# matteosantama/dantzig

Hardware: AMD Instinct MI355X
Metric: simplex_iterations_per_sec (higher is better)
Workload: dtype f64

## Files before the change

dantzig_amd/_build.py:

```python
from __future__ import annotations

import os
import shutil
import subprocess
from concurrent.futures import ThreadPoolExecutor

HERE = os.path.dirname(os.path.abspath(__file__))
CSRC = os.path.join(HERE, "csrc")
OBJ = os.path.join(HERE, "_obj")
LIB = os.path.join(HERE, "libdantzig_amd.so")
ARCH = "gfx950"
SOURCES = ["engine.hip", "k_vector.hip", "k_price.hip", "k_strict.hip", "k_fast.hip", "k_chain.hip", "k_sparse.hip", "k_refactor.hip", "k_rowshard.hip", "k_drift.hip", "k_restart.hip", "k_extend.hip", "k_remove.hip", "k_batch.hip", "k_batch_fast.hip",
           "k_mip.hip", "k_duals.hip", "k_ranging.hip", "k_rays.hip", "model.cpp", "mip.cpp", "lpgen.cpp"]
FLAGS = ["-O3", "-std=c++17", "-fPIC", "-ffp-contract=off", "-fno-fast-math", "-Wall",
         "-Wno-unused-result", "-Wno-unused-value"]


def _hipcc() -> str:
    exe = shutil.which("hipcc") or "/opt/rocm/bin/hipcc"
    if not os.path.exists(exe):
        raise RuntimeError("hipcc not found: dantzig_amd needs the ROCm toolchain to build")
    return exe


def _newest(paths) -> float:
    return max(os.path.getmtime(p) for p in paths)


def _deps():
    hdrs = [os.path.join(CSRC, "common.h"), os.path.join(CSRC, "k_price_kernels.h"),
            os.path.join(CSRC, "fast_decide.h"), os.path.join(CSRC, "fast_rows.h"),
            os.path.join(CSRC, "chain_barrier.h"), os.path.join(CSRC, "batch_strict.h"),
            os.path.join(CSRC, "batch_host.h"),
            os.path.join(CSRC, "mip_internal.h"), os.path.join(CSRC, "duals.h"), os.path.join(CSRC, "ranging.h"), os.path.join(CSRC, "rays.h"),
            os.path.join(os.path.dirname(HERE), "include", "dantzig_amd.h")]
    return hdrs


def _compile(src: str) -> str:
    path = os.path.join(CSRC, src)
    obj = os.path.join(OBJ, src + ".o")
    if os.path.exists(obj) and os.path.getmtime(obj) >= _newest([path] + _deps()):
        return obj
    cmd = [_hipcc(), f"--offload-arch={ARCH}", *FLAGS, "-c", path, "-o", obj]
    if src.endswith(".cpp"):
        cmd.insert(1, "-x")
        cmd.insert(2, "c++")
        cmd = [c for c in cmd if not c.startswith("--offload-arch")]
    subprocess.check_call(cmd)
    return obj


def build(force: bool = False, verbose: bool = False) -> str:
    os.makedirs(OBJ, exist_ok=True)
    if force:
        for f in os.listdir(OBJ):
            os.remove(os.path.join(OBJ, f))
    with ThreadPoolExecutor(max_workers=4) as ex:
        objs = list(ex.map(_compile, SOURCES))
    if force or not os.path.exists(LIB) or os.path.getmtime(LIB) < _newest(objs):
        cmd = [_hipcc(), f"--offload-arch={ARCH}", "-shared", "-fPIC", "-o", LIB, *objs, "-ldl", "-pthread"]
        subprocess.check_call(cmd)
    if verbose:
        print("built", LIB)
    return LIB


if __name__ == "__main__":
    import sys

    build(force="--force" in sys.argv, verbose=True)
```

dantzig_amd/_ffi.py:

```python
from __future__ import annotations

import ctypes as C
import os

import numpy as np

_HERE = os.path.dirname(os.path.abspath(__file__))
LIB_PATH = os.path.join(_HERE, "libdantzig_amd.so")

OPTIMAL, UNBOUNDED, INFEASIBLE, ITER_LIMIT, SINGULAR, PANIC, RUNNING, NEAR_TIE, NODE_LIMIT = range(9)
E_DEVICE, E_ARG, E_NOMEM = -1, -2, -3
STRICT, FAST, AUTO = 0, 1, 2
PRICE_AUTO, PRICE_SEQ, PRICE_WAVE, PRICE_TREE = 0, 1, 2, 3
STEP_PRIMAL, STEP_DUAL = 0, 1
NEAR_TIE_COUNT, NEAR_TIE_STOP = 0, 1
(K_STATUS, K_FTRAN, K_RATIO, K_BTRAN, K_PRICE, K_UPDATE, K_BASIS_UPDATE, K_LU, K_XCHG1, K_XCHG2,
 K_COUNT) = range(11)
KERNEL_CLASSES = ["status", "ftran", "ratio", "btran", "price", "update", "basis_update", "lu",
                  "exchange1", "exchange2"]

EXPORTS = [
    "dzg_abi_version", "dzg_status_str", "dzg_last_error", "dzg_device_count",
    "dzg_opts_default", "dzg_solver_create", "dzg_solver_run", "dzg_solver_result",
    "dzg_solver_destroy", "dzg_core_solve", "dzg_model_solve", "dzg_build_standard_form",
    "dzg_kernel_lu_solve", "dzg_kernel_neg_t_dot", "dzg_kernel_first_pivot",
    "dzg_kernel_second_pivot", "dzg_gen_dense_lp", "dzg_gen_sparse_lp", "dzg_merge_candidates",
    "dzg_shard_record_doubles", "dzg_shard_phase1", "dzg_shard_phase2", "dzg_shard_phase3",
    "dzg_solver_poll", "dzg_solver_set_budget", "dzg_comm_unique_id", "dzg_shard_comm_init",
    "dzg_shard_run", "dzg_shard_run_lockstep", "dzg_solver_stream", "dzg_solver_refactor",
    "dzg_gen_dense_lp_block", "dzg_solver_set_profile", "dzg_kernel_neg_t_dot_csc",
    "dzg_shard_comm_size", "dzg_solver_upload_columns", "dzg_debug_hold_cus", "dzg_debug_hold_wait",
    "dzg_core_solve_full_csc", "dzg_debug_live_lists", "dzg_debug_rl_listed",
    "dzg_debug_basis_inverse", "dzg_batch_solve", "dzg_model_solve_batch", "dzg_mip_opts_default",
    "dzg_mip_solve", "dzg_mip_last_warm_stats", "dzg_debug_cand_reduce", "dzg_debug_chain_instance",
    "dzg_solver_duals", "dzg_batch_solve_duals", "dzg_model_solve_duals",
    "dzg_model_solve_batch_duals", "dzg_model_map_duals",
    "dzg_solver_ranging", "dzg_batch_solve_ranging", "dzg_model_solve_ranging",
    "dzg_model_solve_batch_ranging",
    "dzg_solver_ray", "dzg_batch_solve_rays", "dzg_model_solve_rays", "dzg_model_solve_batch_rays",
    "dzg_model_map_ray",
    "dzg_batch_solve_fast", "dzg_model_solve_batch_fast", "dzg_debug_batch_fast_inverse",
    "dzg_solver_reoptimize",
    "dzg_solver_extend", "dzg_solver_dims", "dzg_debug_matrix", "dzg_debug_matrix_rows",
    "dzg_debug_extend_ms",
    "dzg_solver_remove",
]

BATCH_MAX_ROWS = 128
DUALS_FRESH, DUALS_CARRIED = 1, 2
DUALS_SOURCE_NAMES = {DUALS_FRESH: "fresh", DUALS_CARRIED: "carried"}
RAY_PRIMAL, RAY_FARKAS = 1, 2


class Lp(C.Structure):
    _fields_ = [
        ("m", C.c_int64), ("n", C.c_int64), ("n_struct", C.c_int64),
        ("a", C.c_void_p), ("lda", C.c_int64), ("var_col", C.c_void_p),
        ("c", C.c_void_p), ("constant", C.c_double),
        ("basis", C.c_void_p), ("nonbasis", C.c_void_p), ("x", C.c_void_p), ("z", C.c_void_p),
        ("col_ptr", C.c_void_p), ("row_idx", C.c_void_p), ("val", C.c_void_p),
        ("xbar", C.c_void_p), ("zbar", C.c_void_p),
    ]


class Opts(C.Structure):
    _fields_ = [
        ("numerics", C.c_int32), ("price_kernel", C.c_int32), ("device", C.c_int32),
        ("auto_strict_rows", C.c_int32), ("max_iter", C.c_int64), ("epsilon", C.c_double),
        ("log_capacity", C.c_int64), ("poll_interval", C.c_int32), ("profile", C.c_int32),
        ("col_begin", C.c_int64), ("col_end", C.c_int64), ("rank", C.c_int32),
        ("world", C.c_int32), ("stream", C.c_void_p), ("refactor_interval", C.c_int64),
        ("a_is_block", C.c_int32), ("near_tie_action", C.c_int32),
        ("replicate_matrix", C.c_int32), ("auto_restart_rows", C.c_int32), ("tie_tol", C.c_double),
        ("seven_launches", C.c_int32), ("auto_strict_budget_s", C.c_int32),
        ("shard_rows", C.c_int32), ("reserved0", C.c_int32),
    ]


class Pivot(C.Structure):
    _fields_ = [("kind", C.c_int32), ("reserved", C.c_int32), ("entering", C.c_int64),
                ("leaving", C.c_int64), ("mu", C.c_double)]


class Result(C.Structure):
    _fields_ = [
        ("status", C.c_int32), ("numerics_used", C.c_int32), ("iterations", C.c_int64),
        ("objective", C.c_double),
        ("basis", C.c_void_p), ("nonbasis", C.c_void_p), ("x", C.c_void_p), ("xbar", C.c_void_p),
        ("z", C.c_void_p), ("zbar", C.c_void_p), ("log", C.c_void_p), ("log_cap", C.c_int64),
        ("kernel_ms", C.c_double * K_COUNT), ("kernel_launches", C.c_int64 * K_COUNT),
        ("price_bytes", C.c_double), ("solve_ms", C.c_double), ("max_pivot_error", C.c_double),
        ("near_ties", C.c_int64), ("first_near_tie", C.c_int64), ("min_margin", C.c_double),
        ("margins", C.c_void_p), ("dense_columns", C.c_int64), ("refactors", C.c_int64),
        ("chain_fallbacks", C.c_int64), ("price_pass_used", C.c_int32),
        ("price_rows_copy", C.c_int32), ("state_drift", C.c_double),
    ]


class Model(C.Structure):
    _fields_ = [
        ("nvars", C.c_int64), ("has_lb", C.c_void_p), ("has_ub", C.c_void_p),
        ("lb", C.c_void_p), ("ub", C.c_void_p),
        ("obj_nterms", C.c_int64), ("obj_var", C.c_void_p), ("obj_coef", C.c_void_p),
        ("obj_const", C.c_double),
        ("ncons", C.c_int64), ("con_ptr", C.c_void_p), ("con_var", C.c_void_p),
        ("con_coef", C.c_void_p), ("con_b", C.c_void_p),
    ]


class ModelResult(C.Structure):
    _fields_ = [("status", C.c_int32), ("numerics_used", C.c_int32), ("iterations", C.c_int64),
                ("objective", C.c_double), ("values", C.c_void_p), ("m", C.c_int64),
                ("n", C.c_int64), ("near_ties", C.c_int64), ("first_near_tie", C.c_int64)]


class Duals(C.Structure):
    _fields_ = [("source", C.c_int32), ("reserved", C.c_int32), ("y", C.c_void_p), ("d", C.c_void_p),
# ... 66 lines not shown
class MipWarmStats(C.Structure):
    _fields_ = [("nodes_warm", C.c_int64), ("nodes_restarted", C.c_int64),
                ("warm_iterations", C.c_int64), ("restart_iterations", C.c_int64)]


class MipNode(C.Structure):
    _fields_ = [("id", C.c_int64), ("parent", C.c_int64), ("branch_var", C.c_int64),
                ("direction", C.c_int32), ("status", C.c_int32), ("bound", C.c_double),
                ("iterations", C.c_int64), ("objective", C.c_double)]


class MipResult(C.Structure):
    _fields_ = [("status", C.c_int32), ("has_incumbent", C.c_int32), ("objective", C.c_double),
                ("values", C.c_void_p), ("best_bound", C.c_double), ("nodes_solved", C.c_int64),
                ("nodes_batched", C.c_int64), ("nodes_sequential", C.c_int64), ("nodes_fast", C.c_int64),
                ("nodes_pruned", C.c_int64), ("nodes_dropped", C.c_int64), ("rounds", C.c_int64),
                ("lp_iterations", C.c_int64), ("incumbent_node", C.c_int64), ("failed_node", C.c_int64),
                ("log", C.c_void_p), ("log_cap", C.c_int64), ("log_count", C.c_int64)]


class Candidate(C.Structure):
    _fields_ = [("ratio", C.c_double), ("pos", C.c_int64), ("y", C.c_double),
                ("ybar", C.c_double), ("dy", C.c_double)]


class DantzigAmdError(RuntimeError):
    """A call into the HIP engine failed (no GPU, bad argument, out of memory)."""


_lib = None


def lib() -> C.CDLL:
    global _lib
    if _lib is None:
        if not os.path.exists(LIB_PATH):
            raise DantzigAmdError(
                f"{LIB_PATH} is missing: build the HIP engine first "
                "(python -m dantzig_amd._build). dantzig_amd has no CPU fallback.")
        _lib = C.CDLL(LIB_PATH)
        _lib.dzg_status_str.restype = C.c_char_p
        _lib.dzg_last_error.restype = C.c_char_p
        _lib.dzg_merge_candidates.restype = C.c_int64
        _lib.dzg_solver_destroy.restype = None
        _lib.dzg_opts_default.restype = None
        _lib.dzg_gen_dense_lp.argtypes = [C.c_uint64, C.c_int64, C.c_int64, C.c_void_p, C.c_int64,
                                          C.c_void_p, C.c_void_p]
        _lib.dzg_gen_dense_lp_block.argtypes = [C.c_uint64, C.c_int64, C.c_int64, C.c_int64,
                                                C.c_int64, C.c_void_p, C.c_int64, C.c_void_p,
                                                C.c_void_p]
        _lib.dzg_solver_run.argtypes = [C.c_void_p, C.c_int64]
        _lib.dzg_solver_result.argtypes = [C.c_void_p, C.c_void_p]
        _lib.dzg_solver_destroy.argtypes = [C.c_void_p]
        _lib.dzg_shard_record_doubles.restype = C.c_int64
        _lib.dzg_shard_record_doubles.argtypes = [C.c_void_p]
        _lib.dzg_shard_phase1.argtypes = [C.c_void_p, C.c_void_p]
        _lib.dzg_shard_phase2.argtypes = [C.c_void_p, C.c_void_p, C.c_void_p]
        _lib.dzg_shard_phase3.argtypes = [C.c_void_p, C.c_void_p]
        _lib.dzg_solver_poll.argtypes = [C.c_void_p, C.c_void_p, C.c_void_p]
        _lib.dzg_solver_set_budget.argtypes = [C.c_void_p, C.c_int64]
        _lib.dzg_comm_unique_id.argtypes = [C.c_void_p]
        _lib.dzg_shard_comm_init.argtypes = [C.c_void_p, C.c_void_p]
        _lib.dzg_shard_run.argtypes = [C.c_void_p, C.c_int64]
        _lib.dzg_shard_comm_size.argtypes = [C.c_void_p]
        _lib.dzg_shard_run_lockstep.argtypes = [C.c_void_p, C.c_int32, C.c_int64]
        _lib.dzg_solver_stream.restype = C.c_void_p
        _lib.dzg_solver_stream.argtypes = [C.c_void_p]
        _lib.dzg_solver_refactor.argtypes = [C.c_void_p]
        _lib.dzg_solver_set_profile.argtypes = [C.c_void_p, C.c_int32]
        _lib.dzg_core_solve_full_csc.argtypes = [C.c_int64, C.c_int64, C.c_void_p, C.c_void_p,
                                                 C.c_void_p, C.c_void_p, C.c_double, C.c_void_p,
                                                 C.c_void_p, C.c_void_p, C.c_void_p, C.c_void_p,
                                                 C.c_void_p]
        _lib.dzg_debug_hold_cus.argtypes = [C.c_int32, C.c_int32, C.c_double]
        _lib.dzg_debug_live_lists.restype = C.c_int64
        _lib.dzg_debug_live_lists.argtypes = [C.c_void_p, C.c_void_p]
        _lib.dzg_debug_basis_inverse.restype = C.c_int
        _lib.dzg_debug_basis_inverse.argtypes = [C.c_void_p, C.c_int64, C.c_int64, C.c_void_p, C.c_void_p]
        _lib.dzg_debug_cand_reduce.restype = C.c_int
        _lib.dzg_debug_cand_reduce.argtypes = [C.c_int32, C.c_int32, C.c_int64, C.c_void_p, C.c_void_p,
                                               C.c_void_p, C.c_void_p, C.c_void_p, C.c_void_p, C.c_void_p]
        _lib.dzg_debug_chain_instance.restype = C.c_int
        _lib.dzg_debug_chain_instance.argtypes = [C.c_int32] * 7
        _lib.dzg_batch_solve.argtypes = [C.c_void_p, C.c_int64, C.c_void_p, C.c_int64, C.c_void_p]
        _lib.dzg_model_solve_batch.argtypes = [C.c_void_p, C.c_int64, C.c_void_p, C.c_void_p]
        _lib.dzg_batch_solve_fast.argtypes = [C.c_void_p, C.c_int64, C.c_void_p, C.c_int64, C.c_int64,
                                              C.c_void_p]
        _lib.dzg_model_solve_batch_fast.argtypes = [C.c_void_p, C.c_int64, C.c_void_p, C.c_void_p]
        _lib.dzg_debug_batch_fast_inverse.restype = C.c_int
        _lib.dzg_debug_batch_fast_inverse.argtypes = [C.c_void_p, C.c_int64, C.c_void_p, C.c_int64, C.c_int64,
                                                      C.c_void_p, C.c_void_p]
        _lib.dzg_solver_duals.argtypes = [C.c_void_p, C.c_void_p]
        _lib.dzg_batch_solve_duals.argtypes = [C.c_void_p, C.c_int64, C.c_void_p, C.c_int64, C.c_void_p,
                                               C.c_void_p]
        _lib.dzg_model_solve_duals.argtypes = [C.c_void_p, C.c_void_p, C.c_void_p, C.c_void_p]
        _lib.dzg_model_solve_batch_duals.argtypes = [C.c_void_p, C.c_int64, C.c_void_p, C.c_void_p,
                                                     C.c_void_p]
        _lib.dzg_model_map_duals.argtypes = [C.c_void_p, C.c_void_p, C.c_int64, C.c_void_p]
        _lib.dzg_solver_ranging.argtypes = [C.c_void_p, C.c_void_p, C.c_void_p, C.c_void_p]
        _lib.dzg_batch_solve_ranging.argtypes = [C.c_void_p, C.c_int64, C.c_void_p, C.c_int64, C.c_void_p,
                                                 C.c_void_p, C.c_void_p, C.c_void_p]
        _lib.dzg_model_solve_ranging.argtypes = [C.c_void_p, C.c_void_p, C.c_void_p, C.c_void_p, C.c_void_p,
                                                 C.c_void_p]
        _lib.dzg_model_solve_batch_ranging.argtypes = [C.c_void_p, C.c_int64, C.c_void_p, C.c_void_p,
                                                       C.c_void_p, C.c_void_p, C.c_void_p]
        _lib.dzg_solver_ray.argtypes = [C.c_void_p, C.c_void_p]
        _lib.dzg_batch_solve_rays.argtypes = [C.c_void_p, C.c_int64, C.c_void_p, C.c_int64, C.c_void_p,
                                              C.c_void_p, C.c_void_p]
        _lib.dzg_model_solve_rays.argtypes = [C.c_void_p, C.c_void_p, C.c_void_p, C.c_void_p, C.c_void_p]
        _lib.dzg_model_solve_batch_rays.argtypes = [C.c_void_p, C.c_int64, C.c_void_p, C.c_void_p,
                                                    C.c_void_p, C.c_void_p]
        _lib.dzg_model_map_ray.argtypes = [C.c_void_p, C.c_int32, C.c_void_p, C.c_void_p, C.c_int64,
                                           C.c_int64, C.c_void_p]
        _lib.dzg_solver_reoptimize.argtypes = [C.c_void_p, C.c_void_p]
        _lib.dzg_solver_extend.argtypes = [C.c_void_p, C.c_void_p]
        _lib.dzg_solver_remove.argtypes = [C.c_void_p, C.c_void_p, C.c_void_p, C.c_void_p]
        _lib.dzg_solver_dims.argtypes = [C.c_void_p, C.c_void_p, C.c_void_p, C.c_void_p]
        _lib.dzg_debug_matrix.argtypes = [C.c_void_p, C.c_int64, C.c_int64, C.c_void_p, C.c_int64]
        _lib.dzg_debug_matrix_rows.restype = C.c_int64
        _lib.dzg_debug_matrix_rows.argtypes = [C.c_void_p, C.c_int64, C.c_int64, C.c_void_p, C.c_int64]
        _lib.dzg_debug_extend_ms.argtypes = [C.c_void_p, C.c_void_p]
        _lib.dzg_mip_opts_default.restype = None
        _lib.dzg_mip_opts_default.argtypes = [C.c_void_p]
        _lib.dzg_mip_solve.argtypes = [C.c_void_p, C.c_void_p, C.c_void_p, C.c_void_p, C.c_void_p]
        _lib.dzg_mip_last_warm_stats.restype = None
        _lib.dzg_mip_last_warm_stats.argtypes = [C.c_void_p]
        _lib.dzg_solver_upload_columns.argtypes = [C.c_void_p, C.c_int64, C.c_int64, C.c_void_p,
                                                   C.c_int64]
    return _lib


def ptr(a: np.ndarray | None) -> C.c_void_p:
    return C.c_void_p(None if a is None else a.ctypes.data)


def f64(a) -> np.ndarray:
    return np.ascontiguousarray(a, dtype=np.float64)


def i64(a) -> np.ndarray:
    return np.ascontiguousarray(a, dtype=np.int64)


def status_str(code: int) -> str:
    return lib().dzg_status_str(int(code)).decode()


def check(rc: int, what: str) -> int:
    if rc < 0:
        msg = lib().dzg_last_error().decode()
        raise DantzigAmdError(f"{what}: {status_str(rc)} ({msg})")
    return rc


class RangingBuffers:

    def __init__(self, cost_dirs, rhs_dirs, pivot_tol: float = 0.0):
        def csr(dirs):
            ptr_, idx, val = [0], [], []
            for d in dirs:
                for j, v in d.items():
                    idx.append(int(j))
                    val.append(float(v))
                ptr_.append(len(idx))
            return i64(ptr_), i64(idx + [0]), f64(val + [0.0])

# ... 90 lines not shown
```

dantzig_amd/core.py:

```python
from __future__ import annotations

import ctypes as C
from dataclasses import dataclass, field

import numpy as np

from . import _ffi
from ._ffi import (AUTO, FAST, STRICT, PRICE_AUTO, PRICE_SEQ, PRICE_WAVE, PRICE_TREE,
                   STEP_DUAL,
                   STEP_PRIMAL, NEAR_TIE_COUNT, NEAR_TIE_STOP, DantzigAmdError, f64, i64, ptr)

STATUS_NAMES = {0: "optimal", 1: "unbounded", 2: "infeasible", 3: "iter_limit", 4: "singular",
                5: "panic", 6: "running", 7: "near_tie"}


@dataclass
class CoreLP:
    a: np.ndarray | None
    c: np.ndarray
    basis: np.ndarray
    nonbasis: np.ndarray
    x: np.ndarray
    z: np.ndarray
    var_col: np.ndarray | None = None
# ... 416 lines not shown
        c = None if c is None else f64(c)
        if b is not None and b.shape != (m,):
            raise ValueError(f"reoptimize: b has shape {b.shape}, the LP has {m} rows")
        if c is not None and c.shape != (n,):
            raise ValueError(f"reoptimize: c has shape {c.shape}, the LP has {n} variables")
        chg = _ffi.Reopt(ptr(b), ptr(c), 0.0 if constant is None else float(constant),
                         0 if constant is None else 1, 0)
        _ffi.check_reopt(_ffi.lib().dzg_solver_reoptimize(self._h, C.byref(chg)), "dzg_solver_reoptimize")

    def extend(self, rows=None, rhs=None, cols=None, c_cols=None) -> None:
        lp2 = extended_lp(self._lp, rows, rhs, cols, c_cols)
        m, ns = self._lp.m, self._lp.n_struct
        rows, rhs, cols, c_cols = _extend_blocks(m, ns, rows, rhs, cols, c_cols)
        p, r = len(rhs), len(c_cols)
        rows_rm = np.ascontiguousarray(rows)
        cols_cm = np.ascontiguousarray(cols.T)
        ext = _ffi.Extend(p, r, ptr(rows_rm) if p else None, max(ns, 1), ptr(rhs) if p else None,
                          ptr(cols_cm) if r else None, max(m + p, 1), ptr(c_cols) if r else None)
        _ffi.check_extend(_ffi.lib().dzg_solver_extend(self._h, C.byref(ext)), "dzg_solver_extend")
        self._lp = lp2

    def _at_current_basis(self) -> CoreLP:
        import dataclasses

        res = self.result(log=False)
        return dataclasses.replace(self._lp, basis=res.basis, nonbasis=res.nonbasis, x=res.x, z=res.z,
                                   xbar=None, zbar=None)

    def removable(self) -> tuple[np.ndarray, np.ndarray]:
        if self._lp.a is None or self._lp.block is not None:
            raise NotImplementedError("remove is not supported on CSC storage or sharded solvers")
        m, ns = self._lp.m, self._lp.n_struct
        res = self.result(log=False)
        codes = _codes(self._lp)
        in_basis, out_of_basis = codes[res.basis], codes[res.nonbasis]
        row_mask, col_mask = np.zeros(m, bool), np.zeros(ns, bool)
        row_mask[-1 - in_basis[in_basis < 0]] = True
        col_mask[out_of_basis[out_of_basis >= 0]] = True
        return row_mask, col_mask

    def remove(self, rows=None, cols=None) -> tuple[np.ndarray, np.ndarray]:
        if self._lp.a is None or self._lp.block is not None:
            raise NotImplementedError("remove is not supported on CSC storage or sharded solvers")
        drop_row, drop_col = _remove_lists(self._lp.m, self._lp.n_struct, rows, cols)
        lp2, _, _ = reduced_lp(self._at_current_basis(), rows, cols)
        r, c = np.flatnonzero(drop_row).astype(np.int64), np.flatnonzero(drop_col).astype(np.int64)
        var_map, row_map = np.zeros(self._lp.n, np.int64), np.zeros(self._lp.m, np.int64)
        rem = _ffi.Remove(len(r), ptr(r) if len(r) else None, len(c), ptr(c) if len(c) else None)
        _ffi.check_extend(_ffi.lib().dzg_solver_remove(self._h, C.byref(rem), ptr(var_map), ptr(row_map)),
                          "dzg_solver_remove")
        self._lp = lp2
        return var_map, row_map

    def dims(self) -> tuple[int, int, int]:
        v = [C.c_int64(0), C.c_int64(0), C.c_int64(0)]
        _ffi.check(_ffi.lib().dzg_solver_dims(self._h, *(C.byref(x) for x in v)), "dzg_solver_dims")
        return tuple(int(x.value) for x in v)

    def debug_matrix(self) -> np.ndarray:
        m, _, ns = self.dims()
        out = np.zeros((max(ns, 1), max(m, 1)))
        _ffi.check(_ffi.lib().dzg_debug_matrix(self._h, 0, ns, ptr(out), max(m, 1)), "dzg_debug_matrix")
        return out[:ns, :m].T.copy()

    def debug_matrix_rows(self) -> np.ndarray | None:
        m, _, ns = self.dims()
        out = np.zeros((max(m, 1), max(ns, 1)))
        got = _ffi.lib().dzg_debug_matrix_rows(self._h, 0, m, ptr(out), max(ns, 1))
        _ffi.check(int(got), "dzg_debug_matrix_rows")
        return out[:m, :ns].copy() if got == m and m > 0 else None

    def debug_extend_ms(self) -> tuple[float, float, float]:
        ms = np.zeros(3)
        _ffi.check(_ffi.lib().dzg_debug_extend_ms(self._h, ptr(ms)), "dzg_debug_extend_ms")
        return tuple(float(x) for x in ms)

    def debug_inverse(self, row0: int, row1: int) -> tuple[np.ndarray, dict]:
        m = self._lp.m
        out = np.zeros((max(int(row1) - int(row0), 0), m))
        info = np.zeros(4, np.int64)
        _ffi.check(_ffi.lib().dzg_debug_basis_inverse(self._h, int(row0), int(row1), ptr(out), ptr(info)),
                   "dzg_debug_basis_inverse")
        return out, dict(k=int(info[0]), neta=int(info[1]), rows=(int(info[2]), int(info[3])))

    def close(self) -> None:
        if self._h:
            _ffi.lib().dzg_solver_destroy(self._h)
            self._h = C.c_void_p(None)

    def __enter__(self):
        return self

    def __exit__(self, *exc):
        self.close()

    def __del__(self):
        try:
            self.close()
        except Exception:
            pass


def solve(lp: CoreLP, log: bool = True, **opts) -> CoreResult:
    with Solver(lp, **opts) as s:
        s.run(0)
        return s.result(log=log)


def core_solve(lp: CoreLP, log_cap: int = 1 << 20, **opts) -> CoreResult:
    with Solver.__new__(Solver)._prepare(lp, opts) as s:
        m, q = lp.m, lp.n - lp.m
        basis, nonbasis = np.zeros(max(m, 1), np.int64), np.zeros(max(q, 1), np.int64)
        x, xbar = np.zeros(max(m, 1)), np.zeros(max(m, 1))
        z, zbar = np.zeros(max(q, 1)), np.zeros(max(q, 1))
        buf = (_ffi.Pivot * max(log_cap, 1))()
        margins = np.full(max(log_cap, 1), np.inf)
        r = _ffi.Result()
        r.basis, r.nonbasis, r.x, r.xbar = ptr(basis), ptr(nonbasis), ptr(x), ptr(xbar)
        r.z, r.zbar = ptr(z), ptr(zbar)
        r.log, r.log_cap, r.margins = C.cast(buf, C.c_void_p), log_cap, ptr(margins)
        rc = _ffi.lib().dzg_core_solve(C.byref(s._c_lp), C.byref(s._opts), C.byref(r))
        _ffi.check(rc, "dzg_core_solve")
        cnt = int(min(r.iterations, log_cap))
        arr = np.ctypeslib.as_array(buf)[:cnt]
        pivots = list(zip(arr["kind"].tolist(), arr["entering"].tolist(),
                          arr["leaving"].tolist(), arr["mu"].tolist()))
        return CoreResult(
            status=STATUS_NAMES.get(r.status, str(r.status)), status_code=r.status,
            numerics="strict" if r.numerics_used == STRICT else "fast",
            iterations=int(r.iterations), objective=float(r.objective),
            basis=basis[:m].copy(), nonbasis=nonbasis[:q].copy(), x=x[:m].copy(),
            xbar=xbar[:m].copy(), z=z[:q].copy(), zbar=zbar[:q].copy(), pivots=pivots,
            margins=margins[:cnt].copy(), **_counters(r))


_PIVOT_DTYPE = np.dtype([("kind", "<i4"), ("reserved", "<i4"), ("entering", "<i8"),
                         ("leaving", "<i8"), ("mu", "<f8")])


def solve_batch(lps, log: bool = True, log_cap: int = 4096, pivots_per_launch: int = 0,
                duals: bool = False, ranging=False, pivot_tol: float = 0.0, rays: bool = False,
                **opts) -> list:
    import time

    lps = list(lps)
    numerics = opts.get("numerics", AUTO)
    if numerics not in (STRICT, AUTO):
        raise ValueError("solve_batch runs STRICT numerics only (numerics=STRICT or AUTO)")
    if rays and ranging is not False and ranging is not None:
        raise ValueError("rays=True and ranging: the ranging call carries no ray; ask in two calls")
    for i, lp in enumerate(lps):
        if lp.block is not None:
            raise ValueError(f"lps[{i}]: a column-block LP cannot be batched")
        if lp.a is None and lp.n_struct > 0:
            raise ValueError(f"lps[{i}]: CSC input cannot be batched (dense `a` only)")
        if lp.m > _ffi.BATCH_MAX_ROWS:
            raise ValueError(f"lps[{i}]: {lp.m} rows; the batch takes at most {_ffi.BATCH_MAX_ROWS}")
    marshalled = [_c_lp(lp) for lp in lps]
    count = len(lps)
    c_lps = (_ffi.Lp * max(count, 1))(*[c for c, _ in marshalled])
    ms = [lp.m for lp in lps]
    qs = [lp.n - lp.m for lp in lps]
    mo = np.concatenate([[0], np.cumsum(ms)]).astype(np.int64)
    qo = np.concatenate([[0], np.cumsum(qs)]).astype(np.int64)
    basis, x, xbar = np.zeros(mo[-1] + 1, np.int64), np.zeros(mo[-1] + 1), np.zeros(mo[-1] + 1)
    nonbasis, z, zbar = np.zeros(qo[-1] + 1, np.int64), np.zeros(qo[-1] + 1), np.zeros(qo[-1] + 1)
# ... 303 lines not shown
```

dantzig_amd/csrc/common.h:

```cpp
#pragma once

#include <hip/hip_runtime.h>
#include <stdint.h>

#include "../../include/dantzig_amd.h"

#define DZG_WAVE 64

struct DzgCtl {
    int status;
    int kind;
    long long iter;
    long long iter_stop;
    int enter_pos;
    int leave_pos;
    int enter_var;
    int leave_var;
    double mu;
    double t, s, tbar, sbar;
    long long nb_struct;
    double price_bytes;
    int lu_mu;
    int lu_pivot_zero;
    int ncompact;
// ... 457 lines not shown
    double *P0, *P1;
    int *piv;
    int *pz;
    int *ptab;
    double *part_r;
    int *part_k;
    int nparts;
};
void dzg_lu_layout(int n, DzgLu *w);

struct __attribute__((aligned(16))) DzgLiveEntry {
    int row;
    int pad_;
    double val;
};

struct DzgDev {
    int m, q, n, ns;
    long long lda;
    const double *A;
    int csc;
    const long long *cptr;
    const int *ridx;
    const double *cval;
    const int *var_col;
    int *basis, *nonbasis;
    double *x, *xbar, *z, *zbar;
    double *dx, *dz, *v, *acol;
    DzgCtl *ctl;
    int *log_kind, *log_enter, *log_leave;
    double *log_mu;
    long long log_cap;
    double *binv;
    long long ldb;
    int *drow;
    int *dslot;
    double *U;
    double *W;
    long long ldw;
    double *Wc;
    double *ag;
    double *beta;
    double *beta_part;
    int beta_split;
    int *plist;
    int *pslot;
    int *pcode;
    int *cpos;
    double *fpx_r, *fpz_r, *rx_r, *rz_r;
    int *fpx_k, *fpz_k, *rx_k, *rz_k;
    double *fpx_h, *fpz_h, *rx_h, *rz_h;
    double *log_margin;
    int *bcode, *nbcode;
    int spb;
    const long long *rptr;
    const int *cidx;
    const double *rval;
    int *sslot;
    int *spos;
    int *bslot;
    int *rowpos;
    int *bcnt;
    int *bcol;
    double *bval;
    double *dxs;
    int *acol_code;
    int *lcnt;
    DzgLiveEntry *lent;
    unsigned long long *rl_work;
    DzgLu lu;
    double eps;
    int col0, col1, rank, world;
    int repl;
    long long xstride;
    const double *At;
    long long ldt;
    double *ppart;
    double *vc;
    int rows_T;
    int k_lo_hint;
    int k_hint;
    int price_cols_hint;
    int rs, rs_r0, rs_r1;
    long long rs_mcol;
    int ftran_variant;
    int ftran_nt_k;
    int fold_k;
};

#ifdef __HIPCC__
__device__ __forceinline__ const double *dzg_enter_col(const DzgCtl *ctl, int code,
                                                       const double *A, long long lda, int col0,
                                                       const double *xrecv, long long xstride)
{
    if (code < 0) return nullptr;
    if (xrecv && xstride > 8) return xrecv + (long long)ctl->enter_src * xstride + 8;
    return A + (long long)(code - col0) * lda;
}
#endif

void dzg_launch_status(const DzgDev &d, hipStream_t st);
void dzg_launch_ratio(const DzgDev &d, int need_kind, hipStream_t st);
void dzg_launch_prepare(const DzgDev &d, hipStream_t st);
void dzg_launch_update_vectors(const DzgDev &d, hipStream_t st);
void dzg_launch_load_column(const DzgDev &d, int need_kind, hipStream_t st);
void dzg_launch_unit_rhs(const DzgDev &d, hipStream_t st);
int dzg_run_first_pivot(int64_t len, const double *y, const double *ybar, int64_t *pos_out);
int dzg_run_second_pivot(int64_t len, double mu, const double *y, const double *ybar,
                         const double *dy, int64_t *pos_out);

void dzg_launch_price(const DzgDev &d, int kernel, hipStream_t st);
void dzg_launch_price_fast(const DzgDev &d, int kernel, hipStream_t st, int need_kind = -1,
                           int skip_finish = 0, int small = 0, unsigned long long *dbg = nullptr);
int dzg_price_small(const DzgDev &d, int kernel);
int dzg_price_small_partials(const DzgDev &d);
int dzg_price_rows_certain(const DzgDev &d, int kernel);
void dzg_launch_transpose_to_rows(const double *A, long long lda, int m, int n, double *At,
                                  long long ldt, hipStream_t st);
int dzg_price_rows_groups(void);
int dzg_price_partials(int kernel);
int dzg_price_partials_dev(const DzgDev &d, int kernel);
#define DZG_PRICE_CSC_KERNEL 100
#define DZG_RL_WORK_SLOTS 2048
void dzg_launch_price_raw(int kernel, int m, long long lda, const double *A, const int *cols,
                          int ncols, const double *v, double *out, hipStream_t st);
void dzg_launch_price_csc_raw(const long long *cptr, const int *ridx, const double *cval,
                              const int *cols, int ncols, const double *v, double *out,
                              hipStream_t st);

void dzg_launch_strict_solve(const DzgDev &d, int transposed, hipStream_t st);
void dzg_launch_lu_raw(const DzgLu &w, DzgCtl *ctl, double *x_out, hipStream_t st);

void dzg_launch_fast_init(const DzgDev &d, hipStream_t st);
void dzg_launch_fast_select_prep(const DzgDev &d, int mode, int nrz, const double *xrecv,
                                 hipStream_t st);
void dzg_launch_fast_gemv(const DzgDev &d, int need_kind, const double *xrecv, hipStream_t st);
void dzg_launch_fast_btran(const DzgDev &d, hipStream_t st);
void dzg_launch_fast_update(const DzgDev &d, int only_partials, hipStream_t st);
void dzg_launch_fast_flush(const DzgDev &d, hipStream_t st);
void dzg_launch_refactor_lists(const DzgDev &d, int *spos, int *scode, int *lpos, int *lrow,
                               int *counts, hipStream_t st);
void dzg_launch_refactor_a(const DzgDev &d, int k, double *G, double *X, long long ldg, int *scode,
                           int *singular, hipStream_t st);
double *dzg_launch_refactor_b(const DzgDev &d, int k, int nl, double *G, double *X, double *Pn, double *Tri,
                              long long ldg,
                              int *piv, int *spos, int *scode, int *lpos, int *lrow, int *lslot,
                              int *singular, hipStream_t st);
void dzg_launch_refactor_c(const DzgDev &d, int k, int nl, double *G, double *X, long long ldg,
                           int *lpos, int *singular, hipStream_t st);
void dzg_launch_lockstep_sum(double *const *bufs, int world, long long count, hipStream_t st);
void dzg_launch_shard_propose(const DzgDev &d, int mode, int nrz, double *xsend, hipStream_t st);
void dzg_launch_lockstep_allgather(double *const *ptrs, int world, int which, long long xstride,
                                   hipStream_t st);

#define DZG_CHAIN_AGCAP 16384
#define DZG_CHAIN_BAR_WORDS (16 * 10)
int dzg_chain_resident_per_cu(void);
enum {
    DZG_CHAIN_GENERIC = 0,
    DZG_CHAIN_P1_NARROW = 1,
    DZG_CHAIN_P4_NARROW = 2,
    DZG_CHAIN_P4_WIDE = 3,
};
void dzg_launch_chain_pre(const DzgDev &d, int grid, unsigned long long *bar,
                          unsigned long long *dbg, const double *xrecv, hipStream_t st, int instances = 0);
void dzg_launch_chain_post(const DzgDev &d, int grid, unsigned long long *bar,
                           unsigned long long *dbg, int only_partials, int nrz, const double *xrecv,
                           hipStream_t st, int fold = 0, int price_small = 0, int instances = 0);

void dzg_launch_rs_propose(const DzgDev &d, int mode, int nrz, double *xsend, hipStream_t st);
void dzg_launch_rs_select(const DzgDev &d, int mode, const double *xrecv, hipStream_t st);
void dzg_launch_rs_gemv(const DzgDev &d, int kind, const double *xrecv1, const double *xrecv2,
                        hipStream_t st);
void dzg_launch_rs_books(const DzgDev &d, const double *xrecv1, hipStream_t st);
void dzg_launch_rs_lockstep_gather(double *const *ptrs, int world, int m, int slice, hipStream_t st);
void dzg_launch_rs_pack(const DzgDev &d, int slice, double *send, hipStream_t st);
void dzg_launch_rs_unpack(const DzgDev &d, int slice, const double *recv, hipStream_t st);

void dzg_launch_drift(const DzgDev &d, const double *b0, const double *xb0, const double *cdev,
                      const double *cbdev, double *agb, double *agx, double *part, double *y, double *dzy, double *out,
                      int k_bound, hipStream_t st);
int dzg_drift_blocks(void);
int dzg_drift_chunks(void);

void dzg_launch_restart_x(const DzgDev &d, const double *rhs, double *ag, int k_bound, hipStream_t st);
void dzg_launch_restart_z(const DzgDev &d, const double *cdev, const double *dzy, hipStream_t st);

void dzg_launch_extend_restride(const double *src, long long lda, double *dst, long long ldn, int m, int ncols,
                                hipStream_t st);
void dzg_launch_extend_rows(const double *rows, long long ldr, int p, int ns, double *A, long long lda, int row0,
                            hipStream_t st);

void dzg_launch_remove_gather(const double *src, long long lda, double *dst, long long ldn, int m,
                              const int *keep_row, int mk, const int *keep_col, int nk, hipStream_t st);

void dzg_launch_sp_init(const DzgDev &d, int first, hipStream_t st);
void dzg_launch_sp_ftran(const DzgDev &d, int need_kind, int nrz, hipStream_t st);
void dzg_launch_sp_btran(const DzgDev &d, hipStream_t st);
void dzg_launch_sp_pivot(const DzgDev &d, hipStream_t st);
void dzg_launch_sp_update(const DzgDev &d, int only_partials, hipStream_t st);
void dzg_launch_sp_flush(const DzgDev &d, hipStream_t st);
void dzg_launch_sp_ref_copy(const DzgDev &d, int k, const double *Xinv, long long ldx, hipStream_t st);
int dzg_sp_grid(int m);
int dzg_sp_fused_resident_per_cu(void);
void dzg_launch_sp_pre(const DzgDev &d, unsigned long long *bar, hipStream_t st);
void dzg_launch_sp_mid(const DzgDev &d, unsigned long long *bar, int nrz, hipStream_t st);
```

dantzig_amd/csrc/engine.hip:

```cpp
#include <dlfcn.h>

#include <chrono>
#include <cstdio>
#include <cstdlib>
#include <cstring>
#include <limits>
#include <string>
#include <utility>
#include <algorithm>
#include <vector>

#include "common.h"
#include "duals.h"
#include "ranging.h"
#include "rays.h"

static thread_local std::string g_err;

static int fail(int code, const std::string &msg)
{
    g_err = msg;
    return code;
}

// ... 21 lines not shown
    case DZG_NEAR_TIE: return "near_tie";
    case DZG_NODE_LIMIT: return "node_limit";
    case DZG_E_DEVICE: return "device_error";
    case DZG_E_ARG: return "bad_argument";
    case DZG_E_NOMEM: return "out_of_memory";
    default: return "unknown";
    }
}

extern "C" int dzg_device_count(void)
{
    int n = 0;
    if (hipGetDeviceCount(&n) != hipSuccess) return 0;
    return n;
}

extern "C" void dzg_opts_default(dzg_opts *o)
{
    std::memset(o, 0, sizeof(*o));
    o->numerics = DZG_NUMERICS_AUTO;
    o->price_kernel = DZG_PRICE_AUTO;
    o->device = 0;
    o->auto_strict_rows = 192;
    o->max_iter = 10000000;
    o->epsilon = 1e-12;
    o->log_capacity = -1;
    o->poll_interval = 32;
    o->profile = 0;
    o->world = 1;
    o->near_tie_action = DZG_NEAR_TIE_COUNT;
    o->auto_restart_rows = DZG_AUTO_STRICT_RESTART_ROWS;
    o->tie_tol = 1e-11;
}

struct dzg_solver {
    DzgDev d{};
    dzg_opts opts{};
    int numerics = DZG_NUMERICS_FAST;
    hipStream_t st = nullptr;
    bool own_stream = true;
    DzgCtl *h_ctl = nullptr;
    std::vector<void *> allocs;
    std::vector<double> c_host;
    std::vector<double> x0_host;
    std::vector<int> var_col_host;
    double constant = 0.0;
    double solve_ms = 0.0;
    int since_flush = 0;
    double *rfG = nullptr, *rfX = nullptr, *rfPn = nullptr, *rfTri = nullptr;
    long long rf_ld = 0, rf_rows = 0;
    int *rf_piv = nullptr, *rf_spos = nullptr, *rf_scode = nullptr, *rf_lpos = nullptr,
        *rf_lrow = nullptr, *rf_counts = nullptr, *rf_lslot = nullptr;
    long long since_refactor = 0;
    bool pending_refactor = false;
    bool in_lockstep = false;
    hipGraphExec_t g_solve[2] = {nullptr, nullptr};
    bool graphs_tried = false;
    int prof_slot = -1;
    int64_t refactors = 0;
    double *A_alloc = nullptr;
    long long cols_present = 0;
    std::vector<std::pair<int64_t, int64_t>> col_blocks;
    double drift_trigger = 1e-9;
    double max_err_life = 0.0;
    double state_drift = 0.0;
    double *dr_b0 = nullptr, *dr_xb0 = nullptr, *dr_c = nullptr, *dr_cb = nullptr, *dr_agb = nullptr,
           *dr_agx = nullptr,
           *dr_part = nullptr, *dr_y = nullptr, *dr_dzy = nullptr, *dr_out = nullptr;
    double *du_c = nullptr, *du_rhs0 = nullptr, *du_part = nullptr, *du_y = nullptr, *du_dzy = nullptr,
           *du_d = nullptr, *du_out = nullptr;
    int *du_codes = nullptr;
    DzgCtl *du_ctl = nullptr;
    double *ry_vec = nullptr, *ry_d = nullptr, *ry_part = nullptr, *ry_h = nullptr, *ry_res = nullptr;
    double *ro_ag = nullptr;
    double *ro_res = nullptr;
    double extend_ms[3] = {0.0, 0.0, 0.0};
    unsigned long long *chain_bar = nullptr;
    unsigned long long *chain_dbg = nullptr;
    int chain_grid = 0;
    long long chain_kcap = DZG_CHAIN_AGCAP;
    bool batch_chain = false;
    bool chain_fold = true;
    bool chain_instances = true;
    int64_t chain_fallbacks = 0;
    long long chain_retry_iter = 0;
    void *comm = nullptr;
    double *xsend = nullptr, *xrecv1 = nullptr, *xrecv2 = nullptr;
    long long xstride_max = 0;
    const double *rs_recv1 = nullptr;
    int rs_slice = 0;
    double *rs_gsend = nullptr, *rs_grecv = nullptr;
    std::vector<hipEvent_t> ev;
    double kernel_ms[DZG_K_COUNT] = {};
    int64_t kernel_launches[DZG_K_COUNT] = {};
};

template <typename T> static int dev_alloc(dzg_solver *s, T **p, size_t count)
{
    void *q = nullptr;
    size_t bytes = sizeof(T) * (count ? count : 1);
    if (hipMalloc(&q, bytes) != hipSuccess)
        return fail(DZG_E_NOMEM, "hipMalloc of " + std::to_string(bytes) + " bytes failed");
    s->allocs.push_back(q);
    *p = static_cast<T *>(q);
    return 0;
}

#define TRY(expr)            \
    do {                     \
        int rc_ = (expr);    \
        if (rc_ != 0) return rc_; \
    } while (0)

static int validate(const dzg_lp *lp, std::string &why, bool matrix_on_device = false)
{
    if (!lp) { why = "lp is NULL"; return 0; }
    if (lp->m < 0 || lp->n < lp->m || lp->n_struct < 0 || lp->n_struct > lp->n) { why = "bad sizes"; return 0; }
    if (lp->n >= (1ll << 31) - 64 || lp->m >= (1ll << 31) - 64) { why = "index range"; return 0; }
    if (lp->n_struct > 0 && lp->a && lp->lda < lp->m) { why = "lda"; return 0; }
    if (lp->n_struct > 0 && !lp->a && !matrix_on_device) {
        if (!lp->col_ptr || lp->col_ptr[0] != 0) { why = "neither a nor col_ptr"; return 0; }
        for (int64_t j = 0; j < lp->n_struct; ++j) {
            if (lp->col_ptr[j + 1] < lp->col_ptr[j]) { why = "col_ptr not monotone"; return 0; }
            for (int64_t e = lp->col_ptr[j]; e < lp->col_ptr[j + 1]; ++e) {
                if (!lp->row_idx || !lp->val || lp->row_idx[e] < 0 || lp->row_idx[e] >= lp->m ||
                    (e > lp->col_ptr[j] && lp->row_idx[e] <= lp->row_idx[e - 1])) {
                    why = "row_idx must ascend strictly inside a column";
                    return 0;
                }
            }
        }
    }
    const int64_t q = lp->n - lp->m;
    if ((lp->m > 0 && (!lp->basis || !lp->x)) || (q > 0 && (!lp->nonbasis || !lp->z)) || (lp->n > 0 && !lp->c)) { why = "NULL state vector"; return 0; }
    if (!lp->var_col && lp->n != lp->n_struct + lp->m) { why = "var_col == NULL needs n == n_struct + m"; return 0; }
    std::vector<char> seen((size_t)lp->n, 0);
    for (int64_t k = 0; k < lp->n; ++k) {
        int64_t v = k < lp->m ? lp->basis[k] : lp->nonbasis[k - lp->m];
        if (v < 0 || v >= lp->n || seen[(size_t)v]) { why = "basis/nonbasis is not a partition of 0..n-1"; return 0; }
        seen[(size_t)v] = 1;
    }
    if (lp->var_col) {
        for (int64_t v = 0; v < lp->n; ++v) {
            int64_t c = lp->var_col[v];
            if (c >= lp->n_struct || c < -lp->m) { why = "var_col out of range"; return 0; }
        }
    }
    return 1;
}

int dzg_set_error(int code, const std::string &msg) { return fail(code, msg); }
int dzg_lp_valid(const dzg_lp *lp, std::string &why) { return validate(lp, why); }

namespace {
struct NcclUniqueId { char internal[128]; };
struct Rccl {
    void *handle = nullptr;
    int (*GetUniqueId)(NcclUniqueId *) = nullptr;
    int (*CommInitRank)(void **, int, NcclUniqueId, int) = nullptr;
    int (*AllGather)(const void *, void *, size_t, int, void *, hipStream_t) = nullptr;
    int (*AllReduce)(const void *, void *, size_t, int, int, void *, hipStream_t) = nullptr;
    int (*CommDestroy)(void *) = nullptr;
    int (*CommCount)(void *, int *) = nullptr;
    const char *(*GetErrorString)(int) = nullptr;
    bool ok = false;
};
// ... 464 lines not shown
        if (!d.csc) TRY(dev_alloc(s, &d.cpos, (size_t)(d.col1 > d.col0 ? d.col1 - d.col0 : 1)));
        const size_t np = 4096;
        TRY(dev_alloc(s, &d.fpx_r, np)); TRY(dev_alloc(s, &d.fpz_r, np));
        TRY(dev_alloc(s, &d.rx_r, np)); TRY(dev_alloc(s, &d.rz_r, np));
        TRY(dev_alloc(s, &d.fpx_k, np)); TRY(dev_alloc(s, &d.fpz_k, np));
        TRY(dev_alloc(s, &d.rx_k, np)); TRY(dev_alloc(s, &d.rz_k, np));
        TRY(dev_alloc(s, &d.fpx_h, np)); TRY(dev_alloc(s, &d.fpz_h, np));
        TRY(dev_alloc(s, &d.rx_h, np)); TRY(dev_alloc(s, &d.rz_h, np));
        if (o.refactor_interval != 0) TRY(refactor_workspace(s));
        if (d.spb && !o.seven_launches) {
            hipDeviceProp_t prop;
            HIP_OK(hipGetDeviceProperties(&prop, o.device));
            const int cus = prop.multiProcessorCount > 0 ? prop.multiProcessorCount : 1;
            const char *off = std::getenv("DZG_SP_FUSED");
            if (!(off && off[0] == '0') && (long long)dzg_sp_fused_resident_per_cu() * cus >= dzg_sp_grid(m)) {
                TRY(dev_alloc(s, &s->chain_bar, (size_t)DZG_CHAIN_BAR_WORDS));
                HIP_OK(hipMemsetAsync(s->chain_bar, 0, sizeof(unsigned long long) * DZG_CHAIN_BAR_WORDS, s->st));
            }
        }
        if (d.spb) {
            TRY(dev_alloc(s, &d.sslot, (size_t)m)); TRY(dev_alloc(s, &d.spos, (size_t)m));
            TRY(dev_alloc(s, &d.bslot, (size_t)(ns ? ns : 1))); TRY(dev_alloc(s, &d.rowpos, (size_t)m));
            TRY(dev_alloc(s, &d.dxs, (size_t)m)); TRY(dev_alloc(s, &d.acol_code, 1));
            HIP_OK(hipMemsetAsync(d.acol, 0, sizeof(double) * (size_t)(m ? m : 1), s->st));
            HIP_OK(hipMemsetAsync(d.dxs, 0, sizeof(double) * (size_t)(m ? m : 1), s->st));
        }
        if (!d.csc && !o.seven_launches && !d.rs) {
            hipDeviceProp_t prop;
            HIP_OK(hipGetDeviceProperties(&prop, o.device));
            int grid = prop.multiProcessorCount > 0 ? prop.multiProcessorCount : 1;
            if (grid > 256) grid = 256;
            const int per_cu = dzg_chain_resident_per_cu();
            if (per_cu < 1) grid = 0;
            if (const char *g = std::getenv("DZG_CHAIN_GRID")) {
                const int v = std::atoi(g);
                if (v >= 1 && v < grid) grid = v;
            }
            const int gdiv = grid > 0 ? grid : 1;
            const long long rows_per = (((long long)m + gdiv - 1) / gdiv + 3) & ~3ll;
            const long long cols_per = ((long long)q + gdiv - 1) / gdiv;
            if (grid >= 1 && rows_per <= 512 && cols_per <= 512) {
                s->chain_grid = grid;
                if (const char *cap = std::getenv("DZG_CHAIN_KCAP")) {
                    const long long v = std::atoll(cap);
                    if (v >= 0 && v < s->chain_kcap) s->chain_kcap = v;
                }
                if (const char *dbg = std::getenv("DZG_CHAIN_DEBUG")) {
                    if (dbg[0] == '1') {
                        TRY(dev_alloc(s, &s->chain_dbg, (size_t)16 * DZG_STAMP_SLOTS));
                        HIP_OK(hipMemsetAsync(s->chain_dbg, 0, sizeof(unsigned long long) * 16 * DZG_STAMP_SLOTS, s->st));
                    }
                }
                if (const char *nf = std::getenv("DZG_CHAIN_NO_FOLD")) s->chain_fold = nf[0] != '1';
                if (const char *ci = std::getenv("DZG_CHAIN_INSTANCES")) s->chain_instances = ci[0] != '0';
                TRY(dev_alloc(s, &s->chain_bar, (size_t)DZG_CHAIN_BAR_WORDS));
                HIP_OK(hipMemsetAsync(s->chain_bar, 0, sizeof(unsigned long long) * DZG_CHAIN_BAR_WORDS, s->st));
            }
        }
        {
            const char *rows_env = std::getenv("DZG_PRICE_ROWS");
            const int nown = d.col1 - d.col0;
            if (!d.csc && o.price_kernel == DZG_PRICE_AUTO && m > 0 && nown > 0 && ns > 0 &&
                !(rows_env && rows_env[0] == '0')) {
                d.ldt = ((long long)nown + 3) / 4 * 4;
                void *at_mem = nullptr;
                if (hipMalloc(&at_mem, sizeof(double) * (size_t)m * (size_t)d.ldt) != hipSuccess) {
                    (void)hipGetLastError();
                    at_mem = nullptr;
                }
                double *at = static_cast<double *>(at_mem);
                if (at) {
                    s->allocs.push_back(at_mem);
                    TRY(dev_alloc(s, &d.ppart, (size_t)dzg_price_rows_groups() * (size_t)d.ldt));
                    TRY(dev_alloc(s, &d.vc, (size_t)m));
                    HIP_OK(hipMemsetAsync(d.vc, 0, sizeof(double) * (size_t)m, s->st));
                    dzg_launch_transpose_to_rows(d.A, d.lda, m, nown, at, d.ldt, s->st);
                }
                d.At = at;
                d.rows_T = (int)(0.93 * (double)m * (double)ns / ((double)ns + (double)m));
                if (const char *t = std::getenv("DZG_PRICE_ROWS_T")) d.rows_T = std::atoi(t);
                if (d.rows_T < 1) { d.At = nullptr; d.vc = nullptr; }
            }
        }
        dzg_launch_fast_init(d, s->st);
        if (d.spb) {
            dzg_launch_sp_init(d, 1, s->st);
            dzg_launch_sp_update(d, 1, s->st);
        } else {
            dzg_launch_fast_update(d, 1, s->st);
        }
        if (needs_initial_refactor && src) {
            HIP_OK(hipStreamSynchronize(s->st));
            const auto t0 = std::chrono::steady_clock::now();
            TRY(refactor_now(s));
            HIP_OK(hipStreamSynchronize(s->st));
            s->extend_ms[1] = ms_since(t0);
        } else if (needs_initial_refactor) {
            TRY(refactor_now(s));
        }
    } else {
        dzg_lu_layout(m, &d.lu);
        const size_t mm = (size_t)(m ? m : 1);
        TRY(dev_alloc(s, &d.lu.W, mm * (size_t)d.lu.ldw));
        TRY(dev_alloc(s, &d.lu.P0, mm * DZG_LU_LDP)); TRY(dev_alloc(s, &d.lu.P1, mm * DZG_LU_LDP));
        TRY(dev_alloc(s, &d.lu.piv, mm)); TRY(dev_alloc(s, &d.lu.pz, mm));
        TRY(dev_alloc(s, &d.lu.ptab, mm * DZG_LU_NB));
        TRY(dev_alloc(s, &d.lu.part_r, (size_t)2 * d.lu.nparts));
        TRY(dev_alloc(s, &d.lu.part_k, (size_t)2 * d.lu.nparts));
    }
    if (o.profile) {
        s->ev.resize((size_t)o.poll_interval * DZG_K_COUNT * 2);
        for (auto &e : s->ev) HIP_OK(hipEventCreateWithFlags(&e, hipEventDisableSystemFence));
    }
    HIP_OK(hipStreamSynchronize(s->st));
    HIP_OK(hipGetLastError());
    guard.s = nullptr;
    *out = s;
    return 0;
}

extern "C" int dzg_solver_create(const dzg_lp *lp, const dzg_opts *opts_in, dzg_solver **out)
{
    return solver_create(lp, opts_in, out, nullptr);
}

namespace {
static inline bool prof_on(const dzg_solver *s, int cls, int slot)
{
    const int p = s->opts.profile;
    if (p == 0 || slot < 0) return false;
    if (p < 0) return true;
    const int stride = (p >> 16) & 0xff;
    return (p & (1 << cls)) && (stride <= 1 || slot % stride == stride - 1);
}

struct Prof {
    dzg_solver *s;
    int slot;
    void begin(int cls) const
    {
        if (prof_on(s, cls, slot))
            hipEventRecord(s->ev[((size_t)slot * DZG_K_COUNT + cls) * 2], s->st);
    }
    void end(int cls) const
    {
        if (prof_on(s, cls, slot))
            hipEventRecord(s->ev[((size_t)slot * DZG_K_COUNT + cls) * 2 + 1], s->st);
    }
};
}

static int price_kernel_for(const dzg_solver *s)
{
    if (s->d.csc)
        return s->opts.price_kernel == DZG_PRICE_SEQ ? DZG_PRICE_SEQ : DZG_PRICE_CSC_KERNEL;
    if (s->opts.price_kernel != DZG_PRICE_AUTO) return s->opts.price_kernel;
    return DZG_PRICE_TREE;
}

static int price_partials_for(const dzg_solver *s, int pk)
{
    return dzg_price_partials_dev(s->d, pk);
}

static void enqueue_fast_iteration(dzg_solver *s, int slot)
{
    const DzgDev &d = s->d;
    hipStream_t st = s->st;
    Prof pf{s, slot};
    const int pk = price_kernel_for(s);
    pf.begin(DZG_K_STATUS);
    dzg_launch_fast_select_prep(d, 0, 0, nullptr, st);
    pf.end(DZG_K_STATUS);
    pf.begin(DZG_K_FTRAN);
    dzg_launch_fast_gemv(d, DZG_STEP_PRIMAL, nullptr, st);
    pf.end(DZG_K_FTRAN);
    pf.begin(DZG_K_BTRAN);
    dzg_launch_fast_btran(d, st);
    pf.end(DZG_K_BTRAN);
    pf.begin(DZG_K_PRICE);
    dzg_launch_price_fast(d, pk, st);
    pf.end(DZG_K_PRICE);
    pf.begin(DZG_K_RATIO);
    dzg_launch_fast_select_prep(d, 1, price_partials_for(s, pk), nullptr, st);
    dzg_launch_fast_gemv(d, DZG_STEP_DUAL, nullptr, st);
    pf.end(DZG_K_RATIO);
    pf.begin(DZG_K_UPDATE);
    dzg_launch_fast_update(d, 0, st);
    pf.end(DZG_K_UPDATE);
    if (++s->since_flush >= DZG_RMAX) {
        pf.begin(DZG_K_BASIS_UPDATE);
        dzg_launch_fast_flush(d, st);
        pf.end(DZG_K_BASIS_UPDATE);
        s->since_flush = 0;
    } else {
        pf.begin(DZG_K_BASIS_UPDATE);
        pf.end(DZG_K_BASIS_UPDATE);
    }
}

static void enqueue_chain_iteration(dzg_solver *s, int slot)
{
    const DzgDev &d = s->d;
    hipStream_t st = s->st;
    Prof pf{s, slot};
    const int pk = price_kernel_for(s);
    pf.begin(DZG_K_FTRAN);
    dzg_launch_chain_pre(d, s->chain_grid, s->chain_bar, s->chain_dbg, nullptr, st,
                         s->chain_instances);
    pf.end(DZG_K_FTRAN);
    const int small = dzg_price_small(d, pk);
    const int fold = !small && s->chain_fold && dzg_price_rows_certain(d, pk);
    pf.begin(DZG_K_PRICE);
    dzg_launch_price_fast(d, pk, st, -1, fold, small, small ? s->chain_dbg : nullptr);
    pf.end(DZG_K_PRICE);
    pf.begin(DZG_K_UPDATE);
    dzg_launch_chain_post(d, s->chain_grid, s->chain_bar, s->chain_dbg, 0,
                          small ? dzg_price_small_partials(d)
                                : (fold ? s->chain_grid : price_partials_for(s, pk)),
                          nullptr, st, fold, small, s->chain_instances);
    pf.end(DZG_K_UPDATE);
    pf.begin(DZG_K_BASIS_UPDATE);
    if (++s->since_flush >= DZG_RMAX) {
        dzg_launch_fast_flush(d, st);
        s->since_flush = 0;
    }
    pf.end(DZG_K_BASIS_UPDATE);
}

static void enqueue_sparse_iteration(dzg_solver *s, int slot)
{
    const DzgDev &d = s->d;
    hipStream_t st = s->st;
    Prof pf{s, slot};
    if (s->batch_chain) {
        const int pk = price_kernel_for(s);
        pf.begin(DZG_K_FTRAN);
        dzg_launch_sp_pre(d, s->chain_bar, st);
        pf.end(DZG_K_FTRAN);
        pf.begin(DZG_K_PRICE);
        dzg_launch_price_fast(d, pk, st);
        pf.end(DZG_K_PRICE);
        pf.begin(DZG_K_RATIO);
        dzg_launch_sp_mid(d, s->chain_bar, price_partials_for(s, pk), st);
        pf.end(DZG_K_RATIO);
        pf.begin(DZG_K_UPDATE);
        dzg_launch_sp_update(d, 0, st);
        pf.end(DZG_K_UPDATE);
        pf.begin(DZG_K_BASIS_UPDATE);
        if (++s->since_flush >= DZG_RMAX) {
            dzg_launch_sp_flush(d, st);
            s->since_flush = 0;
        }
        pf.end(DZG_K_BASIS_UPDATE);
        return;
    }
    pf.begin(DZG_K_FTRAN);
    dzg_launch_sp_ftran(d, DZG_STEP_PRIMAL, 0, st);
    pf.end(DZG_K_FTRAN);
    pf.begin(DZG_K_BTRAN);
    dzg_launch_sp_btran(d, st);
    pf.end(DZG_K_BTRAN);
    pf.begin(DZG_K_PRICE);
    dzg_launch_price_fast(d, price_kernel_for(s), st);
    pf.end(DZG_K_PRICE);
    pf.begin(DZG_K_RATIO);
    dzg_launch_sp_ftran(d, DZG_STEP_DUAL, price_partials_for(s, price_kernel_for(s)), st);
    pf.end(DZG_K_RATIO);
    pf.begin(DZG_K_UPDATE);
    dzg_launch_sp_pivot(d, st);
    dzg_launch_sp_update(d, 0, st);
    pf.end(DZG_K_UPDATE);
    pf.begin(DZG_K_BASIS_UPDATE);
    if (++s->since_flush >= DZG_RMAX) {
        dzg_launch_sp_flush(d, st);
        s->since_flush = 0;
    }
    pf.end(DZG_K_BASIS_UPDATE);
}

static void collect_profile(dzg_solver *s, int slots_real)
{
    if (!s->opts.profile) return;
    for (int slot = 0; slot < slots_real; ++slot)
        for (int cls = 0; cls < DZG_K_COUNT; ++cls) {
            if (!prof_on(s, cls, slot)) continue;
            if (s->d.csc && !s->d.spb && s->d.world == 1 && !s->comm && cls != DZG_K_PRICE)
                continue;
            if (s->batch_chain && s->d.world == 1 && !s->comm &&
                (cls == DZG_K_STATUS || cls == DZG_K_BTRAN || (cls == DZG_K_RATIO && !s->d.spb)))
                continue;
            float ms = 0.f;
            size_t base = ((size_t)slot * DZG_K_COUNT + cls) * 2;
            if (hipEventElapsedTime(&ms, s->ev[base], s->ev[base + 1]) == hipSuccess) {
                s->kernel_ms[cls] += ms;
                s->kernel_launches[cls] += 1;
            }
// ... 63 lines not shown
                   s->h_ctl->status == DZG_INFEASIBLE))
        *active = true;
    if (!*active) return 0;
    if (counts[0] != s->h_ctl->ncompact)
        return fail(DZG_E_DEVICE, "refactor: structural basics != dense columns");
    TRY(refactor_panels(s, counts[0], counts[1]));
    dzg_launch_refactor_a(d, counts[0], s->rfG, s->rfX, s->rf_ld, s->rf_scode, s->rf_counts + 2, s->st);
    return 0;
}

static int refactor_stage_b(dzg_solver *s, const int counts[2], double **block)
{
    *block = dzg_launch_refactor_b(s->d, counts[0], counts[1], s->rfG, s->rfX, s->rfPn, s->rfTri, s->rf_ld,
                                   s->rf_piv, s->rf_spos, s->rf_scode, s->rf_lpos, s->rf_lrow, s->rf_lslot,
                                   s->rf_counts + 2, s->st);
    return 0;
}

static int refactor_stage_c(dzg_solver *s, const int counts[2])
{
    dzg_launch_refactor_c(s->d, counts[0], counts[1], s->rfG, s->rfX, s->rf_ld, s->rf_lpos,
                          s->rf_counts + 2, s->st);
    s->since_flush = 0;
    s->h_ctl->neta = 0;
    s->since_refactor = 0;
    s->refactors += 1;
    s->pending_refactor = false;
    return 0;
}

static int shard_sum(dzg_solver *s, double *buf, size_t count)
{
    if (count == 0) return 0;
    Rccl &r = rccl();
    if (!s->comm || !r.ok || !r.AllReduce)
        return fail(DZG_E_ARG, "refactorisation of a partitioned column-sharded solver needs its "
                               "ranks' columns: dzg_shard_comm_init first (or the lockstep loop)");
    if (r.AllReduce(buf, buf, count, kNcclFloat64, kNcclSum, s->comm, s->st) != 0)
        return fail(DZG_E_DEVICE, "ncclAllReduce (basic columns of a refactorisation)");
    return 0;
}

static int measure_drift(dzg_solver *s)
{
    if (!s->dr_b0 || s->d.world != 1 || s->d.spb) return 0;
    DzgDev &d = s->d;
    if (!s->dr_out) {
        TRY(dev_alloc(s, &s->dr_agb, (size_t)d.m + 2)); TRY(dev_alloc(s, &s->dr_agx, (size_t)d.m + 2));
        TRY(dev_alloc(s, &s->dr_part, (size_t)dzg_drift_chunks() * (size_t)d.ldw));
        TRY(dev_alloc(s, &s->dr_y, (size_t)d.m + 2)); TRY(dev_alloc(s, &s->dr_dzy, (size_t)d.q));
        TRY(dev_alloc(s, &s->dr_out, (size_t)8 * dzg_drift_blocks()));
    }
    dzg_launch_drift(d, s->dr_b0, s->dr_xb0, s->dr_c, s->dr_cb, s->dr_agb, s->dr_agx, s->dr_part, s->dr_y,
                     s->dr_dzy, s->dr_out, (int)s->h_ctl->ncompact, s->st);
    const int nb = dzg_drift_blocks();
    std::vector<double> out((size_t)8 * nb);
    HIP_OK(hipMemcpyAsync(out.data(), s->dr_out, sizeof(double) * out.size(), hipMemcpyDeviceToHost, s->st));
    HIP_OK(hipStreamSynchronize(s->st));
    double e[8] = {0, 0, 0, 0, 0, 0, 0, 0};
    for (int b = 0; b < nb; ++b) {
        for (int j = 0; j < 4; ++j) e[j] = std::max(e[j], out[(size_t)4 * b + j]);
        for (int j = 0; j < 2; ++j) e[4 + j] = std::max(e[4 + j], out[(size_t)4 * nb + 2 * b + j]);
        for (int j = 0; j < 2; ++j) e[6 + j] = std::max(e[6 + j], out[(size_t)6 * nb + 2 * b + j]);
    }
    double drift = 0.0;
    for (int j = 0; j < 8; j += 2) {
        const double rel = e[j] / std::max(1.0, e[j + 1]);
        if (rel == rel && rel > drift) drift = rel;
    }
    s->state_drift = drift;
    DzgCtl *h = s->h_ctl;
    h->drift_tau = 4.0 * drift;
    HIP_OK(hipMemcpyAsync(&d.ctl->drift_tau, &h->drift_tau, sizeof(double), hipMemcpyHostToDevice, s->st));
    if (h->tie_tol >= 0.0) {
        h->tau = std::max(h->tie_tol, h->drift_tau);
        HIP_OK(hipMemcpyAsync(&d.ctl->tau, &h->tau, sizeof(double), hipMemcpyHostToDevice, s->st));
    }
    HIP_OK(hipStreamSynchronize(s->st));
    return 0;
}

static int refactor_now(dzg_solver *s, bool at_end)
{
    if (partitioned(s) && s->in_lockstep)
        return fail(DZG_E_ARG, "refactor: the lockstep loop refactorises its ranks together");
    int counts[2];
    bool active = false;
    TRY(refactor_stage_a(s, counts, &active, at_end));
    if (!active) return 0;
    if (partitioned(s)) TRY(shard_sum(s, s->rfG, (size_t)counts[0] * (size_t)s->rf_ld));
    double *block = nullptr;
    TRY(refactor_stage_b(s, counts, &block));
    if (partitioned(s) && block) TRY(shard_sum(s, block, (size_t)counts[1] * (size_t)s->rf_ld));
    TRY(refactor_stage_c(s, counts));
    return measure_drift(s);
}

static int refactor_lockstep(dzg_solver **sv, int world)
{
    if (!partitioned(sv[0])) {
        for (int r = 0; r < world; ++r) TRY(refactor_now(sv[r]));
        return 0;
    }
    std::vector<int> counts((size_t)2 * world, 0);
    bool active = false;
    for (int r = 0; r < world; ++r) {
        bool a = false;
        TRY(refactor_stage_a(sv[r], &counts[(size_t)2 * r], &a));
        if (r > 0 && (a != active || counts[(size_t)2 * r] != counts[0] || counts[(size_t)2 * r + 1] != counts[1]))
            return fail(DZG_E_DEVICE, "lockstep refactor: ranks diverged");
        active = a;
    }
    if (!active) return 0;
    hipStream_t st = sv[0]->st;
    double **dptrs = nullptr;
    HIP_OK(hipMalloc(&dptrs, sizeof(double *) * (size_t)world));
    struct Free { double **p; ~Free() { hipFree(p); } } free_ptrs{dptrs};
    std::vector<double *> ptrs((size_t)world);
    for (int r = 0; r < world; ++r) ptrs[(size_t)r] = sv[r]->rfG;
    HIP_OK(hipMemcpyAsync(dptrs, ptrs.data(), sizeof(double *) * (size_t)world, hipMemcpyHostToDevice, st));
    dzg_launch_lockstep_sum(dptrs, world, (long long)counts[0] * sv[0]->rf_ld, st);
    HIP_OK(hipStreamSynchronize(st));
    bool any_block = false;
    for (int r = 0; r < world; ++r) {
        double *block = nullptr;
        TRY(refactor_stage_b(sv[r], &counts[(size_t)2 * r], &block));
        ptrs[(size_t)r] = block;
        any_block = any_block || block;
    }
    if (any_block) {
        HIP_OK(hipMemcpyAsync(dptrs, ptrs.data(), sizeof(double *) * (size_t)world, hipMemcpyHostToDevice, st));
        dzg_launch_lockstep_sum(dptrs, world, (long long)counts[1] * sv[0]->rf_ld, st);
        HIP_OK(hipStreamSynchronize(st));
    }
    for (int r = 0; r < world; ++r) TRY(refactor_stage_c(sv[r], &counts[(size_t)2 * r]));
    return 0;
}

extern "C" int dzg_solver_refactor(dzg_solver *s)
{
    if (!s || s->numerics != DZG_NUMERICS_FAST) return fail(DZG_E_ARG, "refactor: FAST solver");
    HIP_OK(hipSetDevice(s->opts.device));
    TRY(refactor_now(s));
    HIP_OK(hipStreamSynchronize(s->st));
    HIP_OK(hipGetLastError());
    return 0;
}

static int batch_size(const dzg_solver *s)
{
    const long long remaining = s->h_ctl->iter_stop - s->h_ctl->iter;
    const int poll = s->opts.poll_interval;
    return (int)(remaining < poll ? (remaining < 1 ? 1 : remaining) : poll);
}

static int health_stop(dzg_solver *s)
{
    if (s->h_ctl->max_pivot_err > 1e-4) {
        int st = DZG_SINGULAR;
        HIP_OK(hipMemcpy(&s->d.ctl->status, &st, sizeof(int), hipMemcpyHostToDevice));
        s->h_ctl->status = st;
    }
    return 0;
}

enum HealthAction { HEALTH_OK = 0, HEALTH_REFACTOR, HEALTH_GIVE_UP };

static bool can_refactor(const dzg_solver *s)
{
    return !partitioned(s) || s->comm != nullptr || s->in_lockstep;
}

static HealthAction health_decide(dzg_solver *s)
{
    if (!can_refactor(s)) return s->h_ctl->max_pivot_err > 1e-4 ? HEALTH_GIVE_UP : HEALTH_OK;
    if (!(s->h_ctl->max_pivot_err > s->drift_trigger && s->since_refactor > 0)) return HEALTH_OK;
    const bool fresh = s->refactors > 0 && s->since_refactor <= 2ll * s->opts.poll_interval;
    if (fresh) s->drift_trigger *= 100.0;
    if (fresh && s->h_ctl->max_pivot_err > 1e-4) return HEALTH_GIVE_UP;
    return HEALTH_REFACTOR;
}

static int health_give_up(dzg_solver *s, bool *stop)
{
    if (can_refactor(s)) s->h_ctl->max_pivot_err = 1.0;
    TRY(health_stop(s));
    *stop = s->h_ctl->status != DZG_RUNNING;
    return 0;
}

static int health_check(dzg_solver *s, bool *stop)
{
    *stop = false;
    switch (health_decide(s)) {
    case HEALTH_OK: return 0;
    case HEALTH_REFACTOR: {
        const int rrc = refactor_now(s);
        if (rrc == DZG_E_DEVICE || rrc == DZG_E_NOMEM) return rrc;
        if (rrc != 0) return health_give_up(s, stop);
        return 0;
    }
    default: return health_give_up(s, stop);
    }
}

static int budget_spent(dzg_solver *s, bool *spent)
{
    *spent = s->h_ctl->status == DZG_RUNNING && s->h_ctl->iter >= s->h_ctl->iter_stop;
    if (*spent) {
        int st = DZG_ITER_LIMIT;
        HIP_OK(hipMemcpy(&s->d.ctl->status, &st, sizeof(int), hipMemcpyHostToDevice));
        s->h_ctl->status = st;
    }
    return 0;
}

static int chain_recover(dzg_solver *s)
{
    DzgCtl *h = s->h_ctl;
    s->chain_fallbacks += 1;
    s->chain_retry_iter = s->chain_fallbacks >= 3 ? std::numeric_limits<long long>::max()
                                                  : h->iter + 64ll * s->opts.poll_interval;
    HIP_OK(hipMemsetAsync(s->chain_bar, 0, sizeof(unsigned long long) * DZG_CHAIN_BAR_WORDS, s->st));
    h->status = DZG_RUNNING;
    h->bar_timeout = 0;
    h->bar_gen = 0;
    HIP_OK(hipMemcpyAsync(&s->d.ctl->status, &h->status, sizeof(int), hipMemcpyHostToDevice, s->st));
    HIP_OK(hipMemcpyAsync(&s->d.ctl->bar_timeout, &h->bar_timeout, sizeof(int), hipMemcpyHostToDevice, s->st));
    HIP_OK(hipMemcpyAsync(&s->d.ctl->bar_gen, &h->bar_gen, sizeof(unsigned long long), hipMemcpyHostToDevice, s->st));
    HIP_OK(hipStreamSynchronize(s->st));
    return 0;
}

static int run_fast(dzg_solver *s)
{
    for (;;) {
        bool spent = false;
        TRY(budget_spent(s, &spent));
        if (spent) break;
        if (s->opts.refactor_interval > 0 && s->since_refactor >= s->opts.refactor_interval)
            TRY(refactor_now(s));
        const long long before = s->h_ctl->iter;
        const int batch = batch_size(s);
        s->since_flush = s->h_ctl->neta;
        s->d.price_cols_hint = (int)s->h_ctl->nb_struct + batch;
        const int k_bound = (int)s->h_ctl->ncompact + batch;
        const int k_low = (int)s->h_ctl->ncompact > batch ? (int)s->h_ctl->ncompact - batch : 0;
        if (s->d.spb) {
            s->d.k_hint = k_bound;
            s->batch_chain = s->chain_bar && s->h_ctl->iter >= s->chain_retry_iter;
            for (int b = 0; b < batch; ++b) enqueue_sparse_iteration(s, b);
            s->d.k_hint = 0;
        } else if (s->d.csc) {
            TRY(shard_buffers(s));
            const size_t nb = sizeof(double) * (size_t)s->d.xstride;
            for (int b = 0; b < batch; ++b) {
                s->prof_slot = s->opts.profile ? b : -1;
                TRY(dzg_shard_phase1(s, s->xsend));
                HIP_OK(hipMemcpyAsync(s->xrecv1, s->xsend, nb, hipMemcpyDeviceToDevice, s->st));
                TRY(dzg_shard_phase2(s, s->xrecv1, s->xsend));
                HIP_OK(hipMemcpyAsync(s->xrecv2, s->xsend, nb, hipMemcpyDeviceToDevice, s->st));
                TRY(dzg_shard_phase3(s, s->xrecv2));
            }
            s->prof_slot = -1;
        } else {
            s->batch_chain = s->chain_bar && s->h_ctl->iter >= s->chain_retry_iter &&
                             (long long)s->h_ctl->ncompact + batch <= s->chain_kcap;
            s->d.k_hint = k_bound;
            s->d.k_lo_hint = k_low;
            if (s->batch_chain)
                for (int b = 0; b < batch; ++b) enqueue_chain_iteration(s, b);
            else
                for (int b = 0; b < batch; ++b) enqueue_fast_iteration(s, b);
            s->d.k_hint = s->d.k_lo_hint = 0;
        }
        s->since_refactor += batch;
        TRY(read_ctl(s));
        HIP_OK(hipGetLastError());
        if (s->h_ctl->bar_timeout) {
            TRY(chain_recover(s));
            continue;
        }
        collect_profile(s, (int)(s->h_ctl->iter - before));
        if (s->h_ctl->status != DZG_RUNNING) break;
        bool stop = false;
        TRY(health_check(s, &stop));
        if (stop) break;
    }
    return 0;
}

static void strict_solve(dzg_solver *s, int transposed)
{
    const DzgDev &d = s->d;
    hipStream_t st = s->st;
    if (!s->graphs_tried) {
        s->graphs_tried = true;
        const bool off = getenv("DZG_NO_GRAPH") != nullptr;
        for (int t = 0; t < 2 && !off; ++t) {
            hipGraph_t graph = nullptr;
            if (hipStreamBeginCapture(st, hipStreamCaptureModeThreadLocal) != hipSuccess) break;
            dzg_launch_strict_solve(d, t, st);
            if (hipStreamEndCapture(st, &graph) != hipSuccess || !graph) {
                (void)hipGetLastError();
                break;
            }
            if (hipGraphInstantiate(&s->g_solve[t], graph, nullptr, nullptr, 0) != hipSuccess) {
                s->g_solve[t] = nullptr;
                (void)hipGetLastError();
            }
            hipGraphDestroy(graph);
        }
    }
    if (s->g_solve[transposed] && hipGraphLaunch(s->g_solve[transposed], st) == hipSuccess) return;
    dzg_launch_strict_solve(d, transposed, st);
}

static int run_strict(dzg_solver *s)
{
    const DzgDev &d = s->d;
    hipStream_t st = s->st;
    for (;;) {
        dzg_launch_status(d, st);
        TRY(read_ctl(s));
        if (s->h_ctl->status != DZG_RUNNING) break;
        if (s->h_ctl->kind == DZG_STEP_PRIMAL) {
            dzg_launch_load_column(d, -1, st);
            hipMemcpyAsync(d.dx, d.acol, sizeof(double) * (size_t)d.m, hipMemcpyDeviceToDevice, st);
            strict_solve(s, 0);
            dzg_launch_ratio(d, DZG_STEP_PRIMAL, st);
            dzg_launch_unit_rhs(d, st);
            strict_solve(s, 1);
            dzg_launch_price(d, DZG_PRICE_SEQ, st);
        } else {
            dzg_launch_unit_rhs(d, st);
            strict_solve(s, 1);
            dzg_launch_price(d, DZG_PRICE_SEQ, st);
            dzg_launch_ratio(d, DZG_STEP_DUAL, st);
            dzg_launch_load_column(d, -1, st);
            hipMemcpyAsync(d.dx, d.acol, sizeof(double) * (size_t)d.m, hipMemcpyDeviceToDevice, st);
            strict_solve(s, 0);
        }
        dzg_launch_prepare(d, st);
        dzg_launch_update_vectors(d, st);
    }
    HIP_OK(hipGetLastError());
    return 0;
}

static int set_budget(dzg_solver *s, int64_t max_new_iters)
{
    if (s->d.repl && s->cols_present != s->d.ns)
        return fail(DZG_E_ARG, "replicate_matrix: " + std::to_string(s->d.ns - s->cols_present) +
                               " structural columns have not been uploaded (dzg_solver_upload_columns)");
    s->d.k_hint = s->d.k_lo_hint = 0;
    if (s->pending_refactor && !partitioned(s)) TRY(refactor_now(s));
// ... 32 lines not shown

extern "C" int dzg_solver_set_profile(dzg_solver *s, int32_t mask)
{
    if (!s) return fail(DZG_E_ARG, "solver is NULL");
    if (mask != 0 && s->ev.empty())
        return fail(DZG_E_ARG, "kernel timing needs opts.profile != 0 at creation (it reserves the events)");
    s->opts.profile = mask;
    return 0;
}

extern "C" int dzg_solver_poll(dzg_solver *s, int32_t *status, int64_t *iterations)
{
    if (!s) return fail(DZG_E_ARG, "solver is NULL");
    HIP_OK(hipSetDevice(s->opts.device));
    TRY(read_ctl(s));
    HIP_OK(hipGetLastError());
    if (status) *status = s->h_ctl->status;
    if (iterations) *iterations = s->h_ctl->iter;
    return 0;
}

extern "C" int64_t dzg_shard_record_doubles(const dzg_solver *s) { return s ? s->d.xstride : 0; }

static void phase_stamp(dzg_solver *s, int cls, int end)
{
    if (prof_on(s, cls, s->prof_slot))
        hipEventRecord(s->ev[((size_t)s->prof_slot * DZG_K_COUNT + cls) * 2 + end], s->st);
}

extern "C" int dzg_shard_phase1(dzg_solver *s, double *send_dev)
{
    if (!s || !send_dev || s->numerics != DZG_NUMERICS_FAST) return fail(DZG_E_ARG, "phase1");
    phase_stamp(s, DZG_K_STATUS, 0);
    if (s->d.rs)
        dzg_launch_rs_propose(s->d, 0, 0, send_dev, s->st);
    else
        dzg_launch_shard_propose(s->d, 0, 0, send_dev, s->st);
    phase_stamp(s, DZG_K_STATUS, 1);
    return 0;
}

extern "C" int dzg_shard_phase2(dzg_solver *s, const double *recv_dev, double *send_dev)
{
    if (!s || !recv_dev || !send_dev || s->numerics != DZG_NUMERICS_FAST)
        return fail(DZG_E_ARG, "phase2");
    const DzgDev &d = s->d;
    hipStream_t st = s->st;
    const int pk = price_kernel_for(s);
    if (d.rs) {
        s->rs_recv1 = recv_dev;
        phase_stamp(s, DZG_K_FTRAN, 0);
        dzg_launch_rs_select(d, 0, recv_dev, st);
        dzg_launch_rs_gemv(d, DZG_STEP_PRIMAL, recv_dev, nullptr, st);
        phase_stamp(s, DZG_K_FTRAN, 1);
        phase_stamp(s, DZG_K_PRICE, 0);
        dzg_launch_price_fast(d, pk, st, DZG_STEP_DUAL);
        phase_stamp(s, DZG_K_PRICE, 1);
        phase_stamp(s, DZG_K_RATIO, 0);
        dzg_launch_rs_propose(d, 1, price_partials_for(s, pk), send_dev, st);
        phase_stamp(s, DZG_K_RATIO, 1);
        return 0;
    }
    phase_stamp(s, DZG_K_FTRAN, 0);
    if (s->batch_chain) {
        dzg_launch_chain_pre(d, s->chain_grid, s->chain_bar, s->chain_dbg, recv_dev, st);
    } else {
        dzg_launch_fast_select_prep(d, 4, 0, recv_dev, st);
        dzg_launch_fast_gemv(d, DZG_STEP_PRIMAL, recv_dev, st);
        dzg_launch_fast_btran(d, st);
    }
    phase_stamp(s, DZG_K_FTRAN, 1);
    phase_stamp(s, DZG_K_PRICE, 0);
    dzg_launch_price_fast(d, pk, st);
    phase_stamp(s, DZG_K_PRICE, 1);
    phase_stamp(s, DZG_K_RATIO, 0);
    dzg_launch_shard_propose(d, 1, price_partials_for(s, pk), send_dev, st);
    phase_stamp(s, DZG_K_RATIO, 1);
    return 0;
}

extern "C" int dzg_shard_phase3(dzg_solver *s, const double *recv_dev)
{
    if (!s || !recv_dev || s->numerics != DZG_NUMERICS_FAST) return fail(DZG_E_ARG, "phase3");
    const DzgDev &d = s->d;
    hipStream_t st = s->st;
    phase_stamp(s, DZG_K_UPDATE, 0);
    if (d.rs) {
        if (!s->rs_recv1) return fail(DZG_E_ARG, "phase3 before phase2");
        if (s->rs_recv1 == recv_dev)
            return fail(DZG_E_ARG, "shard_rows: phase 3 still reads the records of exchange 1 (the leaving "
                                   "row of a dual step, the entering column of a primal one): the second "
                                   "exchange needs a receive buffer of its own");
        dzg_launch_rs_select(d, 1, recv_dev, st);
        dzg_launch_price_fast(d, price_kernel_for(s), st, DZG_STEP_PRIMAL);
        dzg_launch_rs_gemv(d, DZG_STEP_DUAL, s->rs_recv1, recv_dev, st);
        dzg_launch_rs_books(d, s->rs_recv1, st);
        dzg_launch_fast_update(d, 0, st);
    } else if (s->batch_chain) {
        dzg_launch_chain_post(d, s->chain_grid, s->chain_bar, s->chain_dbg, 0, 0, recv_dev, st);
    } else {
        dzg_launch_fast_select_prep(d, 5, 0, recv_dev, st);
        dzg_launch_fast_gemv(d, DZG_STEP_DUAL, recv_dev, st);
        dzg_launch_fast_update(d, 0, st);
    }
    if (++s->since_flush >= DZG_RMAX) {
        dzg_launch_fast_flush(d, st);
        s->since_flush = 0;
    }
    phase_stamp(s, DZG_K_UPDATE, 1);
    return 0;
}

static void rs_batch_stride(dzg_solver *s, int k_bound)
{
    if (!s->d.rs) return;
    long long krow = ((long long)s->d.m + 2 + 15) / 16 * 16;
    if (k_bound > 0) {
        const long long need = ((long long)k_bound + 2 + 15) / 16 * 16;
        if (need < krow) krow = need;
    }
    s->d.xstride = DZG_RS_COL + s->d.rs_mcol + krow;
}

static int rs_gather_state(dzg_solver *s)
{
    if (!s->d.rs) return 0;
    Rccl &r = rccl();
    dzg_launch_rs_pack(s->d, s->rs_slice, s->rs_gsend, s->st);
    if (r.AllGather(s->rs_gsend, s->rs_grecv, (size_t)2 * s->rs_slice, kNcclFloat64, s->comm, s->st) != 0)
        return fail(DZG_E_DEVICE, "ncclAllGather (x, xbar of a row-sharded solve)");
    dzg_launch_rs_unpack(s->d, s->rs_slice, s->rs_grecv, s->st);
    HIP_OK(hipStreamSynchronize(s->st));
    return 0;
}

static void shard_comm_destroy(dzg_solver *s)
{
    if (s->comm && rccl().ok) rccl().CommDestroy(s->comm);
    s->comm = nullptr;
}

extern "C" void *dzg_solver_stream(dzg_solver *s) { return s ? (void *)s->st : nullptr; }

extern "C" int dzg_comm_unique_id(void *unique_id_128)
{
    if (!unique_id_128) return fail(DZG_E_ARG, "unique_id is NULL");
    Rccl &r = rccl();
    if (!r.ok) return fail(DZG_E_DEVICE, "librccl could not be loaded");
    NcclUniqueId id;
    const int rc = r.GetUniqueId(&id);
    if (rc != 0) return fail(DZG_E_DEVICE, std::string("ncclGetUniqueId: ") + (r.GetErrorString ? r.GetErrorString(rc) : "?"));
    std::memcpy(unique_id_128, &id, sizeof(id));
    return 0;
}

static int shard_buffers(dzg_solver *s)
{
    if (s->xsend) return 0;
    const size_t n = (size_t)(s->xstride_max ? s->xstride_max : s->d.xstride);
    if (s->d.rs) {
        TRY(dev_alloc(s, &s->rs_gsend, (size_t)2 * s->rs_slice));
        TRY(dev_alloc(s, &s->rs_grecv, (size_t)2 * s->rs_slice * (size_t)s->d.world));
    }
    TRY(dev_alloc(s, &s->xsend, n));
    TRY(dev_alloc(s, &s->xrecv1, n * (size_t)s->d.world));
    TRY(dev_alloc(s, &s->xrecv2, n * (size_t)s->d.world));
// ... 1741 lines not shown
    HIP_OK(hipMalloc(&dout, sizeof(double) * (size_t)(ncols ? ncols : 1)));
    HIP_OK(hipMalloc(&dcols, sizeof(int) * (size_t)(ncols ? ncols : 1)));
    HIP_OK(hipMemset(dA, 0, abytes));
    HIP_OK(hipMemset(dv, 0, sizeof(double) * ((size_t)m + 2)));
    if (n_struct > 0)
        HIP_OK(hipMemcpy2D(dA, sizeof(double) * ldd, a, sizeof(double) * lda, sizeof(double) * m,
                           n_struct, hipMemcpyHostToDevice));
    HIP_OK(hipMemcpy(dv, v, sizeof(double) * m, hipMemcpyHostToDevice));
    std::vector<int> c32((size_t)(ncols ? ncols : 1));
    for (int64_t k = 0; k < ncols; ++k) {
        if (cols[k] >= n_struct || cols[k] < -m) return fail(DZG_E_ARG, "cols out of range");
        c32[(size_t)k] = (int)cols[k];
    }
    HIP_OK(hipMemcpy(dcols, c32.data(), sizeof(int) * (size_t)(ncols ? ncols : 1), hipMemcpyHostToDevice));
    dzg_launch_price_raw(kernel, (int)m, ldd, dA, dcols, (int)ncols, dv, dout, 0);
    HIP_OK(hipDeviceSynchronize());
    HIP_OK(hipGetLastError());
    if (ncols > 0) HIP_OK(hipMemcpy(out, dout, sizeof(double) * ncols, hipMemcpyDeviceToHost));
    hipFree(dA); hipFree(dv); hipFree(dout); hipFree(dcols);
    return 0;
}

extern "C" int dzg_kernel_neg_t_dot_csc(int64_t m, int64_t n_struct, const int64_t *col_ptr,
                                        const int32_t *row_idx, const double *val,
                                        const int64_t *cols, int64_t ncols, const double *v,
                                        double *out, int32_t device)
{
    if (m <= 0 || n_struct < 0 || ncols < 0 || !v || !out || (ncols > 0 && !cols) || !col_ptr ||
        col_ptr[0] != 0 || (n_struct > 0 && col_ptr[n_struct] > 0 && (!row_idx || !val)))
        return fail(DZG_E_ARG, "bad argument");
    if (dzg_device_count() <= 0) return fail(DZG_E_DEVICE, "no HIP device visible");
    HIP_OK(hipSetDevice(device));
    const size_t nnz = (size_t)col_ptr[n_struct];
    for (int64_t j = 0; j < n_struct; ++j)
        for (int64_t e = col_ptr[j]; e < col_ptr[j + 1]; ++e)
            if (row_idx[e] < 0 || row_idx[e] >= m) return fail(DZG_E_ARG, "row_idx out of range");
    std::vector<long long> cp((size_t)n_struct + 1);
    for (int64_t j = 0; j <= n_struct; ++j) cp[(size_t)j] = col_ptr[j];
    std::vector<int> c32((size_t)(ncols ? ncols : 1));
    for (int64_t k = 0; k < ncols; ++k) {
        if (cols[k] >= n_struct || cols[k] < -m) return fail(DZG_E_ARG, "cols out of range");
        c32[(size_t)k] = (int)cols[k];
    }
    long long *dcp; int *dri, *dcols; double *dcv, *dv, *dout;
    HIP_OK(hipMalloc(&dcp, sizeof(long long) * cp.size()));
    HIP_OK(hipMalloc(&dri, sizeof(int) * (nnz + 1)));
    HIP_OK(hipMalloc(&dcv, sizeof(double) * (nnz + 1)));
    HIP_OK(hipMalloc(&dv, sizeof(double) * ((size_t)m + 2)));
    HIP_OK(hipMalloc(&dout, sizeof(double) * c32.size()));
    HIP_OK(hipMalloc(&dcols, sizeof(int) * c32.size()));
    HIP_OK(hipMemcpy(dcp, cp.data(), sizeof(long long) * cp.size(), hipMemcpyHostToDevice));
    if (nnz) {
        HIP_OK(hipMemcpy(dri, row_idx, sizeof(int) * nnz, hipMemcpyHostToDevice));
        HIP_OK(hipMemcpy(dcv, val, sizeof(double) * nnz, hipMemcpyHostToDevice));
    }
    HIP_OK(hipMemset(dv, 0, sizeof(double) * ((size_t)m + 2)));
    HIP_OK(hipMemcpy(dv, v, sizeof(double) * m, hipMemcpyHostToDevice));
    HIP_OK(hipMemcpy(dcols, c32.data(), sizeof(int) * c32.size(), hipMemcpyHostToDevice));
    dzg_launch_price_csc_raw(dcp, dri, dcv, dcols, (int)ncols, dv, dout, 0);
    HIP_OK(hipDeviceSynchronize());
    HIP_OK(hipGetLastError());
    if (ncols > 0) HIP_OK(hipMemcpy(out, dout, sizeof(double) * ncols, hipMemcpyDeviceToHost));
    hipFree(dcp); hipFree(dri); hipFree(dcv); hipFree(dv); hipFree(dout); hipFree(dcols);
    return 0;
}

extern "C" int dzg_kernel_first_pivot(int64_t len, const double *y, const double *ybar,
                                      int64_t *pos_out, int32_t device)
{
    if (len < 0 || !pos_out) return fail(DZG_E_ARG, "bad argument");
    if (dzg_device_count() <= 0) return fail(DZG_E_DEVICE, "no HIP device visible");
    HIP_OK(hipSetDevice(device));
    return dzg_run_first_pivot(len, y, ybar, pos_out);
}

extern "C" int dzg_kernel_second_pivot(int64_t len, double mu, const double *y, const double *ybar,
                                       const double *dy, int64_t *pos_out, int32_t device)
{
    if (len < 0 || !pos_out) return fail(DZG_E_ARG, "bad argument");
    if (dzg_device_count() <= 0) return fail(DZG_E_DEVICE, "no HIP device visible");
    HIP_OK(hipSetDevice(device));
    return dzg_run_second_pivot(len, mu, y, ybar, dy, pos_out);
}
```

dantzig_amd/csrc/k_chain.hip:

```cpp
#include <chrono>
#include "common.h"
#include "fast_decide.h"
#include "fast_rows.h"

#include "chain_barrier.h"


#define CH_NW (CH_THREADS / 64)
#define CH_MAXP 16

template <bool NARROW>
__device__ __forceinline__ bool chain_wide(int k)
{
    if constexpr (NARROW)
        return false;
    else
        return k > 512;
}
template <bool NOFOLD>
__device__ __forceinline__ int chain_fold_on(int fold)
{
    if constexpr (NOFOLD)
        return 0;
    else
        return fold;
}
template <bool NOFOLD>
__device__ __forceinline__ bool chain_one_wave(int nrz)
{
    if constexpr (NOFOLD)
        return true;
    else
        return nrz <= 256;
}

__device__ __forceinline__ void chain_rows(int m, int &r0, int &r1)
{
    const int per = ((m + (int)gridDim.x - 1) / (int)gridDim.x + 3) & ~3;
    r0 = (int)blockIdx.x * per;
    if (r0 > m) r0 = m;
    r1 = r0 + per < m ? r0 + per : m;
}

__device__ __forceinline__ void chain_cols(int q, int &q0, int &q1)
{
    const int per = (q + (int)gridDim.x - 1) / (int)gridDim.x;
    q0 = (int)blockIdx.x * per;
    if (q0 > q) q0 = q;
    q1 = q0 + per < q ? q0 + per : q;
}

__device__ __forceinline__ DzgCand2 chain_wave_best2(DzgCand2 c)
{
    return dzg_wave_best2_flat<64>(c);
}
__device__ __forceinline__ DzgCand2 chain_block_best2(DzgCand2 c)
{
    static_assert(CH_THREADS == 512, "eight wave results: one half row");
    return dzg_block_best2_flat<8>(c, true);
}

struct ChainSpec {
    double r[4], h[4];
    int k[4];
};
__device__ __forceinline__ void chain_spec_load(ChainSpec &s, const double *__restrict__ pr,
                                                const int *__restrict__ pk,
                                                const double *__restrict__ ph, int lane)
{
#pragma unroll
    for (int j = 0; j < 4; ++j) {
        s.r[j] = pr[lane + 64 * j];
        s.k[j] = pk[lane + 64 * j];
        s.h[j] = ph[lane + 64 * j];
    }
}
__device__ __forceinline__ DzgCand2 chain_spec_reduce(const ChainSpec &s, int count, int lane);
__device__ __forceinline__ void chain_spec_pin(const ChainStamps &ts, ChainSpec &s)
{
    if (ts.on)
        asm volatile("" : "+v"(s.r[0]), "+v"(s.r[1]), "+v"(s.r[2]), "+v"(s.r[3]), "+v"(s.k[0]), "+v"(s.k[1]),
                          "+v"(s.k[2]), "+v"(s.k[3]), "+v"(s.h[0]), "+v"(s.h[1]), "+v"(s.h[2]), "+v"(s.h[3]));
}
__device__ __forceinline__ void chain_spec_load_sc1(ChainSpec &s, const double *pr, const int *pk,
                                                    const double *ph, int lane)
{
// ... 122 lines not shown
    }
    int turn = CH_BETA_WAVE;
    for (int item = blockIdx.x; item < 4 * neta; item += gridDim.x) {
        if (wave == turn) chain_beta_item(d, item, code, a);
        turn = turn + 1 < CH_NW ? turn + 1 : 0;
    }
}
__device__ __forceinline__ void chain_beta_published()
{
    __builtin_amdgcn_s_waitcnt(0);
}
__device__ __forceinline__ void chain_beta_fetch(const DzgDev &d, int neta, int code, double *s_beta)
{
    const int tid = threadIdx.x;
    if (tid < 4 * R_) {
        const double s0 = tid < 4 * neta ? ld_sc1(d.beta_part + tid) : 0.0;
        const double s1 = __shfl_down(s0, 1, DZG_WAVE);
        const double s2 = __shfl_down(s0, 2, DZG_WAVE);
        const double s3 = __shfl_down(s0, 3, DZG_WAVE);
        const int t = tid >> 2;
        if ((tid & 3) == 0) s_beta[t] = t < neta ? (code < 0 ? s0 : fast_beta_fold(s0, s1, s2, s3)) : 0.0;
    }
}

template <int LPR, int MAXP>
__device__ __forceinline__ void chain_dot_head(const DzgDev &d, int r0, int r1, int k,
                                               const double *s_ag, double (&accs)[MAXP])
{
    constexpr int RPW = 64 / LPR;
    const int lane = threadIdx.x & 63, wave = threadIdx.x >> 6;
    const int sub = lane % LPR, grp = lane / LPR;
    const int k2 = (k + 1) & ~1;
    const int variant = d.ftran_variant >= 0 ? d.ftran_variant : (k >= d.ftran_nt_k ? 2 : 0);
    if (LPR == 64 && variant == 1) {
#pragma unroll
        for (int pass = 0; pass < MAXP; ++pass) {
            const int i = r0 + (pass * CH_NW + wave) * RPW + grp;
            accs[pass] = fast_gemv_row_head<LPR, 1>(i < r1 ? i : d.m, d.m, k2, d.binv, d.ldb, s_ag, sub);
        }
        return;
    }
    if (LPR == 64 && variant == 2) {
#pragma unroll
        for (int pass = 0; pass < MAXP; ++pass) {
            const int i = r0 + (pass * CH_NW + wave) * RPW + grp;
            accs[pass] = fast_gemv_row_head<LPR, 2>(i < r1 ? i : d.m, d.m, k2, d.binv, d.ldb, s_ag, sub);
        }
        return;
    }
#pragma unroll
    for (int pass = 0; pass < MAXP; ++pass) {
        const int i = r0 + (pass * CH_NW + wave) * RPW + grp;
        accs[pass] = fast_gemv_row_head<LPR>(i < r1 ? i : d.m, d.m, k2, d.binv, d.ldb, s_ag, sub);
    }
}

template <int LPR, int MAXP>
__device__ __forceinline__ void chain_dot_tail(const DzgDev &d, int r0, int r1, int k, int neta,
                                               const double *s_ag, const double *s_beta,
                                               const double (&accs)[MAXP], double *s_dx)
{
    constexpr int RPW = 64 / LPR;
    const int lane = threadIdx.x & 63, wave = threadIdx.x >> 6;
    const int sub = lane % LPR, grp = lane / LPR;
    const int k2 = (k + 1) & ~1;
    const int npass = (r1 - r0 + CH_NW * RPW - 1) / (CH_NW * RPW);
#pragma unroll
    for (int pass = 0; pass < MAXP; ++pass) {
        if (pass < npass) {
            const int i = r0 + (pass * CH_NW + wave) * RPW + grp;
            const int ii = i < r1 ? i : d.m;
            const double acc = fast_gemv_row_tail<LPR>(accs[pass], ii, d.m, neta, d.U, d.ldw, s_beta, sub);
            if (ii < d.m && sub == 0) s_dx[i - r0] = acc;
        }
    }
    for (int pass = MAXP; pass < npass; ++pass) {
        const int i = r0 + (pass * CH_NW + wave) * RPW + grp;
        const int ii = i < r1 ? i : d.m;
        const double acc = fast_gemv_row<LPR>(ii, d.m, k2, neta, d.binv, d.ldb, s_ag, d.U, d.ldw, s_beta, sub);
        if (ii < d.m && sub == 0) s_dx[i - r0] = acc;
    }
}

template <bool SHARD, int MAXP, bool NARROW>
__global__ __launch_bounds__(CH_THREADS) void k_chain_pre(const DzgDev d, unsigned long long *bar,
                                                          unsigned long long *dbg,
                                                          const double *__restrict__ xrecv)
{
    __shared__ double s_ag[CH_AGCAP];
    __shared__ double s_beta[R_], s_dx[CH_THREADS], s_up[R_];
    __shared__ ChainSlots s_c;
    ChainStamps ts;
    ts.start(dbg);
    DzgCtl *ctl = d.ctl;
    const int tid = threadIdx.x, lane = tid & 63, wave = tid >> 6;
    const int m = d.m, nwg = (int)gridDim.x;
    const bool lead = blockIdx.x == 0 && tid == 0;
    ChainSpec sp;
    if (wave == 0 && !SHARD)
        chain_spec_load(sp, d.fpz_r, d.fpz_k, d.fpz_h, lane);
    else if (wave == 1)
        chain_spec_load(sp, d.fpx_r, d.fpx_k, d.fpx_h, lane);
    DzgCand2 cj_rec = dzg_cand2_none();
    int w_rec = -1;
    if (SHARD) w_rec = shard_merge(xrecv, d.xstride, d.world, cj_rec);
    int r0, r1;
    chain_rows(m, r0, r1);
    const int row = r0 + tid;
    const bool has_row = row < r1;
    int dslot_i = -1, bcode_i = 0;
    double x_i = 0.0, xbar_i = 0.0;
    if (has_row) {
        dslot_i = d.dslot[row];
        bcode_i = d.bcode[row];
        x_i = d.x[row];
        xbar_i = d.xbar[row];
    }
    DzgCtl c = *ctl;
    if (c.status != DZG_RUNNING) return;
    unsigned long long gen = c.bar_gen;
    const int neta = c.neta, k = c.ncompact;
    const int dr0 = tid < k ? d.drow[tid] : -1;
    const int dr1 = tid + CH_THREADS < k ? d.drow[tid + CH_THREADS] : -1;
    if (wave < 2 && !(SHARD && wave == 0)) {
        chain_spec_pin(ts, sp);
        const unsigned long long t_site = ts.now();
        DzgCand2 w = chain_spec_reduce(sp, c.fp_count, lane);
        ts.pin(w);
        ts.site(DZG_SITE_PRE_FIRST, t_site);
        if (lane == 0) chain_put(s_c, wave, w);
    }
    __syncthreads();
    const DzgCand2 cj = SHARD ? cj_rec : chain_get(s_c, 0), ci = chain_get(s_c, 1);
    int kind;
    double mu;
    const unsigned long long t_status = ts.now();
    if (!fast_status(ctl, c, lead, cj, ci, d.eps, m, SHARD, kind, &mu)) return;
    ts.pin(mu);
    ts.site(DZG_SITE_PRE_STATUS, t_status);
    const int slot = kind == DZG_STEP_PRIMAL ? 0 : 1;
    ts.mark(slot);
    if (k > CH_AGCAP || c.fp_count > 256 || (NARROW && k > 512)) {
        if (lead) ctl->status = DZG_PANIC;
        return;
    }
    if (lead) {
        ctl->neta_cur = neta;
        ctl->k_cur = k;
    }
    int p;
    if (kind == DZG_STEP_PRIMAL) {
        const int epos = cj.k;
        const int code = d.nbcode[epos];
        double zr = 0.0, zbr = 0.0;
        if (lead) {
            zr = d.z[epos];
            zbr = d.zbar[epos];
        }
        const double *a = chain_col<SHARD>(d, code, xrecv, w_rec);
        const bool has_unit = has_row && bcode_i < 0;
        double unit_i = 0.0;
        if (has_unit) unit_i = code >= 0 ? a[-1 - bcode_i] : (code == bcode_i ? 1.0 : 0.0);
        int edslot = -1;
        if (lead && code < 0) edslot = d.dslot[-1 - code];
        chain_stage_ag(s_ag, k, code, a, d.drow, dr0, dr1);
        chain_beta(d, neta, code, a);
        ts.mark(slot);
        if (lead) {
            ctl->enter_code = code;
            ctl->zr = zr;
            ctl->zbar_r = zbr;
            ctl->enter_dslot = edslot;
            if (SHARD) ctl->enter_src = w_rec;
        }
        __syncthreads();
        double accs[MAXP];
        if (chain_wide<NARROW>(k))
            chain_dot_head<64>(d, r0, r1, k, s_ag, accs);
        else
            chain_dot_head<16>(d, r0, r1, k, s_ag, accs);
        chain_beta_published();
        ts.mark(slot);
        if (!chain_barrier(ctl, bar, gen)) return;
        ts.mark(slot);
        chain_beta_fetch(d, neta, code, s_beta);
        __syncthreads();
        if (chain_wide<NARROW>(k))
            chain_dot_tail<64>(d, r0, r1, k, neta, s_ag, s_beta, accs, s_dx);
        else
            chain_dot_tail<16>(d, r0, r1, k, neta, s_ag, s_beta, accs, s_dx);
        __syncthreads();
        DzgCand2 best = dzg_cand2_none();
        if (has_row) {
            double dxi = s_dx[tid];
            if (has_unit) dxi += unit_i;
            d.dx[row] = dxi;
            const double scaled = mu * xbar_i;
            const double den = x_i + scaled;
            DzgCand2 cnd;
            cnd.r = dzg_div(dxi, den);
            cnd.k = row;
            cnd.h = -__builtin_inf();
            if (cnd.r > 0.0) best = dzg_better2(best, cnd);
            if (dzg_noise_zero(den, x_i, scaled, c.tau)) best.h = __builtin_inf();
        }
        ts.pin(best);
        const unsigned long long t_rowbest = ts.now();
        best = chain_best(best, r1 - r0);
        ts.pin(best);
        ts.site(DZG_SITE_PRE_ROWBEST, t_rowbest);
        if (tid == 0) {
            st_sc1(d.rx_r + blockIdx.x, best.r);
            st_sc1(d.rx_k + blockIdx.x, best.k);
            st_sc1(d.rx_h + blockIdx.x, best.h);
        }
        ts.mark(slot);
        if (!chain_barrier(ctl, bar, gen)) return;
        ts.mark(slot);
        const unsigned long long t_sc1 = ts.now();
        if (wave == 0) {
            const DzgCand2 w = chain_reduce_sc1(d.rx_r, d.rx_k, d.rx_h, nwg, lane);
            if (lane == 0) chain_put(s_c, 0, w);
        }
        __syncthreads();
        DzgCand2 cw = chain_get(s_c, 0);
        ts.pin(cw);
        ts.site(DZG_SITE_PRE_SC1, t_sc1);
        if (!fast_ratio_outcome(ctl, c, lead, cw, DZG_UNBOUNDED)) {
            if (lead) ctl->bar_gen = gen;
            return;
        }
        p = cw.k;
        if (lead) ctl->leave_pos = p;
        ts.mark(slot);
    } else {
        p = ci.k;
    }
    const int lcode = d.bcode[p];
    double xp = 0.0, xbp = 0.0;
    if (lead) {
        xp = d.x[p];
        xbp = d.xbar[p];
    }
    double up = 0.0, base = 0.0, w[R_];
    if (tid < R_ && tid < neta) up = d.U[(long long)tid * d.ldw + p];
    if (has_row) {
        if (dslot_i >= 0) base = d.binv[(long long)p * d.ldb + dslot_i];
        fast_btran_eta_load(w, neta, d.W, d.ldw, row);
    }
    if (tid < R_) s_up[tid] = up;
    __syncthreads();
    if (has_row) {
        if (dslot_i < 0) base = lcode == -1 - row ? 1.0 : 0.0;
        const double vr = base - fast_btran_eta_fma(w, neta, s_up);
        d.v[row] = vr;
        if (dslot_i >= 0 && d.vc) d.vc[dslot_i] = vr;
    }
    if (lead) {
        ctl->xp = xp;
        ctl->xbp = xbp;
        ctl->leave_code = lcode;
        if (gen != c.bar_gen) ctl->bar_gen = gen;
    }
    ts.mark(slot);
    ts.done(slot);
}

__device__ __forceinline__ double chain_fold_dz(const DzgDev &d, int code, int G)
{
    if (code < 0) {
        const double p = 1.0 * -d.v[-1 - code];
        return 0.0 + p;
    }
    const double *src = d.ppart + (code - d.col0);
    double sum = 0.0;
    int gg = 0;
    for (; gg + 8 <= G; gg += 8) {
        double t[8];
#pragma unroll
        for (int e = 0; e < 8; ++e) t[e] = src[(long long)(gg + e) * d.ldt];
#pragma unroll
        for (int e = 0; e < 8; ++e) sum = sum + t[e];
    }
    for (; gg < G; ++gg) sum = sum + src[(long long)gg * d.ldt];
    return -sum;
}

template <bool SHARD, int MAXP, bool NARROW, bool NOFOLD>
__global__ __launch_bounds__(CH_THREADS) void k_chain_post(const DzgDev d, unsigned long long *bar,
                                                           const DzgPivotArgs pa, int only_partials,
                                                           int nrz, unsigned long long *dbg,
                                                           const double *__restrict__ xrecv, int fold_arg)
{
    const int fold = chain_fold_on<NOFOLD>(fold_arg);
    __shared__ double s_ag[CH_AGCAP];
    __shared__ double s_beta[R_], s_dx[CH_THREADS];
    __shared__ double s_dxp;
    __shared__ ChainSlots s_c;
    ChainStamps ts;
    ts.start(only_partials ? nullptr : dbg);
    const unsigned long long t_books = (dbg && !only_partials && blockIdx.x == 0 && threadIdx.x == CH_THREADS - 64)
                                           ? __builtin_amdgcn_s_memrealtime()
                                           : 0ull;
    int slot = 2;
    DzgCtl *ctl = d.ctl;
    const int tid = threadIdx.x, lane = tid & 63, wave = tid >> 6;
    const int m = d.m, q = d.q;
    const bool lead = blockIdx.x == 0 && tid == 0;
    DzgCand2 mine = dzg_cand2_none();
    ChainSpec sp;
    const bool one_wave = chain_one_wave<NOFOLD>(nrz);
    if (SHARD || fold) {
    } else if (!only_partials && one_wave) {
        if (wave == 0) chain_spec_load(sp, d.rz_r, d.rz_k, d.rz_h, lane);
    } else if (!only_partials) {
#pragma unroll
        for (int j = 0; j < 4; ++j) {
            const int i = tid + CH_THREADS * j;
            DzgCand2 o;
            o.r = d.rz_r[i];
            o.k = d.rz_k[i];
            o.h = d.rz_h[i];
            if (i < nrz) mine = dzg_better2(mine, o);
        }
        for (int i = tid + 4 * CH_THREADS; i < nrz; i += CH_THREADS) {
            DzgCand2 o;
            o.r = d.rz_r[i];
            o.k = d.rz_k[i];
            o.h = d.rz_h[i];
            mine = dzg_better2(mine, o);
        }
    }
    int r0, r1, q0, q1;
    chain_rows(m, r0, r1);
    chain_cols(q, q0, q1);
    const int row = r0 + tid, col = q0 + tid;
    const bool has_row = row < r1, has_col = col < q1;
    double x_i = 0.0, xbar_i = 0.0, v_i = 0.0, dx_i = 0.0, z_k = 0.0, zbar_k = 0.0, dz_k = 0.0;
    int bcode_i = 0, nbcode_k = -1;
    if (has_row) {
        x_i = d.x[row];
        xbar_i = d.xbar[row];
        if (!only_partials) {
            v_i = d.v[row];
            dx_i = d.dx[row];
            bcode_i = d.bcode[row];
        }
    }
// ... 154 lines not shown
                }
            } else {
                chain_dot_tail<16>(d, r0, r1, k, neta, s_ag, s_beta, accs, s_dx);
                if (wave == CH_NW - 1) {
                    const double acc = fast_gemv_row_tail<16>(accp, lane < 16 ? p : m, m, neta, d.U, d.ldw,
                                                              s_beta, lane % 16);
                    if (lane == 0) s_dxp = ci < 0 ? acc + unit_p : acc;
                }
            }
            __syncthreads();
            dxp = s_dxp;
            if (has_row) {
                dx_i = s_dx[tid];
                if (has_unit) dx_i += unit_i;
                d.dx[row] = dx_i;
            }
            ts.mark(slot);
        } else {
            r = c.enter_pos;
            cj = c.enter_code;
            zr = c.zr;
            zbr = c.zbar_r;
            dzr = (!SHARD && fold) ? chain_fold_dz(d, cj, G) : d.dz[r];
            if (SHARD) {
                int w_rec = -1;
                for (int rk = 0; rk < d.world && w_rec < 0; ++rk)
                    if ((int)xrecv[(long long)rk * d.xstride + 1] == r) w_rec = rk;
                if (w_rec < 0) {
                    if (lead) ctl->status = DZG_PANIC;
                    return;
                }
                const double *rec = xrecv + (long long)w_rec * d.xstride;
                zr = rec[2];
                zbr = rec[3];
                dzr = rec[4];
                if (lead) {
                    ctl->zr = zr;
                    ctl->zbar_r = zbr;
                    ctl->dz_r = dzr;
                    ctl->use_record = 1;
                }
            }
            edslot = c.enter_dslot;
            dxp = d.dx[p];
            ts.mark(slot);
        }
        const DzgPivotScalars ps = fast_pivot_scalars(xp, xbp, dxp, zr, zbr, dzr, neta, c.max_pivot_err);
        const bool appended = ci < 0, deleted = cj < 0;
        new_code_r = ci;
        if (blockIdx.x == 0 && wave == CH_NW - 1) {
            c.neta = neta;
            c.ncompact = k;
            fast_pivot_books_s(ctl, c, pa, ps, 1);
            if (t_books && kind == DZG_STEP_DUAL && lane == 0) {
                __builtin_amdgcn_s_waitcnt(0);
                dbg[16 * DZG_SITE_SLOT + DZG_SITE_BOOKS] += __builtin_amdgcn_s_memrealtime() - t_books;
                dbg[16 * (DZG_SITE_SLOT + 1) + DZG_SITE_BOOKS] += 1;
            }
        }
        if (!ps.ok) {
            if (lead && gen != c.bar_gen) ctl->bar_gen = gen;
            return;
        }
        if (deleted) {
            del_last = k + (appended ? 1 : 0) - 1;
            del_ce = edslot;
        }
        if (appended) app_col = k;
        if (lead && gen != c.bar_gen) ctl->bar_gen = gen;
        t = ps.t;
        s = ps.s;
        tbar = ps.tbar;
        sbar = ps.sbar;
        teta = neta;
        wzero = cj < 0 ? -1 - cj : -1;
        rdxp = 1.0 / dxp;
        if (c.tie_tol >= 0.0) {
            double adaptive = 64.0 * ps.max_err;
            if (c.drift_tau > adaptive) adaptive = c.drift_tau;
            tau = adaptive > c.tie_tol ? adaptive : c.tie_tol;
        }
        ts.mark(slot);
    }
    DzgCand2 bx = dzg_cand2_none(), bz = dzg_cand2_none();
    if (has_row) {
        double xi = x_i, xb = xbar_i;
        if (!only_partials) {
            const double a = t * dx_i, b = tbar * dx_i;
            xi = (row == p) ? t : xi - a;
            xb = (row == p) ? tbar : xb - b;
            d.x[row] = xi;
            d.xbar[row] = xb;
            d.U[(long long)teta * d.ldw + row] = (row == p ? dx_i - 1.0 : dx_i) * rdxp;
            d.W[(long long)teta * d.ldw + row] = (row == wzero) ? 0.0 : v_i;
            double *brow = d.binv + (long long)row * d.ldb;
            if (del_last >= 0) {
                const double last_val = (app_col == del_last) ? (row == p ? 1.0 : 0.0) : brow[del_last];
                if (del_ce != del_last) brow[del_ce] = last_val;
                brow[del_last] = 0.0;
            } else if (app_col >= 0 && row == p) {
                brow[app_col] = 1.0;
            }
        }
        dzg_first_pivot_entry(bx, xi, xb, row, tau);
    }
    if (has_col) {
        double zk = z_k, zb = zbar_k;
        if (!only_partials) {
            const double a = s * dz_k, b = sbar * dz_k;
            zk = (col == r) ? s : zk - a;
            zb = (col == r) ? sbar : zb - b;
            d.z[col] = zk;
            d.zbar[col] = zb;
        }
        bool mine = true;
        if (SHARD) {
            const int code = (!only_partials && col == r) ? new_code_r : nbcode_k;
            mine = code < 0 || (code >= d.col0 && code < d.col1);
        }
        if (mine) dzg_first_pivot_entry(bz, zk, zb, col, tau);
    }
    ts.pin(bx);
    ts.pin(bz);
    const unsigned long long t_best = ts.now();
    chain_best_pair(bx, r1 - r0, bz, q1 - q0);
    ts.pin(bx);
    ts.pin(bz);
    ts.site(DZG_SITE_POST_BX, t_best);
    if (tid == 0) {
        d.fpx_r[blockIdx.x] = bx.r;
        d.fpx_k[blockIdx.x] = bx.k;
        d.fpx_h[blockIdx.x] = bx.h;
        d.fpz_r[blockIdx.x] = bz.r;
        d.fpz_k[blockIdx.x] = bz.k;
        d.fpz_h[blockIdx.x] = bz.h;
        if (blockIdx.x == 0) ctl->fp_count = (int)gridDim.x;
    }
    ts.mark(slot);
    if (slot == 3) ts.since_start(DZG_SITE_POST_END);
    ts.done(slot);
}

static_assert(CH_BAR_WORDS == DZG_CHAIN_BAR_WORDS, "barrier counter block");

static int chain_pick(int m, int grid, int k_bound, int fold, int nrz, int shard, int post)
{
    if (shard || grid < 1 || m < 0 || k_bound <= 0) return DZG_CHAIN_GENERIC;
    const int per = ((m + grid - 1) / grid + 3) & ~3;
    const bool narrow = k_bound <= 512;
    const int rows_per_pass = CH_NW * (narrow ? 64 / 16 : 64 / 64);
    const int need = (per + rows_per_pass - 1) / rows_per_pass;
    const bool nofold = fold == 0 && nrz <= 256;
    if (narrow) {
        if (need <= 1 && (!post || nofold)) return DZG_CHAIN_P1_NARROW;
        if (need <= 4) return DZG_CHAIN_P4_NARROW;
        return DZG_CHAIN_GENERIC;
    }
    return need <= 4 ? DZG_CHAIN_P4_WIDE : DZG_CHAIN_GENERIC;
}

extern "C" int dzg_debug_chain_instance(int32_t m, int32_t grid, int32_t k_bound, int32_t fold, int32_t nrz,
                                        int32_t shard, int32_t post)
{
    switch (chain_pick(m, grid, k_bound, fold, nrz, shard, post)) {
    case DZG_CHAIN_P1_NARROW: return 1 | 0x100 | (post ? 0x200 : 0);
    case DZG_CHAIN_P4_NARROW: return 4 | 0x100;
    case DZG_CHAIN_P4_WIDE: return 4;
    default: return CH_MAXP;
    }
}

int dzg_chain_resident_per_cu(void)
{
    const void *kernels[] = {
        reinterpret_cast<const void *>(k_chain_pre<false, CH_MAXP, false>),
        reinterpret_cast<const void *>(k_chain_pre<true, CH_MAXP, false>),
        reinterpret_cast<const void *>(k_chain_pre<false, 1, true>),
        reinterpret_cast<const void *>(k_chain_pre<false, 4, true>),
        reinterpret_cast<const void *>(k_chain_pre<false, 4, false>),
        reinterpret_cast<const void *>(k_chain_post<false, CH_MAXP, false, false>),
        reinterpret_cast<const void *>(k_chain_post<true, CH_MAXP, false, false>),
        reinterpret_cast<const void *>(k_chain_post<false, 1, true, true>),
        reinterpret_cast<const void *>(k_chain_post<false, 4, true, false>),
        reinterpret_cast<const void *>(k_chain_post<false, 4, false, false>),
    };
    int least = 1 << 20, n = 0;
    for (const void *kern : kernels) {
        if (hipOccupancyMaxActiveBlocksPerMultiprocessor(&n, kern, CH_THREADS, 0) != hipSuccess) return 0;
        least = n < least ? n : least;
    }
    return least;
}

void dzg_launch_chain_pre(const DzgDev &d, int grid, unsigned long long *bar,
                          unsigned long long *dbg, const double *xrecv, hipStream_t st, int instances)
{
    const int which = instances ? chain_pick(d.m, grid, d.k_hint, 0, 0, xrecv != nullptr, 0) : DZG_CHAIN_GENERIC;
    if (xrecv)
        hipLaunchKernelGGL((k_chain_pre<true, CH_MAXP, false>), dim3(grid), dim3(CH_THREADS), 0, st, d, bar, dbg, xrecv);
    else if (which == DZG_CHAIN_P1_NARROW)
        hipLaunchKernelGGL((k_chain_pre<false, 1, true>), dim3(grid), dim3(CH_THREADS), 0, st, d, bar, dbg, xrecv);
    else if (which == DZG_CHAIN_P4_NARROW)
        hipLaunchKernelGGL((k_chain_pre<false, 4, true>), dim3(grid), dim3(CH_THREADS), 0, st, d, bar, dbg, xrecv);
    else if (which == DZG_CHAIN_P4_WIDE)
        hipLaunchKernelGGL((k_chain_pre<false, 4, false>), dim3(grid), dim3(CH_THREADS), 0, st, d, bar, dbg, xrecv);
    else
        hipLaunchKernelGGL((k_chain_pre<false, CH_MAXP, false>), dim3(grid), dim3(CH_THREADS), 0, st, d, bar, dbg, xrecv);
}

void dzg_launch_chain_post(const DzgDev &d, int grid, unsigned long long *bar,
                           unsigned long long *dbg, int only_partials, int nrz, const double *xrecv,
                           hipStream_t st, int fold, int price_small, int instances)
{
    DzgPivotArgs pa = dzg_pivot_args(d);
    pa.price_small = price_small;
    const int which = instances ? chain_pick(d.m, grid, d.k_hint, fold, nrz, xrecv != nullptr, 1) : DZG_CHAIN_GENERIC;
    if (xrecv)
        hipLaunchKernelGGL((k_chain_post<true, CH_MAXP, false, false>), dim3(grid), dim3(CH_THREADS), 0, st, d, bar,
                           pa, only_partials, nrz, dbg, xrecv, 0);
    else if (which == DZG_CHAIN_P1_NARROW)
        hipLaunchKernelGGL((k_chain_post<false, 1, true, true>), dim3(grid), dim3(CH_THREADS), 0, st, d, bar,
                           pa, only_partials, nrz, dbg, xrecv, fold);
    else if (which == DZG_CHAIN_P4_NARROW)
        hipLaunchKernelGGL((k_chain_post<false, 4, true, false>), dim3(grid), dim3(CH_THREADS), 0, st, d, bar,
                           pa, only_partials, nrz, dbg, xrecv, fold);
    else if (which == DZG_CHAIN_P4_WIDE)
        hipLaunchKernelGGL((k_chain_post<false, 4, false, false>), dim3(grid), dim3(CH_THREADS), 0, st, d, bar,
                           pa, only_partials, nrz, dbg, xrecv, fold);
    else
        hipLaunchKernelGGL((k_chain_post<false, CH_MAXP, false, false>), dim3(grid), dim3(CH_THREADS), 0, st, d, bar,
                           pa, only_partials, nrz, dbg, xrecv, fold);
}

__global__ __launch_bounds__(64) void k_debug_hold(unsigned long long ticks, int *sink, int *started)
{
    extern __shared__ double s_hold[];
    s_hold[threadIdx.x] = 1.0;
    if (threadIdx.x == 0) __hip_atomic_fetch_add(started, 1, __ATOMIC_RELAXED, __HIP_MEMORY_SCOPE_SYSTEM);
    const unsigned long long t0 = __builtin_amdgcn_s_memrealtime();
    unsigned long long spins = 0;
    while (__builtin_amdgcn_s_memrealtime() - t0 < ticks && spins < (1ull << 34)) {
        __builtin_amdgcn_s_sleep(64);
        ++spins;
    }
    if (s_hold[threadIdx.x] == 2.0) *sink = 1;
}

static hipStream_t g_hold_stream = nullptr;
static int *g_hold_sink = nullptr;
static int *g_hold_started = nullptr;

extern "C" int dzg_debug_hold_cus(int32_t device, int32_t workgroups, double seconds)
{
    if (workgroups < 1 || workgroups > 256 || !(seconds > 0.0) || seconds > 30.0) return DZG_E_ARG;
    if (hipSetDevice(device) != hipSuccess) return DZG_E_DEVICE;
    const int lds = 128 * 1024;
    if (hipFuncSetAttribute(reinterpret_cast<const void *>(k_debug_hold),
                            hipFuncAttributeMaxDynamicSharedMemorySize, lds) != hipSuccess)
        return DZG_E_DEVICE;
    if (!g_hold_stream && hipStreamCreateWithFlags(&g_hold_stream, hipStreamNonBlocking) != hipSuccess)
        return DZG_E_DEVICE;
    if (!g_hold_sink && hipMalloc(&g_hold_sink, sizeof(int)) != hipSuccess) return DZG_E_NOMEM;
    if (!g_hold_started && hipHostMalloc(&g_hold_started, sizeof(int), hipHostMallocCoherent) != hipSuccess)
        return DZG_E_NOMEM;
    *(volatile int *)g_hold_started = 0;
    hipLaunchKernelGGL(k_debug_hold, dim3(workgroups), dim3(64), lds, g_hold_stream,
                       (unsigned long long)(seconds * 1e8), g_hold_sink, g_hold_started);
    if (hipGetLastError() != hipSuccess) return DZG_E_DEVICE;
    const auto t0 = std::chrono::steady_clock::now();
    while (*(volatile int *)g_hold_started < workgroups) {
        if (std::chrono::duration<double>(std::chrono::steady_clock::now() - t0).count() > 2.0) return DZG_E_DEVICE;
    }
    return 0;
}

extern "C" int dzg_debug_hold_wait(void)
{
    if (!g_hold_stream) return 0;
    return hipStreamSynchronize(g_hold_stream) == hipSuccess ? 0 : DZG_E_DEVICE;
}
// ... 75 lines not shown
```

dantzig_amd/csrc/k_fast.hip:

```cpp
#include <cstdlib>

#include "common.h"
#include "fast_decide.h"
#include "fast_rows.h"

template <int MODE>
__global__ __launch_bounds__(256) void k_fast_select_prep(
    DzgCtl *ctl, int m, const double *__restrict__ A, long long lda, int col0,
    const double *__restrict__ xrecv, long long xstride,
    const int *__restrict__ nbcode,
    const double *__restrict__ fpx_r, const int *__restrict__ fpx_k,
    const double *__restrict__ fpx_h, const double *__restrict__ fpz_r,
    const int *__restrict__ fpz_k, const double *__restrict__ fpz_h,
    const double *__restrict__ rz_r, const int *__restrict__ rz_k,
    const double *__restrict__ rz_h, int nrz, const double *__restrict__ W, long long ldw,
    const int *__restrict__ drow, double *__restrict__ ag, double *__restrict__ beta, double eps,
    int world)
{
    DzgCtl c = *ctl;
    if (c.status != DZG_RUNNING) return;
    const bool lead = blockIdx.x == 0 && threadIdx.x == 0;
    int epos;
    int code_known = 0, code_val = -1;
    if (MODE == 0 || MODE == 4) {
// ... 220 lines not shown
                                                     int col1, int sharded, double *fpx_r,
                                                     int *fpx_k, double *fpx_h, double *fpz_r,
                                                     int *fpz_k, double *fpz_h,
                                                     const double *__restrict__ v,
                                                     double *__restrict__ U, long long ldu,
                                                     double *__restrict__ W, long long ldw,
                                                     double *__restrict__ binv, long long ldb,
                                                     int r0, int r1, int rowshard)
{
    const DzgCtl c = *ctl;
    if (c.status != DZG_RUNNING) return;
    const int p = c.leave_pos, r = c.enter_pos;
    if (!only_partials && c.del_last >= 0) {
        const int ce = c.del_ce, last = c.del_last;
        for (int i = r0 + blockIdx.x * blockDim.x + threadIdx.x; i < r1; i += gridDim.x * blockDim.x) {
            double *row = binv + (long long)i * ldb;
            if (ce != last) row[ce] = row[last];
            row[last] = 0.0;
        }
    }
    const int neta_new = only_partials ? c.neta : c.neta_next;
    if (!only_partials && blockIdx.x == 0 && threadIdx.x == 0) {
        ctl->neta = c.neta_next;
        ctl->ncompact = c.ncompact_next;
    }
    if (blockIdx.x == 0 && threadIdx.x == 0) ctl->fp_count = (int)gridDim.x;
    const int teta = neta_new - 1;
    const int wzero = c.enter_code < 0 ? -1 - c.enter_code : -1;
    const double rdxp = only_partials ? 0.0 : 1.0 / (rowshard ? c.dxp : dx[p]);
    double *ut = U + (long long)(teta < 0 ? 0 : teta) * ldu;
    double *wt = W + (long long)(teta < 0 ? 0 : teta) * ldw;
    const double t = c.t, s = c.s, tbar = c.tbar, sbar = c.sbar;
    const int stride = gridDim.x * blockDim.x;
    const double tau = c.tau;
    DzgCand2 bx = dzg_cand2_none(), bz = dzg_cand2_none();
    if (!only_partials && rowshard)
        for (int i = blockIdx.x * blockDim.x + threadIdx.x; i < m; i += stride)
            if (i < r0 || i >= r1) wt[i] = (i == wzero) ? 0.0 : v[i];
    for (int i = r0 + blockIdx.x * blockDim.x + threadIdx.x; i < r1; i += stride) {
        double xi = x[i], xb = xbar[i];
        if (!only_partials) {
            const double d = dx[i];
            const double a = t * d, b = tbar * d;
            xi = (i == p) ? t : xi - a;
            xb = (i == p) ? tbar : xb - b;
            x[i] = xi;
            xbar[i] = xb;
            ut[i] = (i == p ? d - 1.0 : d) * rdxp;
            wt[i] = (i == wzero) ? 0.0 : v[i];
        }
        dzg_first_pivot_entry(bx, xi, xb, i, tau);
    }
    for (int k = blockIdx.x * blockDim.x + threadIdx.x; k < q; k += stride) {
        double zk = z[k], zb = zbar[k];
        if (!only_partials) {
            const double d = dz[k];
            const double a = s * d, b = sbar * d;
            zk = (k == r) ? s : zk - a;
            zb = (k == r) ? sbar : zb - b;
            z[k] = zk;
            zbar[k] = zb;
        }
        bool mine = true;
        if (sharded) {
            const int code = nbcode[k];
            mine = code < 0 || (code >= col0 && code < col1);
        }
        if (mine) dzg_first_pivot_entry(bz, zk, zb, k, tau);
    }
    bx = dzg_block_best2(bx);
    bz = dzg_block_best2(bz);
    if (threadIdx.x == 0) {
        fpx_r[blockIdx.x] = bx.r;
        fpx_k[blockIdx.x] = bx.k;
        fpx_h[blockIdx.x] = bx.h;
        fpz_r[blockIdx.x] = bz.r;
        fpz_k[blockIdx.x] = bz.k;
        fpz_h[blockIdx.x] = bz.h;
    }
}

__global__ __launch_bounds__(256) void k_fast_gather_w(const DzgCtl *ctl, const double *__restrict__ W,
                                                       long long ldw, const int *__restrict__ drow,
                                                       double *__restrict__ Wc)
{
    if (ctl->neta < R_) return;
    const int k = ctl->ncompact, neta = ctl->neta;
    const int t = blockIdx.y;
    const int c = blockIdx.x * blockDim.x + threadIdx.x;
    const int kpad = (k + 15) & ~15;
    if (c >= kpad) return;
    Wc[(long long)t * ldw + c] = (t < neta && c < k) ? W[(long long)t * ldw + drow[c]] : 0.0;
}

template <bool PRELOAD>
__global__ __launch_bounds__(256) void k_fast_flush_mfma(const DzgCtl *ctl, int m,
                                                         double *__restrict__ binv, long long ldb,
                                                         const double *__restrict__ U, long long ldu,
                                                         const double *__restrict__ Wc,
                                                         long long ldw)
{
    const int neta = ctl->neta, k = ctl->ncompact;
    if (neta < R_ || k <= 0) return;
    const int lane = threadIdx.x & 63, wave = threadIdx.x >> 6;
    const int c0 = blockIdx.x * 64;
    const int i0 = (blockIdx.y * 4 + wave) * 16;
    if (c0 >= k || i0 >= m) return;
    const int li = lane & 15, lk = lane >> 4;
    double4_t acc[4];
#pragma unroll
    for (int j = 0; j < 4; ++j) {
#pragma unroll
        for (int g = 0; g < 4; ++g) {
            const int row = i0 + lk + 4 * g, col = c0 + 16 * j + li;
            acc[j][g] = (row < m && col < k) ? binv[(long long)row * ldb + col] : 0.0;
        }
    }
    const int arow = i0 + li;
    const int arowc = arow < m ? arow : 0;
    if (PRELOAD) {
        double av[R_ / 4], bv[R_ / 4][4];
#pragma unroll
        for (int s = 0; s < R_ / 4; ++s) {
            const int t = 4 * s + lk;
            av[s] = U[(long long)t * ldu + arowc];
            const double *wrow = Wc + (long long)t * ldw + c0 + li;
#pragma unroll
            for (int j = 0; j < 4; ++j) bv[s][j] = wrow[16 * j];
        }
#pragma unroll
        for (int s = 0; s < R_ / 4; ++s) {
            const double a = arow < m ? -av[s] : 0.0;
#pragma unroll
            for (int j = 0; j < 4; ++j)
                acc[j] = __builtin_amdgcn_mfma_f64_16x16x4f64(a, bv[s][j], acc[j], 0, 0, 0);
        }
    } else {
        for (int s = 0; s < R_ / 4; ++s) {
            const int t = 4 * s + lk;
            const double a = arow < m ? -U[(long long)t * ldu + arowc] : 0.0;
            const double *wrow = Wc + (long long)t * ldw + c0 + li;
#pragma unroll
            for (int j = 0; j < 4; ++j) {
                const double b = wrow[16 * j];
                acc[j] = __builtin_amdgcn_mfma_f64_16x16x4f64(a, b, acc[j], 0, 0, 0);
            }
        }
    }
#pragma unroll
    for (int j = 0; j < 4; ++j) {
#pragma unroll
        for (int g = 0; g < 4; ++g) {
            const int row = i0 + lk + 4 * g, col = c0 + 16 * j + li;
            if (row < m && col < k) binv[(long long)row * ldb + col] = acc[j][g];
        }
    }
}

#define FLD 72
__global__ __launch_bounds__(256) void k_fast_flush_mfma_lds(const DzgCtl *ctl, int m,
                                                             double *__restrict__ binv, long long ldb,
                                                             const double *__restrict__ U, long long ldu,
                                                             const double *__restrict__ Wc, long long ldw)
{
    __shared__ double s_w[R_ * FLD];
    const int neta = ctl->neta, k = ctl->ncompact;
    if (neta < R_ || k <= 0) return;
    const int lane = threadIdx.x & 63, wave = threadIdx.x >> 6;
    const int c0 = blockIdx.x * 64;
// ... 164 lines not shown
}

__global__ __launch_bounds__(256) void k_fast_init_partials(double *r, int *k, double *h, int n)
{
    const int i = blockIdx.x * blockDim.x + threadIdx.x;
    if (i < n) {
        r[i] = 0.0;
        k[i] = -1;
        h[i] = -__builtin_inf();
    }
}

void dzg_launch_fast_init(const DzgDev &d, hipStream_t st)
{
    {
        const int np = 4096;
        double *rs[4] = {d.fpx_r, d.fpz_r, d.rx_r, d.rz_r}, *hs[4] = {d.fpx_h, d.fpz_h, d.rx_h, d.rz_h};
        int *ks[4] = {d.fpx_k, d.fpz_k, d.rx_k, d.rz_k};
        for (int a = 0; a < 4; ++a)
            hipLaunchKernelGGL(k_fast_init_partials, dim3(np / 256), dim3(256), 0, st, rs[a], ks[a], hs[a], np);
    }
    {
        const int r0 = d.rs ? d.rs_r0 : 0, rows = (d.rs ? d.rs_r1 : d.m) - r0;
        if (rows > 0)
            hipMemsetAsync(d.binv + (long long)r0 * d.ldb, 0, sizeof(double) * (size_t)rows * (size_t)d.ldb, st);
    }
    hipMemsetAsync(d.U, 0, sizeof(double) * (size_t)d.ldw * R_, st);
    hipMemsetAsync(d.W, 0, sizeof(double) * (size_t)d.ldw * R_, st);
    hipMemsetAsync(d.Wc, 0, sizeof(double) * (size_t)d.ldw * R_, st);
    hipMemsetAsync(d.ag, 0, sizeof(double) * ((size_t)d.m + 2), st);
    hipLaunchKernelGGL(k_fast_init, dim3(1), dim3(256), 0, st, d.ctl, d.m, d.q, d.dslot, d.nonbasis,
                       d.var_col, d.plist, d.pslot, d.col0, d.col1, d.csc ? d.cptr : nullptr, d.drow,
                       d.basis, d.bcode, d.nbcode, d.pcode, d.cpos);
}

void dzg_launch_fast_select_prep(const DzgDev &d, int mode, int nrz, const double *xrecv,
                                 hipStream_t st)
{
#define SEL_ARGS d.ctl, d.m, d.A, d.lda, d.col0, xrecv, d.xstride, d.nbcode,                            \
                       d.fpx_r, d.fpx_k, d.fpx_h, d.fpz_r, d.fpz_k, d.fpz_h, d.rz_r, d.rz_k, d.rz_h, nrz,  \
                       d.W, d.ldw, d.drow, d.ag, d.beta, d.eps, d.world
    const dim3 grid(R_ + 1), block(256);
    switch (mode) {
    case 0: hipLaunchKernelGGL((k_fast_select_prep<0>), grid, block, 0, st, SEL_ARGS); break;
    case 1: hipLaunchKernelGGL((k_fast_select_prep<1>), grid, block, 0, st, SEL_ARGS); break;
    case 4: hipLaunchKernelGGL((k_fast_select_prep<4>), grid, block, 0, st, SEL_ARGS); break;
    default: hipLaunchKernelGGL((k_fast_select_prep<5>), grid, block, 0, st, SEL_ARGS); break;
    }
#undef SEL_ARGS
}

void dzg_launch_fast_gemv(const DzgDev &d, int need_kind, const double *xrecv, hipStream_t st)
{
    const DzgPivotArgs pa = dzg_pivot_args(d);
#define GEMV_ARGS d.ctl, need_kind, d.m, d.binv, d.ldb, d.ag, d.U, d.ldw, d.beta, d.A, d.lda, d.col0, xrecv,  \
                  d.xstride, d.bcode, d.x, d.xbar, d.dx, d.rx_r, d.rx_k, d.rx_h, pa,                         \
                  (d.ftran_variant >= 0 ? (d.ftran_variant ? 0 : 0x7fffffff) : d.ftran_nt_k)
    if (need_kind == DZG_STEP_DUAL)
        hipLaunchKernelGGL((k_fast_gemv<true>), dim3(DZG_NB_GEMV), dim3(256), 0, st, GEMV_ARGS);
    else
        hipLaunchKernelGGL((k_fast_gemv<false>), dim3(DZG_NB_GEMV), dim3(256), 0, st, GEMV_ARGS);
#undef GEMV_ARGS
}

void dzg_launch_fast_btran(const DzgDev &d, hipStream_t st)
{
    hipLaunchKernelGGL(k_fast_btran, dim3((d.m + 255) / 256), dim3(256), 0, st, d.ctl, d.m, d.binv,
                       d.ldb, d.dslot, d.bcode, d.U, d.ldw, d.W, d.ldw, d.rx_r, d.rx_k, d.rx_h,
                       d.v, d.vc);
}

void dzg_launch_fast_update(const DzgDev &d, int only_partials, hipStream_t st)
{
    hipLaunchKernelGGL(k_fast_update, dim3(DZG_NB_UPD), dim3(256), 0, st, d.ctl, only_partials, d.x,
                       d.xbar, d.z, d.zbar, d.dx, d.dz, d.m, d.q, d.nbcode, d.col0, d.col1,
                       d.world > 1 ? 1 : 0, d.fpx_r, d.fpx_k, d.fpx_h, d.fpz_r, d.fpz_k, d.fpz_h, d.v, d.U,
                       d.ldw, d.W, d.ldw, d.binv, d.ldb, d.rs ? d.rs_r0 : 0, d.rs ? d.rs_r1 : d.m, d.rs);
}

void dzg_launch_fast_flush(const DzgDev &d, hipStream_t st)
{
    const int kmax = d.k_hint > 0 && d.k_hint < d.m ? d.k_hint : d.m;
    hipLaunchKernelGGL(k_fast_gather_w, dim3((kmax + 15 + 255) / 256, R_), dim3(256), 0, st, d.ctl,
                       d.W, d.ldw, d.drow, d.Wc);
    const int r0 = d.rs ? d.rs_r0 : 0, rows = (d.rs ? d.rs_r1 : d.m) - r0;
    double *binv = d.binv + (long long)r0 * d.ldb;
    const double *U = d.U + r0;
    static const bool steps = std::getenv("DZG_FLUSH_STEPS") != nullptr;
    static const bool no_lds = std::getenv("DZG_FLUSH_NO_LDS") != nullptr;
    if (rows <= 0) {
    } else if (!steps && !no_lds)
        hipLaunchKernelGGL(k_fast_flush_mfma_lds, dim3((kmax + 63) / 64, (rows + 63) / 64), dim3(256), 0, st,
                           d.ctl, rows, binv, d.ldb, U, d.ldw, d.Wc, d.ldw);
    else if (steps)
        hipLaunchKernelGGL(k_fast_flush_mfma<false>, dim3((kmax + 63) / 64, (rows + 63) / 64), dim3(256), 0, st,
                           d.ctl, rows, binv, d.ldb, U, d.ldw, d.Wc, d.ldw);
    else
        hipLaunchKernelGGL(k_fast_flush_mfma<true>, dim3((kmax + 63) / 64, (rows + 63) / 64), dim3(256), 0, st,
                           d.ctl, rows, binv, d.ldb, U, d.ldw, d.Wc, d.ldw);
    hipLaunchKernelGGL(k_fast_flush_done, dim3(1), dim3(1), 0, st, d.ctl, ((kmax + 63) / 64) * 64);
}

void dzg_launch_shard_propose(const DzgDev &d, int mode, int nrz, double *xsend, hipStream_t st)
{
    const int hdr_only = d.xstride <= 8;
    const dim3 grid(hdr_only ? 1 : 1 + (d.m + 255) / 256);
    if (mode == 0)
        hipLaunchKernelGGL((k_shard_propose<0>), grid, dim3(256), 0, st, d.ctl, d.m, d.A, d.lda,
                           d.col0, d.col1, d.nbcode, d.z, d.zbar, d.dz, d.fpz_r,
                           d.fpz_k, d.fpz_h, DZG_NB_UPD, xsend, d.csc, hdr_only);
    else
        hipLaunchKernelGGL((k_shard_propose<1>), grid, dim3(256), 0, st, d.ctl, d.m, d.A, d.lda,
                           d.col0, d.col1, d.nbcode, d.z, d.zbar, d.dz, d.rz_r, d.rz_k,
                           d.rz_h, nrz, xsend, d.csc, hdr_only);
    if (d.csc)
        hipLaunchKernelGGL(k_shard_scatter_col, dim3(1), dim3(256), 0, st, d.ctl, mode, d.cptr,
                           d.ridx, d.cval, d.col0, d.col1, xsend);
}

__global__ __launch_bounds__(256) void k_lockstep_allgather(double *const *ptrs, int world, int which,
                                                            long long xstride)
{
    const int pair = blockIdx.y, dst = pair / world, src = pair % world;
    const double *from = ptrs[src];
    double *to = ptrs[(long long)which * world + dst] + (long long)src * xstride;
    for (long long i = blockIdx.x * blockDim.x + threadIdx.x; i < xstride; i += (long long)gridDim.x * blockDim.x)
        to[i] = from[i];
}

void dzg_launch_lockstep_allgather(double *const *ptrs, int world, int which, long long xstride,
                                   hipStream_t st)
{
    int bx = (int)((xstride + 255) / 256);
    if (bx > 64) bx = 64;
    hipLaunchKernelGGL(k_lockstep_allgather, dim3(bx, world * world), dim3(256), 0, st, ptrs, world,
                       which, xstride);
}
```

dantzig_amd/csrc/k_price_kernels.h:

```cpp
#pragma once
#include "common.h"

typedef double double2_t __attribute__((ext_vector_type(2)));

__device__ __forceinline__ int price_code(const int *__restrict__ nonbasis,
                                          const int *__restrict__ var_col, int pos)
{
    const int v = nonbasis[pos];
    return var_col ? var_col[v] : v;
}

__device__ __forceinline__ void price_candidate(DzgCand2 &best, double dzk, int pos, double mu,
                                                double tau, const double *__restrict__ z,
                                                const double *__restrict__ zbar)
{
    const double zk = z[pos], scaled = mu * zbar[pos];
    const double den = zk + scaled;
    DzgCand2 c;
    c.r = dzg_div(dzk, den);
    c.k = pos;
    c.h = -__builtin_inf();
    if (c.r > 0.0) best = dzg_better2(best, c);
    if (dzg_noise_zero(den, zk, scaled, tau)) best.h = __builtin_inf();
}

__device__ __forceinline__ void price_candidate_v(DzgCand2 &best, double dzk, int pos, double mu,
                                                  double tau, double zk, double zbk)
{
    const double scaled = mu * zbk;
    const double den = zk + scaled;
    DzgCand2 c;
    c.r = dzg_div(dzk, den);
    c.k = pos;
    c.h = -__builtin_inf();
    if (c.r > 0.0) best = dzg_better2(best, c);
    if (dzg_noise_zero(den, zk, scaled, tau)) best.h = __builtin_inf();
}

__device__ __forceinline__ void price_slack_positions(DzgCand2 &best, int q,
                                                      const int *__restrict__ nonbasis,
                                                      const int *__restrict__ var_col,
                                                      const double *__restrict__ v,
                                                      double *__restrict__ dz, double mu,
                                                      double tau, const double *__restrict__ z,
                                                      const double *__restrict__ zbar)
{
    const int nthreads = gridDim.x * blockDim.x;
    for (int pos = blockIdx.x * blockDim.x + threadIdx.x; pos < q; pos += nthreads) {
        const int code = price_code(nonbasis, var_col, pos);
        if (code < 0) {
            const double p = 1.0 * -v[-1 - code];
            const double d = 0.0 + p;
            dz[pos] = d;
            if (z) price_candidate(best, d, pos, mu, tau, z, zbar);
        }
    }
}

__device__ __forceinline__ void price_publish(DzgCand2 best, double *__restrict__ rz_r,
                                              int *__restrict__ rz_k, double *__restrict__ rz_h)
{
    best = dzg_block_best2(best);
    if (rz_r && threadIdx.x == 0) {
        rz_r[blockIdx.x] = best.r;
        rz_k[blockIdx.x] = best.k;
        rz_h[blockIdx.x] = best.h;
    }
}

__device__ __forceinline__ void price_publish_small(DzgCand2 best, double *__restrict__ rz_r,
                                                    int *__restrict__ rz_k, double *__restrict__ rz_h)
{
    best = dzg_block_best2_flat<8>(best, false);
    if (rz_r && threadIdx.x == 0) {
        rz_r[blockIdx.x] = best.r;
        rz_k[blockIdx.x] = best.k;
        rz_h[blockIdx.x] = best.h;
    }
}

template <int CW, int DEPTH = 2, int DBG = 0, bool NT = true>
__global__ __launch_bounds__(256) void k_price_seq2(
    const DzgCtl *ctl, const double *__restrict__ A, long long lda, int m, int q,
    const int *__restrict__ plist, const int *__restrict__ nonbasis,
    const int *__restrict__ var_col, const double *__restrict__ v, double *__restrict__ dz,
    const double *__restrict__ z, const double *__restrict__ zbar, double *__restrict__ rz_r,
    int *__restrict__ rz_k, double *__restrict__ rz_h, int col0 = 0)
{
    constexpr int TR = 128, PAD = 2;
    __shared__ __attribute__((aligned(16))) double tile[4][CW][TR + PAD];
    if (ctl && ctl->status != DZG_RUNNING) return;
    const int lane = threadIdx.x & 63, wave = threadIdx.x >> 6;
    const int nw = gridDim.x * 4;
    const int wg = blockIdx.x * 4 + wave;
    const double mu = ctl ? ctl->mu : 0.0, tau = ctl ? ctl->tau : 0.0;
    DzgCand2 best = dzg_cand2_none();
    price_slack_positions(best, q, nonbasis, var_col, v, dz, mu, tau, z, zbar);

    const int count = plist ? (int)ctl->nb_struct : q;
    const int base = count / nw, rem = count % nw;
    const int start = wg * base + (wg < rem ? wg : rem);
    const int cnt = base + (wg < rem ? 1 : 0);
    const int ntiles = (m + TR - 1) / TR;
    double(*mytile)[TR + PAD] = tile[wave];

    for (int c0 = 0; c0 < cnt; c0 += CW) {
        const int nc = (cnt - c0) < CW ? (cnt - c0) : CW;
        int mypos = -1, mycode = -1;
        if (lane < nc) {
            const int idx = start + c0 + lane;
            mypos = plist ? plist[idx] : idx;
            mycode = price_code(nonbasis, var_col, mypos);
        }
        int lastcode = col0;
#pragma unroll
        for (int l = 0; l < CW; ++l) {
            const int code_l = __builtin_amdgcn_readlane(mycode, l);
            if (code_l >= 0) lastcode = code_l;
        }
        long long off[CW];
#pragma unroll
        for (int l = 0; l < CW; ++l) {
            const int code_l = __builtin_amdgcn_readlane(mycode, l);
            off[l] = (long long)((code_l >= 0 ? code_l : lastcode) - col0) * lda;
        }
        double2_t rg[DEPTH][CW], vg[DEPTH];
        double dbg_sink = 0.0;
        long long cyc_park = 0, cyc_fetch = 0, cyc_walk = 0;
        const int lastpair = (int)lda - 2;
        const int lastv = ((m + 1) & ~1) - 2 >= 0 ? ((m + 1) & ~1) - 2 : 0;

        auto fetch = [&](int t, double2_t(&reg)[CW], double2_t &vreg) {
            const int row = t * TR + 2 * lane;
            const int rowc = row < lda ? row : lastpair;
#pragma unroll
            for (int l = 0; l < CW; ++l) {
                const double2_t *gp = reinterpret_cast<const double2_t *>(A + off[l] + rowc);
                reg[l] = NT ? __builtin_nontemporal_load(gp) : *gp;
            }
            vreg = *reinterpret_cast<const double2_t *>(v + (row < m ? row : lastv));
        };
        auto park = [&](int t, const double2_t(&reg)[CW], const double2_t &vreg) {
            if (DBG == 2) {
#pragma unroll
                for (int l = 0; l < CW; ++l) dbg_sink += reg[l].x + reg[l].y;
                return;
            }
            const int row = t * TR + 2 * lane;
            const bool inside = row < lda && row < m + 1;
            const double nv0 = -vreg.x, nv1 = -vreg.y;
            const double2_t zero = {0.0, 0.0};
            __builtin_amdgcn_wave_barrier();
#pragma unroll
            for (int l = 0; l < CW; ++l) {
                double2_t pr;
                pr.x = reg[l].x != 0.0 ? reg[l].x * nv0 : 0.0;
// ... 466 lines not shown
    const int spos = blockIdx.x * blockDim.x + threadIdx.x;
    const int sub = threadIdx.x & (RL_LPC - 1);
    const int group = spos / RL_LPC;
    const int ngroups = nthreads / RL_LPC;
    int scode = 0, pos0 = -1, code0 = -1;
    if (spos < q) scode = nbcode[spos];
    if (group < q) {
        pos0 = plist[group];
        code0 = pcode[group];
    }
    const int status = ctl->status, count = (int)ctl->nb_struct;
    const double mu = ctl->mu, tau = ctl->tau;
    if (status != DZG_RUNNING) return;
    DzgCand2 best = dzg_cand2_none();
    double sv = 0.0, sz = 0.0, szb = 0.0;
    if (scode < 0) {
        sv = v[-1 - scode];
        sz = z[spos];
        szb = zbar[spos];
    }
    unsigned int walked = 0;
    for (int idx0 = 0; idx0 < count; idx0 += ngroups) {
        const int idx = idx0 + group;
        int pos = -1, code = -1;
        long long e0 = 0, e1 = 0;
        if (idx < count) {
            pos = idx0 == 0 ? pos0 : plist[idx];
            code = idx0 == 0 ? code0 : pcode[idx];
            if (code >= 0) {
                e0 = cptr[code];
                e1 = e0 + lcnt[code];
            }
        }
        double zc = 0.0, zbc = 0.0;
        if (code >= 0 && sub == 0) {
            zc = z[pos];
            zbc = zbar[pos];
            walked += (unsigned int)(e1 - e0);
        }
        double a0 = 0.0, a1 = 0.0;
        long long e = e0 + sub;
        for (; e + RL_LPC < e1; e += 2 * RL_LPC) {
            const DzgLiveEntry n0 = lent[e], n1 = lent[e + RL_LPC];
            a0 = fma(n0.val, v[n0.row], a0);
            a1 = fma(n1.val, v[n1.row], a1);
        }
        if (e < e1) {
            const DzgLiveEntry n0 = lent[e];
            a0 = fma(n0.val, v[n0.row], a0);
        }
        double acc = a0 + a1;
#pragma unroll
        for (int off = RL_LPC / 2; off > 0; off >>= 1) acc += __shfl_xor(acc, off, DZG_WAVE);
        if (code >= 0 && sub == 0) {
            dz[pos] = -acc;
            price_candidate_v(best, -acc, pos, mu, tau, zc, zbc);
        }
    }
    if (scode < 0) {
        const double p = 1.0 * -sv;
        const double d = 0.0 + p;
        dz[spos] = d;
        price_candidate_v(best, d, spos, mu, tau, sz, szb);
    }
    for (int pos = spos + nthreads; pos < q; pos += nthreads) {
        const int code = nbcode[pos];
        if (code < 0) {
            const double p = 1.0 * -v[-1 - code];
            const double d = 0.0 + p;
            dz[pos] = d;
            price_candidate(best, d, pos, mu, tau, z, zbar);
        }
    }
#pragma unroll
    for (int off = 32; off > 0; off >>= 1) walked += __shfl_xor(walked, off, DZG_WAVE);
    if ((threadIdx.x & 63) == 0) s_work[threadIdx.x >> 6] = walked;
    price_publish(best, rz_r, rz_k, rz_h);
    if (threadIdx.x == 0)
        __hip_atomic_fetch_add(work + blockIdx.x,
                               (unsigned long long)s_work[0] + s_work[1] + s_work[2] + s_work[3],
                               __ATOMIC_RELAXED, __HIP_MEMORY_SCOPE_AGENT);
}

#define PR_GMAX DZG_PR_GMAX
#define PR_BATCH DZG_PR_BATCH
#define PR_PIPE 8
template <int VEC, int PIPE = PR_PIPE>
__global__ __launch_bounds__(256) void k_price_rows(
    const DzgCtl *ctl, int rows_T, const double *__restrict__ At, long long ldt,
    const int *__restrict__ drow, const int *__restrict__ bcode, const double *__restrict__ vc,
    double *__restrict__ part, int need_kind = -1)
{
    typedef double vec_t __attribute__((ext_vector_type(2)));
    __shared__ long long s_off[256];
    __shared__ double s_coef[256];
    const int status = ctl->status, k = ctl->ncompact, lp = ctl->leave_pos;
    if (status != DZG_RUNNING || k >= rows_T) return;
    if (need_kind >= 0 && ctl->kind != need_kind) return;
    int G = (k + 1 + PR_BATCH - 1) / PR_BATCH;
    G = G > (int)gridDim.y ? (int)gridDim.y : G;
    const int g = blockIdx.y;
    if (g >= G) return;
    const int lcode = lp >= 0 ? bcode[lp] : 0;
    const int nrows = k + (lcode < 0 ? 1 : 0);
    const long long j0 = ((long long)blockIdx.x * 256 + threadIdx.x) * VEC;
    const bool live = j0 < ldt;
    const double *col = At + (live ? j0 : 0);
    double acc[VEC];
#pragma unroll
    for (int e = 0; e < VEC; ++e) acc[e] = 0.0;
    for (int cbase = g; cbase < nrows; cbase += 256 * G) {
        __syncthreads();
        const int c = cbase + (int)threadIdx.x * G;
        if (c < nrows) {
            const int row = c < k ? drow[c] : -1 - lcode;
            s_off[threadIdx.x] = (long long)row * ldt;
            s_coef[threadIdx.x] = c < k ? vc[c] : 1.0;
        }
        __syncthreads();
        const int left = (nrows - cbase + G - 1) / G;
        const int n = left < 256 ? left : 256;
        const int bfull = n / PIPE;
        vec_t ra[PIPE][VEC / 2], rb[PIPE][VEC / 2];
#define PR_LOAD(B, REG)                                                                              \
    _Pragma("unroll") for (int u = 0; u < PIPE; ++u) {                                            \
        const double *src = col + s_off[(B) * PIPE + u];                                          \
        _Pragma("unroll") for (int h = 0; h < VEC / 2; ++h)                                          \
            REG[u][h] = __builtin_nontemporal_load(reinterpret_cast<const vec_t *>(src) + h);        \
    }
#define PR_FMA(B, REG)                                                                               \
    _Pragma("unroll") for (int u = 0; u < PIPE; ++u) {                                            \
        const double cf = s_coef[(B) * PIPE + u];                                                 \
        _Pragma("unroll") for (int h = 0; h < VEC / 2; ++h) {                                        \
            acc[2 * h] = fma(cf, REG[u][h].x, acc[2 * h]);                                           \
            acc[2 * h + 1] = fma(cf, REG[u][h].y, acc[2 * h + 1]);                                   \
        }                                                                                            \
    }
        int bi = 0;
        if (bfull > 0) { PR_LOAD(0, ra) }
        while (bi + 2 < bfull) {
            PR_LOAD(bi + 1, rb)
            PR_FMA(bi, ra)
            PR_LOAD(bi + 2, ra)
            PR_FMA(bi + 1, rb)
            bi += 2;
        }
        if (bfull - bi == 2) {
            PR_LOAD(bi + 1, rb)
            PR_FMA(bi, ra)
            PR_FMA(bi + 1, rb)
        } else if (bfull - bi == 1) {
            PR_FMA(bi, ra)
        }
#undef PR_LOAD
#undef PR_FMA
        {
            const int i0 = bfull * PIPE;
#pragma unroll
            for (int u = 0; u < PIPE; ++u)
                if (i0 + u < n) {
                    const double *src = col + s_off[i0 + u];
#pragma unroll
                    for (int h = 0; h < VEC / 2; ++h)
                        ra[u][h] = __builtin_nontemporal_load(reinterpret_cast<const vec_t *>(src) + h);
                }
#pragma unroll
            for (int u = 0; u < PIPE; ++u)
                if (i0 + u < n) {
                    const double cf = s_coef[i0 + u];
#pragma unroll
                    for (int h = 0; h < VEC / 2; ++h) {
                        acc[2 * h] = fma(cf, ra[u][h].x, acc[2 * h]);
                        acc[2 * h + 1] = fma(cf, ra[u][h].y, acc[2 * h + 1]);
                    }
                }
        }
    }
    if (live) {
        double *dst = part + (long long)g * ldt + j0;
#pragma unroll
        for (int e = 0; e < VEC; ++e) dst[e] = acc[e];
    }
}

#define PRS_TILE 64
#define PRS_ROWS 512
#define PRS_STAMP_SLOT 4
template <int VEC, int NG, int RPT>
__global__ __launch_bounds__(512, (RPT < PR_BATCH ? 8 : 2)) void k_price_rows_small(
    DzgCtl *__restrict__ ctl, int rows_T, const double *__restrict__ At, long long ldt, int ncols,
    const int *__restrict__ drow, const double *__restrict__ vc, int m,
    const int *__restrict__ cpos, int q, const int *__restrict__ nbcode, const double *__restrict__ v,
    double *__restrict__ dz, const double *__restrict__ z, const double *__restrict__ zbar,
    double *__restrict__ rz_r, int *__restrict__ rz_k, double *__restrict__ rz_h,
    unsigned long long *dbg)
{
    constexpr int LPG = 64 / VEC;
    constexpr int NS = 512 / LPG;
    static_assert(VEC == 1 || VEC == 2, "8- or 16-byte loads");
    static_assert(PR_BATCH % RPT == 0 && PR_GMAX * PR_BATCH >= PRS_ROWS, "a group has at most PR_BATCH rows");
    __shared__ long long s_off[PRS_ROWS];
    __shared__ double s_coef[PRS_ROWS];
    __shared__ __attribute__((aligned(16))) double s_part[PR_GMAX][PRS_TILE];
    ChainStamps ts;
    ts.start(dbg);
    const int tid = threadIdx.x, lane = tid & 63, wave = tid >> 6;
    const int spos = blockIdx.x * 512 + tid;
    int scode = 0;
    if (spos < q) scode = nbcode[spos];
    const long long j = (long long)blockIdx.x * PRS_TILE + lane;
    int pos = -1;
    if (wave == 0 && j < ncols) pos = cpos[j];
    const int li = tid < m ? tid : m - 1;
    const int lrow = drow[li];
    const double lcf = vc[li];
    const int status = ctl->status, k = ctl->ncompact, lp = ctl->leave_pos;
    const int lcode_c = ctl->leave_code;
    const double mu = ctl->mu, tau = ctl->tau;
    asm volatile("" ::"s"(status), "s"(k), "s"(lp), "s"(lcode_c), "s"(mu), "s"(tau));
    if (status != DZG_RUNNING) return;
    if (k >= rows_T || k >= PRS_ROWS) {
        if (blockIdx.x == 0 && tid == 0) ctl->status = DZG_PANIC;
        return;
    }
    ts.mark(PRS_STAMP_SLOT);
    const int lcode = lp >= 0 ? lcode_c : 0;
    {
        const bool own = tid == k && lcode < 0;
        s_off[tid] = (long long)(own ? -1 - lcode : lrow) * ldt;
        s_coef[tid] = own ? 1.0 : lcf;
    }
    __syncthreads();
    ts.mark(PRS_STAMP_SLOT);
    double sv = 0.0, sz = 0.0, szb = 0.0, zc = 0.0, zbc = 0.0;
    if (scode < 0) {
        sv = v[-1 - scode];
        sz = z[spos];
        szb = zbar[spos];
    }
    if (pos >= 0) {
        zc = z[pos];
        zbc = zbar[pos];
    }
    const int nrows = k + (lcode < 0 ? 1 : 0);
    int G = (k + 1 + PR_BATCH - 1) / PR_BATCH;
    G = G > PR_GMAX ? PR_GMAX : G;
    const int slot = tid / LPG, h = tid % LPG;
    const long long jc = (long long)blockIdx.x * PRS_TILE + h * VEC;
    const double *col = At + (jc < ldt ? jc : 0);
    for (int g0 = slot; g0 < G; g0 += NS * NG) {
        double acc[NG][VEC];
#pragma unroll
        for (int t = 0; t < NG; ++t)
#pragma unroll
            for (int e = 0; e < VEC; ++e) acc[t][e] = 0.0;
        for (int r0 = 0; r0 < PR_BATCH; r0 += RPT) {
            if (RPT < PR_BATCH && g0 + r0 * G >= nrows) break;
#define PRS_ENTRY(T, U)                                                                              \
    const int c = g0 + NS * (T) + (r0 + (U)) * G;                                                    \
    const bool ok = g0 + NS * (T) < G && c < nrows
            long long off[NG][RPT];
#pragma unroll
            for (int t = 0; t < NG; ++t)
#pragma unroll
                for (int u = 0; u < RPT; ++u) {
                    PRS_ENTRY(t, u);
                    off[t][u] = s_off[ok ? c : 0];
                }
            double x[NG][RPT][VEC], cf[NG][RPT];
#pragma unroll
            for (int t = 0; t < NG; ++t)
#pragma unroll
                for (int u = 0; u < RPT; ++u) {
                    PRS_ENTRY(t, u);
                    const double *src = col + (ok ? off[t][u] : 0);
                    if constexpr (VEC == 2) {
                        const double2_t w = __builtin_nontemporal_load(reinterpret_cast<const double2_t *>(src));
                        x[t][u][0] = w.x;
                        x[t][u][1] = w.y;
                    } else {
                        x[t][u][0] = __builtin_nontemporal_load(src);
                    }
                }
            __builtin_amdgcn_sched_barrier(0);
#pragma unroll
            for (int t = 0; t < NG; ++t)
#pragma unroll
                for (int u = 0; u < RPT; ++u) {
                    PRS_ENTRY(t, u);
                    cf[t][u] = s_coef[ok ? c : 0];
                }
#pragma unroll
            for (int t = 0; t < NG; ++t)
#pragma unroll
                for (int u = 0; u < RPT; ++u) {
                    PRS_ENTRY(t, u);
#pragma unroll
                    for (int e = 0; e < VEC; ++e)
                        acc[t][e] = ok ? fma(cf[t][u], x[t][u][e], acc[t][e]) : acc[t][e];
                }
#undef PRS_ENTRY
        }
#pragma unroll
        for (int t = 0; t < NG; ++t)
            if (g0 + NS * t < G) {
#pragma unroll
                for (int e = 0; e < VEC; ++e) s_part[g0 + NS * t][h * VEC + e] = acc[t][e];
            }
    }
    __syncthreads();
    ts.mark(PRS_STAMP_SLOT);
    DzgCand2 best = dzg_cand2_none();
    if (pos >= 0) {
        double sum = 0.0;
        for (int g = 0; g < G; ++g) sum = sum + s_part[g][lane];
        dz[pos] = -sum;
        price_candidate_v(best, -sum, pos, mu, tau, zc, zbc);
    }
    if (scode < 0) {
        const double p = 1.0 * -sv;
        const double d = 0.0 + p;
        dz[spos] = d;
        price_candidate_v(best, d, spos, mu, tau, sz, szb);
    }
    for (int ps = spos + (int)gridDim.x * 512; ps < q; ps += (int)gridDim.x * 512) {
        const int code = nbcode[ps];
        if (code < 0) {
            const double p = 1.0 * -v[-1 - code];
            const double d = 0.0 + p;
            dz[ps] = d;
            price_candidate(best, d, ps, mu, tau, z, zbar);
        }
    }
    ts.pin(best);
    const unsigned long long t_publish = ts.now();
    price_publish_small(best, rz_r, rz_k, rz_h);
    ts.site(DZG_SITE_PUBLISH, t_publish);
    ts.mark(PRS_STAMP_SLOT);
    ts.done(PRS_STAMP_SLOT);
}

__global__ __launch_bounds__(256) void k_price_rows_finish(
    const DzgCtl *ctl, int rows_T, const double *__restrict__ part, long long ldt, int q,
    const int *__restrict__ plist, const int *__restrict__ pcode, const int *__restrict__ nbcode,
    const int *__restrict__ bcode, int col0, const double *__restrict__ v, double *__restrict__ dz,
    const double *__restrict__ z, const double *__restrict__ zbar, double *__restrict__ rz_r,
    int *__restrict__ rz_k, double *__restrict__ rz_h, int gmax, int need_kind = -1)
{
    const int nthreads = gridDim.x * blockDim.x;
    const int spos = blockIdx.x * blockDim.x + threadIdx.x;
    int scode = 0, pos0 = -1, code0 = -1;
    if (spos < q) {
        scode = nbcode[spos];
        pos0 = plist[spos];
        code0 = pcode[spos];
    }
    const int status = ctl->status, k = ctl->ncompact;
    const int count = (int)ctl->nb_struct;
    const double mu = ctl->mu, tau = ctl->tau;
    if (status != DZG_RUNNING || k >= rows_T) return;
    if (need_kind >= 0 && ctl->kind != need_kind) return;
    int G = (k + 1 + PR_BATCH - 1) / PR_BATCH;
    G = G > gmax ? gmax : G;
    DzgCand2 best = dzg_cand2_none();
    double sv = 0.0, sz = 0.0, szb = 0.0;
    if (scode < 0) {
        sv = v[-1 - scode];
        sz = z[spos];
        szb = zbar[spos];
    }
    for (int idx = spos; idx < count; idx += nthreads) {
        const int pos = idx == spos ? pos0 : plist[idx];
        const int code = idx == spos ? code0 : pcode[idx];
        if (code < 0) continue;
        const double zc = z[pos], zbc = zbar[pos];
        const double *src = part + (code - col0);
        double sum = 0.0;
        int gg = 0;
        for (; gg + 8 <= G; gg += 8) {
            double t[8];
#pragma unroll
            for (int e = 0; e < 8; ++e) t[e] = src[(long long)(gg + e) * ldt];
#pragma unroll
            for (int e = 0; e < 8; ++e) sum = sum + t[e];
        }
        for (; gg < G; ++gg) sum = sum + src[(long long)gg * ldt];
        dz[pos] = -sum;
        price_candidate_v(best, -sum, pos, mu, tau, zc, zbc);
    }
    if (scode < 0) {
        const double p = 1.0 * -sv;
        const double d = 0.0 + p;
        dz[spos] = d;
        price_candidate_v(best, d, spos, mu, tau, sz, szb);
    }
    for (int pos = spos + nthreads; pos < q; pos += nthreads) {
        const int code = nbcode[pos];
        if (code < 0) {
            const double p = 1.0 * -v[-1 - code];
            const double d = 0.0 + p;
            dz[pos] = d;
            price_candidate(best, d, pos, mu, tau, z, zbar);
        }
    }
    price_publish(best, rz_r, rz_k, rz_h);
}

__global__ __launch_bounds__(256) void k_transpose_to_rows(const double *__restrict__ A, long long lda,
                                                           int m, int n, double *__restrict__ At,
                                                           long long ldt)
{
    __shared__ double tile[32][33];
    const int j0 = blockIdx.x * 32, i0 = blockIdx.y * 32;
    for (int jj = threadIdx.y; jj < 32; jj += 8) {
        const int j = j0 + jj, i = i0 + threadIdx.x;
        tile[jj][threadIdx.x] = (j < n && i < m) ? A[(long long)j * lda + i] : 0.0;
    }
    __syncthreads();
    for (int ii = threadIdx.y; ii < 32; ii += 8) {
        const int i = i0 + ii, j = j0 + threadIdx.x;
// ... 9 lines not shown
```

include/dantzig_amd.h:

```cpp
#ifndef DANTZIG_AMD_H
#define DANTZIG_AMD_H

#include <stdint.h>

#ifdef __cplusplus
extern "C" {
#endif

#define DZG_ABI_VERSION 4

typedef enum {
    DZG_OPTIMAL = 0,
    DZG_UNBOUNDED = 1,
    DZG_INFEASIBLE = 2,
    DZG_ITER_LIMIT = 3,
    DZG_SINGULAR = 4,
    DZG_PANIC = 5,
    DZG_RUNNING = 6,
    DZG_NEAR_TIE = 7,
    DZG_NODE_LIMIT = 8,
    DZG_E_DEVICE = -1,
    DZG_E_ARG = -2,
    DZG_E_NOMEM = -3
} dzg_status;
// ... 349 lines not shown
int dzg_mip_solve(const dzg_model *model, const int32_t *is_integer, const dzg_opts *opts,
                  const dzg_mip_opts *mip_opts, dzg_mip_result *res);
void dzg_mip_last_warm_stats(dzg_mip_warm_stats *out);

typedef struct {
    int64_t m, n, n_struct, lda;
    double *a;
    int64_t *var_col;
    double *c;
    double constant;
    int64_t *basis, *nonbasis;
    double *x, *z;
    int64_t *pos_var, *neg_var;
} dzg_stdform;

int dzg_build_standard_form(const dzg_model *model, dzg_stdform *out);


int dzg_kernel_lu_solve(int64_t n, const double *a, const double *b, double *x_out,
                        double *lu_out, int64_t *p_out, int32_t device);

int dzg_kernel_neg_t_dot(int64_t m, int64_t n_struct, const double *a, int64_t lda,
                         const int64_t *cols, int64_t ncols, const double *v, double *out,
                         int32_t kernel, int32_t device);

int dzg_kernel_neg_t_dot_csc(int64_t m, int64_t n_struct, const int64_t *col_ptr,
                             const int32_t *row_idx, const double *val, const int64_t *cols,
                             int64_t ncols, const double *v, double *out, int32_t device);

int dzg_kernel_first_pivot(int64_t len, const double *y, const double *ybar, int64_t *pos_out,
                           int32_t device);
int dzg_kernel_second_pivot(int64_t len, double mu, const double *y, const double *ybar,
                            const double *dy, int64_t *pos_out, int32_t device);


int dzg_gen_sparse_lp(uint64_t seed, int64_t m, int64_t n_struct, int64_t per_col,
                      int64_t *col_ptr, int32_t *row_idx, double *val, double *b, double *c);

int dzg_gen_dense_lp(uint64_t seed, int64_t m, int64_t n_struct, double *a, int64_t lda,
                     double *b, double *c);

int dzg_gen_dense_lp_block(uint64_t seed, int64_t m, int64_t n_struct, int64_t col_begin,
                           int64_t col_end, double *a_block, int64_t lda, double *b, double *c);

typedef struct {
    double ratio;
    int64_t pos;
    double y, ybar, dy;
} dzg_candidate;

int64_t dzg_shard_record_doubles(const dzg_solver *s);
int dzg_shard_phase1(dzg_solver *s, double *send_dev);
int dzg_shard_phase2(dzg_solver *s, const double *recv_dev, double *send_dev);
int dzg_shard_phase3(dzg_solver *s, const double *recv_dev);
int dzg_comm_unique_id(void *unique_id_128);
int dzg_shard_comm_init(dzg_solver *s, const void *unique_id_128);
int dzg_shard_run(dzg_solver *s, int64_t max_new_iters);
int dzg_shard_comm_size(dzg_solver *s);
int dzg_shard_run_lockstep(dzg_solver **solvers, int32_t world, int64_t max_new_iters);
void *dzg_solver_stream(dzg_solver *s);
int dzg_solver_set_profile(dzg_solver *s, int32_t mask);
int dzg_solver_poll(dzg_solver *s, int32_t *status, int64_t *iterations);
int dzg_solver_set_budget(dzg_solver *s, int64_t max_new_iters);

int dzg_debug_hold_cus(int32_t device, int32_t workgroups, double seconds);
int dzg_debug_hold_wait(void);

int64_t dzg_debug_live_lists(dzg_solver *s, int64_t *entries);
int64_t dzg_debug_rl_listed(dzg_solver *s);
int dzg_debug_matrix(dzg_solver *s, int64_t col0, int64_t col1, double *out, int64_t ld_out);
int64_t dzg_debug_matrix_rows(dzg_solver *s, int64_t row0, int64_t row1, double *out, int64_t ld_out);
int dzg_debug_extend_ms(const dzg_solver *s, double ms[3]);
int dzg_debug_basis_inverse(dzg_solver *s, int64_t row0, int64_t row1, double *out, int64_t info[4]);
int dzg_debug_batch_fast_inverse(const dzg_lp *lps, int64_t count, const dzg_opts *opts, int64_t pivots,
                                 int64_t refactor_every, double *w_out, dzg_result *res);

int dzg_debug_cand_reduce(int32_t device, int32_t form, int64_t ncases, const double *r, const int32_t *k,
                          const double *h, const int32_t *count, double *out_r, int32_t *out_k,
                          double *out_h);

int dzg_debug_chain_instance(int32_t m, int32_t grid, int32_t k_bound, int32_t fold, int32_t nrz,
                             int32_t shard, int32_t post);

int64_t dzg_merge_candidates(const dzg_candidate *cands, int64_t count);

#ifdef __cplusplus
}
#endif
#endif
```

Measured before the change: 34320.

## Fuse small-pricing pass into chain pre kernel using compact eta-row copy

Folds the small-case pricing kernel into the tail of the persistent chain pre kernel when a rule allows it, removing a separate kernel launch per simplex iteration. To let pricing blocks compute the compact BTRAN values themselves, it keeps a compact copy of the eta rows (wk) that is appended to each iteration and regathered after refactor or fallback. The shared pricing code moves into a new header. This adds state that must stay consistent across refactors, plus extra LDS and register pressure in the pre kernel.

```diff
diff --git a/dantzig_amd/_build.py b/dantzig_amd/_build.py
--- a/dantzig_amd/_build.py
+++ b/dantzig_amd/_build.py
@@ -28,7 +28,7 @@
 
 
 def _deps():
-    hdrs = [os.path.join(CSRC, "common.h"), os.path.join(CSRC, "k_price_kernels.h"),
+    hdrs = [os.path.join(CSRC, "common.h"), os.path.join(CSRC, "k_price_kernels.h"), os.path.join(CSRC, "price_small.h"),
             os.path.join(CSRC, "fast_decide.h"), os.path.join(CSRC, "fast_rows.h"),
             os.path.join(CSRC, "chain_barrier.h"), os.path.join(CSRC, "batch_strict.h"),
             os.path.join(CSRC, "batch_host.h"),
diff --git a/dantzig_amd/_ffi.py b/dantzig_amd/_ffi.py
--- a/dantzig_amd/_ffi.py
+++ b/dantzig_amd/_ffi.py
@@ -33,6 +33,7 @@
     "dzg_core_solve_full_csc", "dzg_debug_live_lists", "dzg_debug_rl_listed",
     "dzg_debug_basis_inverse", "dzg_batch_solve", "dzg_model_solve_batch", "dzg_mip_opts_default",
     "dzg_mip_solve", "dzg_mip_last_warm_stats", "dzg_debug_cand_reduce", "dzg_debug_chain_instance",
+    "dzg_debug_chain_price_counts", "dzg_debug_wk_mismatch", "dzg_debug_chain_price_rule",
     "dzg_solver_duals", "dzg_batch_solve_duals", "dzg_model_solve_duals",
     "dzg_model_solve_batch_duals", "dzg_model_map_duals",
     "dzg_solver_ranging", "dzg_batch_solve_ranging", "dzg_model_solve_ranging",
@@ -265,6 +266,11 @@
                                                C.c_void_p, C.c_void_p, C.c_void_p, C.c_void_p, C.c_void_p]
         _lib.dzg_debug_chain_instance.restype = C.c_int
         _lib.dzg_debug_chain_instance.argtypes = [C.c_int32] * 7
+        _lib.dzg_debug_chain_price_counts.argtypes = [C.c_void_p, C.c_void_p]
+        _lib.dzg_debug_wk_mismatch.argtypes = [C.c_void_p, C.c_int32, C.c_void_p]
+        _lib.dzg_debug_chain_price_rule.restype = C.c_int
+        _lib.dzg_debug_chain_price_rule.argtypes = [C.c_int32, C.c_int32, C.c_int32, C.c_int32, C.c_int64,
+                                                    C.c_int32, C.c_int32]
         _lib.dzg_batch_solve.argtypes = [C.c_void_p, C.c_int64, C.c_void_p, C.c_int64, C.c_void_p]
         _lib.dzg_model_solve_batch.argtypes = [C.c_void_p, C.c_int64, C.c_void_p, C.c_void_p]
         _lib.dzg_batch_solve_fast.argtypes = [C.c_void_p, C.c_int64, C.c_void_p, C.c_int64, C.c_int64,
diff --git a/dantzig_amd/core.py b/dantzig_amd/core.py
--- a/dantzig_amd/core.py
+++ b/dantzig_amd/core.py
@@ -522,6 +522,17 @@
         _ffi.check(_ffi.lib().dzg_debug_basis_inverse(self._h, int(row0), int(row1), ptr(out), ptr(info)),
                    "dzg_debug_basis_inverse")
         return out, dict(k=int(info[0]), neta=int(info[1]), rows=(int(info[2]), int(info[3])))
+
+    def debug_chain_price_counts(self) -> tuple[int, int]:
+        counts = np.zeros(2, np.int64)
+        _ffi.check(_ffi.lib().dzg_debug_chain_price_counts(self._h, ptr(counts)), "dzg_debug_chain_price_counts")
+        return int(counts[0]), int(counts[1])
+
+    def debug_wk_mismatch(self, clear_valid: bool = False) -> tuple[int, bool]:
+        info = np.zeros(2, np.int64)
+        _ffi.check(_ffi.lib().dzg_debug_wk_mismatch(self._h, int(bool(clear_valid)), ptr(info)),
+                   "dzg_debug_wk_mismatch")
+        return int(info[0]), bool(info[1])
 
     def close(self) -> None:
         if self._h:
diff --git a/dantzig_amd/csrc/common.h b/dantzig_amd/csrc/common.h
--- a/dantzig_amd/csrc/common.h
+++ b/dantzig_amd/csrc/common.h
@@ -563,10 +563,11 @@
     int k_hint;
     int price_cols_hint;
     int rs, rs_r0, rs_r1;
+    int fold_k;
     long long rs_mcol;
     int ftran_variant;
     int ftran_nt_k;
-    int fold_k;
+    double *wk;
 };
 
 #ifdef __HIPCC__
@@ -644,7 +645,12 @@
     DZG_CHAIN_P4_WIDE = 3,
 };
 void dzg_launch_chain_pre(const DzgDev &d, int grid, unsigned long long *bar,
-                          unsigned long long *dbg, const double *xrecv, hipStream_t st, int instances = 0);
+                          unsigned long long *dbg, const double *xrecv, hipStream_t st, int instances = 0,
+                          int price = 0);
+int dzg_chain_price_rule(int m, int grid, int k_hint, int tiles, long long q, int small, int timed);
+int dzg_chain_price_fused(const DzgDev &d, int grid, int small, int timed);
+int dzg_chain_keeps_wk(const DzgDev &d, int grid, int small);
+void dzg_launch_gather_wk(const DzgDev &d, double *dst, hipStream_t st);
 void dzg_launch_chain_post(const DzgDev &d, int grid, unsigned long long *bar,
                            unsigned long long *dbg, int only_partials, int nrz, const double *xrecv,
                            hipStream_t st, int fold = 0, int price_small = 0, int instances = 0);
diff --git a/dantzig_amd/csrc/engine.hip b/dantzig_amd/csrc/engine.hip
--- a/dantzig_amd/csrc/engine.hip
+++ b/dantzig_amd/csrc/engine.hip
@@ -127,6 +127,9 @@
     bool batch_chain = false;
     bool chain_fold = true;
     bool chain_instances = true;
+    bool chain_price_fused = true;
+    double *wk_buf = nullptr;
+    int64_t chain_fused = 0, chain_unfused = 0;
     int64_t chain_fallbacks = 0;
     long long chain_retry_iter = 0;
     void *comm = nullptr;
@@ -757,6 +760,12 @@
                 if (d.rows_T < 1) { d.At = nullptr; d.vc = nullptr; }
             }
         }
+        if (s->chain_bar && s->chain_grid > 0 && !d.spb && d.At && d.vc && d.cpos && d.world <= 1 && !d.rs &&
+            dzg_price_small_partials(d) <= s->chain_grid) {
+            TRY(dev_alloc(s, &s->wk_buf, (size_t)d.ldw * DZG_RMAX));
+            HIP_OK(hipMemsetAsync(s->wk_buf, 0, sizeof(double) * (size_t)d.ldw * DZG_RMAX, s->st));
+            if (const char *pf = std::getenv("DZG_CHAIN_PRICE_FUSED")) s->chain_price_fused = pf[0] != '0';
+        }
         dzg_launch_fast_init(d, s->st);
         if (d.spb) {
             dzg_launch_sp_init(d, 1, s->st);
@@ -880,14 +889,17 @@
     hipStream_t st = s->st;
     Prof pf{s, slot};
     const int pk = price_kernel_for(s);
+    const int small = dzg_price_small(d, pk);
+    const int fold = !small && s->chain_fold && dzg_price_rows_certain(d, pk);
+    const int fused = s->chain_price_fused &&
+                      dzg_chain_price_fused(d, s->chain_grid, small, prof_on(s, DZG_K_PRICE, slot));
+    (fused ? s->chain_fused : s->chain_unfused) += 1;
     pf.begin(DZG_K_FTRAN);
     dzg_launch_chain_pre(d, s->chain_grid, s->chain_bar, s->chain_dbg, nullptr, st,
-                         s->chain_instances);
+                         s->chain_instances, fused);
     pf.end(DZG_K_FTRAN);
-    const int small = dzg_price_small(d, pk);
-    const int fold = !small && s->chain_fold && dzg_price_rows_certain(d, pk);
     pf.begin(DZG_K_PRICE);
-    dzg_launch_price_fast(d, pk, st, -1, fold, small, small ? s->chain_dbg : nullptr);
+    if (!fused) dzg_launch_price_fast(d, pk, st, -1, fold, small, small ? s->chain_dbg : nullptr);
     pf.end(DZG_K_PRICE);
     pf.begin(DZG_K_UPDATE);
     dzg_launch_chain_post(d, s->chain_grid, s->chain_bar, s->chain_dbg, 0,
@@ -1117,6 +1129,7 @@
 
 static int refactor_now(dzg_solver *s, bool at_end)
 {
+    s->d.wk = nullptr;
     if (partitioned(s) && s->in_lockstep)
         return fail(DZG_E_ARG, "refactor: the lockstep loop refactorises its ranks together");
     int counts[2];
@@ -1254,6 +1267,7 @@
 {
     DzgCtl *h = s->h_ctl;
     s->chain_fallbacks += 1;
+    s->d.wk = nullptr;
     s->chain_retry_iter = s->chain_fallbacks >= 3 ? std::numeric_limits<long long>::max()
                                                   : h->iter + 64ll * s->opts.poll_interval;
     HIP_OK(hipMemsetAsync(s->chain_bar, 0, sizeof(unsigned long long) * DZG_CHAIN_BAR_WORDS, s->st));
@@ -1303,10 +1317,19 @@
                              (long long)s->h_ctl->ncompact + batch <= s->chain_kcap;
             s->d.k_hint = k_bound;
             s->d.k_lo_hint = k_low;
-            if (s->batch_chain)
+            if (s->batch_chain) {
+                if (!(s->wk_buf && s->chain_price_fused && s->chain_instances &&
+                      dzg_chain_keeps_wk(s->d, s->chain_grid, dzg_price_small(s->d, price_kernel_for(s))))) {
+                    s->d.wk = nullptr;
+                } else if (!s->d.wk) {
+                    dzg_launch_gather_wk(s->d, s->wk_buf, s->st);
+                    s->d.wk = s->wk_buf;
+                }
                 for (int b = 0; b < batch; ++b) enqueue_chain_iteration(s, b);
-            else
+            } else {
+                s->d.wk = nullptr;
                 for (int b = 0; b < batch; ++b) enqueue_fast_iteration(s, b);
+            }
             s->d.k_hint = s->d.k_lo_hint = 0;
         }
         s->since_refactor += batch;
@@ -1505,6 +1528,7 @@
 extern "C" int dzg_shard_phase3(dzg_solver *s, const double *recv_dev)
 {
     if (!s || !recv_dev || s->numerics != DZG_NUMERICS_FAST) return fail(DZG_E_ARG, "phase3");
+    s->d.wk = nullptr;
     const DzgDev &d = s->d;
     hipStream_t st = s->st;
     phase_stamp(s, DZG_K_UPDATE, 0);
@@ -3412,3 +3436,44 @@
     HIP_OK(hipSetDevice(device));
     return dzg_run_second_pivot(len, mu, y, ybar, dy, pos_out);
 }
+
+extern "C" int dzg_debug_chain_price_counts(dzg_solver *s, int64_t counts[2])
+{
+    if (!s || !counts) return fail(DZG_E_ARG, "NULL argument");
+    counts[0] = s->chain_fused;
+    counts[1] = s->chain_unfused;
+    return 0;
+}
+
+extern "C" int dzg_debug_chain_price_rule(int32_t m, int32_t grid, int32_t k_hint, int32_t tiles, int64_t q,
+                                          int32_t small, int32_t timed)
+{
+    return dzg_chain_price_rule(m, grid, k_hint, tiles, q, small, timed);
+}
+
+extern "C" int dzg_debug_wk_mismatch(dzg_solver *s, int32_t clear_valid, int64_t info[2])
+{
+    if (!s || !info) return fail(DZG_E_ARG, "NULL argument");
+    const DzgDev &d = s->d;
+    if (!s->wk_buf) return fail(DZG_E_ARG, "wk mismatch: this solver keeps no compact copy of the eta rows");
+    HIP_OK(hipSetDevice(s->opts.device));
+    TRY(read_ctl(s));
+    const int k = s->h_ctl->ncompact, neta = s->h_ctl->neta;
+    if (k < 0 || k > d.m || neta < 0 || neta > DZG_RMAX)
+        return fail(DZG_E_DEVICE, "wk mismatch: control block out of range");
+    info[1] = s->d.wk ? 1 : 0;
+    dzg_launch_gather_wk(d, d.Wc, s->st);
+    const size_t n = (size_t)d.ldw * DZG_RMAX;
+    std::vector<double> kept(n), fresh(n);
+    HIP_OK(hipMemcpyAsync(kept.data(), s->wk_buf, sizeof(double) * n, hipMemcpyDeviceToHost, s->st));
+    HIP_OK(hipMemcpyAsync(fresh.data(), d.Wc, sizeof(double) * n, hipMemcpyDeviceToHost, s->st));
+    HIP_OK(hipStreamSynchronize(s->st));
+    HIP_OK(hipGetLastError());
+    int64_t bad = 0;
+    for (int t = 0; t < neta; ++t)
+        for (int c = 0; c < k; ++c)
+            bad += std::memcmp(&kept[(size_t)t * d.ldw + c], &fresh[(size_t)t * d.ldw + c], sizeof(double)) != 0;
+    info[0] = bad;
+    if (clear_valid) s->d.wk = nullptr;
+    return 0;
+}
diff --git a/dantzig_amd/csrc/k_chain.hip b/dantzig_amd/csrc/k_chain.hip
--- a/dantzig_amd/csrc/k_chain.hip
+++ b/dantzig_amd/csrc/k_chain.hip
@@ -2,6 +2,7 @@
 #include "common.h"
 #include "fast_decide.h"
 #include "fast_rows.h"
+#include "price_small.h"
 
 #include "chain_barrier.h"
 
@@ -290,12 +291,23 @@
     }
 }
 
-template <bool SHARD, int MAXP, bool NARROW>
+#define CHP_COL0 32
+typedef const __attribute__((address_space(4))) DzgDev ChainDevArg;
+__device__ __forceinline__ ChainDevArg *chain_dev_reloaded()
+{
+    ChainDevArg *kd = (ChainDevArg *)__builtin_amdgcn_kernarg_segment_ptr();
+    asm volatile("" : "+s"(kd));
+    return kd;
+}
+template <bool SHARD, int MAXP, bool NARROW, int PRICE = 0>
 __global__ __launch_bounds__(CH_THREADS) void k_chain_pre(const DzgDev d, unsigned long long *bar,
                                                           unsigned long long *dbg,
                                                           const double *__restrict__ xrecv)
 {
-    __shared__ double s_ag[CH_AGCAP];
+    static_assert(PRICE == 0 || (!SHARD && NARROW && MAXP == 1 && PRICE <= 2), "the pricing tail: P1, narrow");
+    static_assert(CH_THREADS == 512 && CH_AGCAP >= 2 * PRS_ROWS + PR_GMAX * PRS_TILE, "the tail's LDS");
+    constexpr bool WK = !SHARD && NARROW && MAXP == 1;
+    __shared__ __attribute__((aligned(16))) double s_ag[CH_AGCAP];
     __shared__ double s_beta[R_], s_dx[CH_THREADS], s_up[R_];
     __shared__ ChainSlots s_c;
     ChainStamps ts;
@@ -324,6 +336,21 @@
         x_i = d.x[row];
         xbar_i = d.xbar[row];
     }
+    const int tiles = PRICE ? (int)((d.ldt + PRS_TILE - 1) / PRS_TILE) : 0;
+    const int spos = (int)blockIdx.x * CH_THREADS + tid, cc = tid - CHP_COL0;
+    int scode = 0, pos = -1, lrow_c = 0;
+    double sz = 0.0, szb = 0.0;
+    const bool tile_on = PRICE != 0 && (int)blockIdx.x < tiles;
+    if (tile_on) {
+        if (spos < d.q) {
+            scode = d.nbcode[spos];
+            sz = d.z[spos];
+            szb = d.zbar[spos];
+        }
+        const long long j = (long long)blockIdx.x * PRS_TILE + lane;
+        if (wave == 0 && j < d.col1 - d.col0) pos = d.cpos[j];
+        if (cc >= 0) lrow_c = d.drow[cc < m ? cc : m - 1];
+    }
     DzgCtl c = *ctl;
     if (c.status != DZG_RUNNING) return;
     unsigned long long gen = c.bar_gen;
@@ -349,6 +376,11 @@
     const int slot = kind == DZG_STEP_PRIMAL ? 0 : 1;
     ts.mark(slot);
     if (k > CH_AGCAP || c.fp_count > 256 || (NARROW && k > 512)) {
+        if (lead) ctl->status = DZG_PANIC;
+        return;
+    }
+    if (PRICE != 0 && (k >= d.rows_T || k >= CH_THREADS - CHP_COL0 || r1 - r0 > CHP_COL0 ||
+                       tiles > nwg || (long long)tiles * CH_THREADS < d.q || !d.wk)) {
         if (lead) ctl->status = DZG_PANIC;
         return;
     }
@@ -452,17 +484,45 @@
     }
     double up = 0.0, base = 0.0, w[R_];
     if (tid < R_ && tid < neta) up = d.U[(long long)tid * d.ldw + p];
-    if (has_row) {
-        if (dslot_i >= 0) base = d.binv[(long long)p * d.ldb + dslot_i];
-        fast_btran_eta_load(w, neta, d.W, d.ldw, row);
-    }
-    if (tid < R_) s_up[tid] = up;
-    __syncthreads();
-    if (has_row) {
-        if (dslot_i < 0) base = lcode == -1 - row ? 1.0 : 0.0;
-        const double vr = base - fast_btran_eta_fma(w, neta, s_up);
-        d.v[row] = vr;
-        if (dslot_i >= 0 && d.vc) d.vc[dslot_i] = vr;
+    int sd = -1;
+    double zc = 0.0, zbc = 0.0, vr = 0.0;
+    if constexpr (PRICE == 0) {
+        if (has_row) {
+            if (dslot_i >= 0) base = d.binv[(long long)p * d.ldb + dslot_i];
+            fast_btran_eta_load(w, neta, d.W, d.ldw, row);
+        }
+        if (tid < R_) s_up[tid] = up;
+        __syncthreads();
+        if (has_row) {
+            if (dslot_i < 0) base = lcode == -1 - row ? 1.0 : 0.0;
+            vr = base - fast_btran_eta_fma(w, neta, s_up);
+            d.v[row] = vr;
+            if (dslot_i >= 0 && d.vc) d.vc[dslot_i] = vr;
+            if constexpr (WK)
+                if (dslot_i >= 0 && d.wk && neta < R_) d.wk[(long long)neta * d.ldw + dslot_i] = vr;
+        }
+    } else {
+        const bool is_col = tile_on && cc >= 0 && cc < k;
+        if (scode < 0) sd = d.dslot[-1 - scode];
+        if (pos >= 0) {
+            zc = d.z[pos];
+            zbc = d.zbar[pos];
+        }
+        if (is_col) base = d.binv[(long long)p * d.ldb + cc];
+        if (has_row && dslot_i >= 0) base = d.binv[(long long)p * d.ldb + dslot_i];
+        if (has_row || is_col)
+            fast_btran_eta_load(w, neta, is_col ? d.wk : d.W, d.ldw, is_col ? cc : row);
+        if (tid < R_) s_up[tid] = up;
+        __syncthreads();
+        if (has_row || is_col) {
+            if (has_row && dslot_i < 0) base = lcode == -1 - row ? 1.0 : 0.0;
+            vr = base - fast_btran_eta_fma(w, neta, s_up);
+        }
+        if (has_row) {
+            d.v[row] = vr;
+            if (dslot_i >= 0 && d.vc) d.vc[dslot_i] = vr;
+            if (dslot_i >= 0 && neta < R_) d.wk[(long long)neta * d.ldw + dslot_i] = vr;
+        }
     }
     if (lead) {
         ctl->xp = xp;
@@ -472,6 +532,35 @@
     }
     ts.mark(slot);
     ts.done(slot);
+    if constexpr (PRICE != 0) {
+        if ((int)blockIdx.x >= tiles) return;
+        const auto *kd = chain_dev_reloaded();
+        if (kd->ctl != ctl) {
+            if (lead) ctl->status = DZG_PANIC;
+            return;
+        }
+        const long long ldt = kd->ldt;
+        ts.stage = 1;
+        long long *s_off = reinterpret_cast<long long *>(s_ag);
+        double *s_coef = s_ag + PRS_ROWS;
+        double(*s_part)[PRS_TILE] = reinterpret_cast<double(*)[PRS_TILE]>(s_ag + 2 * PRS_ROWS);
+        if (cc >= 0) {
+            const bool own = cc == k && lcode < 0;
+            s_off[cc] = (long long)(own ? -1 - lcode : lrow_c) * ldt;
+            s_coef[cc] = own ? 1.0 : vr;
+        }
+        __syncthreads();
+        ts.mark(PRS_STAMP_SLOT);
+        const double sv = sd >= 0 && sd < k ? s_coef[sd] : 0.0;
+        const int G = price_small_rows<2, PRICE, PR_BATCH>(kd->At, ldt, (int)blockIdx.x, k, lcode, s_off, s_coef,
+                                                           s_part);
+        __syncthreads();
+        ts.mark(PRS_STAMP_SLOT);
+        price_small_finish<false>(ts, G, s_part, pos, zc, zbc, scode, spos, sv, sz, szb, tiles, kd->q, kd->nbcode,
+                                  kd->v, kd->dz, kd->z, kd->zbar, mu, c.tau, kd->rz_r, kd->rz_k, kd->rz_h);
+        ts.mark(PRS_STAMP_SLOT);
+        ts.done(PRS_STAMP_SLOT);
+    }
 }
 
 __device__ __forceinline__ double chain_fold_dz(const DzgDev &d, int code, int G)
@@ -792,6 +881,21 @@
         }
         ts.mark(slot);
     }
+    if constexpr (!SHARD && NARROW && MAXP == 1 && NOFOLD)
+    if (d.wk && !only_partials && (int)blockIdx.x == ((int)gridDim.x > 1 ? 1 : 0) && wave == 2 &&
+        lane <= teta && (app_col >= 0 || del_last >= 0)) {
+        double *wrow = d.wk + (long long)lane * d.ldw;
+        double wk_app = 0.0;
+        if (app_col >= 0) {
+            const int rl = -1 - new_code_r;
+            wk_app = lane < teta ? d.W[(long long)lane * d.ldw + rl] : d.v[rl];
+        }
+        if (del_last >= 0) {
+            if (del_ce != del_last) wrow[del_ce] = app_col == del_last ? wk_app : wrow[del_last];
+        } else {
+            wrow[app_col] = wk_app;
+        }
+    }
     DzgCand2 bx = dzg_cand2_none(), bz = dzg_cand2_none();
     if (has_row) {
         double xi = x_i, xb = xbar_i;
@@ -888,6 +992,8 @@
         reinterpret_cast<const void *>(k_chain_pre<false, 1, true>),
         reinterpret_cast<const void *>(k_chain_pre<false, 4, true>),
         reinterpret_cast<const void *>(k_chain_pre<false, 4, false>),
+        reinterpret_cast<const void *>(k_chain_pre<false, 1, true, 1>),
+        reinterpret_cast<const void *>(k_chain_pre<false, 1, true, 2>),
         reinterpret_cast<const void *>(k_chain_post<false, CH_MAXP, false, false>),
         reinterpret_cast<const void *>(k_chain_post<true, CH_MAXP, false, false>),
         reinterpret_cast<const void *>(k_chain_post<false, 1, true, true>),
@@ -902,10 +1008,34 @@
     return least;
 }
 
+int dzg_chain_price_rule(int m, int grid, int k_hint, int tiles, long long q, int small, int timed)
+{
+    if (!small || timed || tiles < 1 || tiles > grid || (long long)tiles * CH_THREADS < q) return 0;
+    if (k_hint <= 0 || k_hint >= CH_THREADS - CHP_COL0) return 0;
+    return chain_pick(m, grid, k_hint, 0, 0, 0, 0) == DZG_CHAIN_P1_NARROW;
+}
+int dzg_chain_price_fused(const DzgDev &d, int grid, int small, int timed)
+{
+    return d.wk && d.At && dzg_chain_price_rule(d.m, grid, d.k_hint, dzg_price_small_partials(d), d.q, small, timed);
+}
+int dzg_chain_keeps_wk(const DzgDev &d, int grid, int small)
+{
+    const int tiles = dzg_price_small_partials(d);
+    return d.At && dzg_chain_price_rule(d.m, grid, d.k_hint, tiles, d.q, small, 0) &&
+           chain_pick(d.m, grid, d.k_hint, 0, tiles, 0, 1) == DZG_CHAIN_P1_NARROW;
+}
+
 void dzg_launch_chain_pre(const DzgDev &d, int grid, unsigned long long *bar,
-                          unsigned long long *dbg, const double *xrecv, hipStream_t st, int instances)
+                          unsigned long long *dbg, const double *xrecv, hipStream_t st, int instances, int price)
 {
     const int which = instances ? chain_pick(d.m, grid, d.k_hint, 0, 0, xrecv != nullptr, 0) : DZG_CHAIN_GENERIC;
+    if (price && !xrecv) {
+        if (d.k_hint < 16 * DZG_PR_BATCH - 1)
+            hipLaunchKernelGGL((k_chain_pre<false, 1, true, 1>), dim3(grid), dim3(CH_THREADS), 0, st, d, bar, dbg, xrecv);
+        else
+            hipLaunchKernelGGL((k_chain_pre<false, 1, true, 2>), dim3(grid), dim3(CH_THREADS), 0, st, d, bar, dbg, xrecv);
+        return;
+    }
     if (xrecv)
         hipLaunchKernelGGL((k_chain_pre<true, CH_MAXP, false>), dim3(grid), dim3(CH_THREADS), 0, st, d, bar, dbg, xrecv);
     else if (which == DZG_CHAIN_P1_NARROW)
diff --git a/dantzig_amd/csrc/k_fast.hip b/dantzig_amd/csrc/k_fast.hip
--- a/dantzig_amd/csrc/k_fast.hip
+++ b/dantzig_amd/csrc/k_fast.hip
@@ -326,9 +326,9 @@
 
 __global__ __launch_bounds__(256) void k_fast_gather_w(const DzgCtl *ctl, const double *__restrict__ W,
                                                        long long ldw, const int *__restrict__ drow,
-                                                       double *__restrict__ Wc)
-{
-    if (ctl->neta < R_) return;
+                                                       double *__restrict__ Wc, int full_only)
+{
+    if (full_only && ctl->neta < R_) return;
     const int k = ctl->ncompact, neta = ctl->neta;
     const int t = blockIdx.y;
     const int c = blockIdx.x * blockDim.x + threadIdx.x;
@@ -659,7 +659,7 @@
 {
     const int kmax = d.k_hint > 0 && d.k_hint < d.m ? d.k_hint : d.m;
     hipLaunchKernelGGL(k_fast_gather_w, dim3((kmax + 15 + 255) / 256, R_), dim3(256), 0, st, d.ctl,
-                       d.W, d.ldw, d.drow, d.Wc);
+                       d.W, d.ldw, d.drow, d.Wc, 1);
     const int r0 = d.rs ? d.rs_r0 : 0, rows = (d.rs ? d.rs_r1 : d.m) - r0;
     double *binv = d.binv + (long long)r0 * d.ldb;
     const double *U = d.U + r0;
@@ -678,6 +678,13 @@
     hipLaunchKernelGGL(k_fast_flush_done, dim3(1), dim3(1), 0, st, d.ctl, ((kmax + 63) / 64) * 64);
 }
 
+void dzg_launch_gather_wk(const DzgDev &d, double *dst, hipStream_t st)
+{
+    const int kmax = d.k_hint > 0 && d.k_hint < d.m ? d.k_hint : d.m;
+    hipLaunchKernelGGL(k_fast_gather_w, dim3((kmax + 15 + 255) / 256, R_), dim3(256), 0, st, d.ctl,
+                       d.W, d.ldw, d.drow, dst ? dst : d.wk, 0);
+}
+
 void dzg_launch_shard_propose(const DzgDev &d, int mode, int nrz, double *xsend, hipStream_t st)
 {
     const int hdr_only = d.xstride <= 8;
diff --git a/dantzig_amd/csrc/k_price_kernels.h b/dantzig_amd/csrc/k_price_kernels.h
--- a/dantzig_amd/csrc/k_price_kernels.h
+++ b/dantzig_amd/csrc/k_price_kernels.h
@@ -1,40 +1,13 @@
 #pragma once
 #include "common.h"
-
-typedef double double2_t __attribute__((ext_vector_type(2)));
+#include "price_small.h"
+
 
 __device__ __forceinline__ int price_code(const int *__restrict__ nonbasis,
                                           const int *__restrict__ var_col, int pos)
 {
     const int v = nonbasis[pos];
     return var_col ? var_col[v] : v;
-}
-
-__device__ __forceinline__ void price_candidate(DzgCand2 &best, double dzk, int pos, double mu,
-                                                double tau, const double *__restrict__ z,
-                                                const double *__restrict__ zbar)
-{
-    const double zk = z[pos], scaled = mu * zbar[pos];
-    const double den = zk + scaled;
-    DzgCand2 c;
-    c.r = dzg_div(dzk, den);
-    c.k = pos;
-    c.h = -__builtin_inf();
-    if (c.r > 0.0) best = dzg_better2(best, c);
-    if (dzg_noise_zero(den, zk, scaled, tau)) best.h = __builtin_inf();
-}
-
-__device__ __forceinline__ void price_candidate_v(DzgCand2 &best, double dzk, int pos, double mu,
-                                                  double tau, double zk, double zbk)
-{
-    const double scaled = mu * zbk;
-    const double den = zk + scaled;
-    DzgCand2 c;
-    c.r = dzg_div(dzk, den);
-    c.k = pos;
-    c.h = -__builtin_inf();
-    if (c.r > 0.0) best = dzg_better2(best, c);
-    if (dzg_noise_zero(den, zk, scaled, tau)) best.h = __builtin_inf();
 }
 
 __device__ __forceinline__ void price_slack_positions(DzgCand2 &best, int q,
@@ -61,17 +34,6 @@
                                               int *__restrict__ rz_k, double *__restrict__ rz_h)
 {
     best = dzg_block_best2(best);
-    if (rz_r && threadIdx.x == 0) {
-        rz_r[blockIdx.x] = best.r;
-        rz_k[blockIdx.x] = best.k;
-        rz_h[blockIdx.x] = best.h;
-    }
-}
-
-__device__ __forceinline__ void price_publish_small(DzgCand2 best, double *__restrict__ rz_r,
-                                                    int *__restrict__ rz_k, double *__restrict__ rz_h)
-{
-    best = dzg_block_best2_flat<8>(best, false);
     if (rz_r && threadIdx.x == 0) {
         rz_r[blockIdx.x] = best.r;
         rz_k[blockIdx.x] = best.k;
@@ -704,8 +666,6 @@
                                __ATOMIC_RELAXED, __HIP_MEMORY_SCOPE_AGENT);
 }
 
-#define PR_GMAX DZG_PR_GMAX
-#define PR_BATCH DZG_PR_BATCH
 #define PR_PIPE 8
 template <int VEC, int PIPE = PR_PIPE>
 __global__ __launch_bounds__(256) void k_price_rows(
@@ -805,9 +765,6 @@
     }
 }
 
-#define PRS_TILE 64
-#define PRS_ROWS 512
-#define PRS_STAMP_SLOT 4
 template <int VEC, int NG, int RPT>
 __global__ __launch_bounds__(512, (RPT < PR_BATCH ? 8 : 2)) void k_price_rows_small(
     DzgCtl *__restrict__ ctl, int rows_T, const double *__restrict__ At, long long ldt, int ncols,
@@ -817,10 +774,6 @@
     double *__restrict__ rz_r, int *__restrict__ rz_k, double *__restrict__ rz_h,
     unsigned long long *dbg)
 {
-    constexpr int LPG = 64 / VEC;
-    constexpr int NS = 512 / LPG;
-    static_assert(VEC == 1 || VEC == 2, "8- or 16-byte loads");
-    static_assert(PR_BATCH % RPT == 0 && PR_GMAX * PR_BATCH >= PRS_ROWS, "a group has at most PR_BATCH rows");
     __shared__ long long s_off[PRS_ROWS];
     __shared__ double s_coef[PRS_ROWS];
     __shared__ __attribute__((aligned(16))) double s_part[PR_GMAX][PRS_TILE];
@@ -864,100 +817,11 @@
         zc = z[pos];
         zbc = zbar[pos];
     }
-    const int nrows = k + (lcode < 0 ? 1 : 0);
-    int G = (k + 1 + PR_BATCH - 1) / PR_BATCH;
-    G = G > PR_GMAX ? PR_GMAX : G;
-    const int slot = tid / LPG, h = tid % LPG;
-    const long long jc = (long long)blockIdx.x * PRS_TILE + h * VEC;
-    const double *col = At + (jc < ldt ? jc : 0);
-    for (int g0 = slot; g0 < G; g0 += NS * NG) {
-        double acc[NG][VEC];
-#pragma unroll
-        for (int t = 0; t < NG; ++t)
-#pragma unroll
-            for (int e = 0; e < VEC; ++e) acc[t][e] = 0.0;
-        for (int r0 = 0; r0 < PR_BATCH; r0 += RPT) {
-            if (RPT < PR_BATCH && g0 + r0 * G >= nrows) break;
-#define PRS_ENTRY(T, U)                                                                              \
-    const int c = g0 + NS * (T) + (r0 + (U)) * G;                                                    \
-    const bool ok = g0 + NS * (T) < G && c < nrows
-            long long off[NG][RPT];
-#pragma unroll
-            for (int t = 0; t < NG; ++t)
-#pragma unroll
-                for (int u = 0; u < RPT; ++u) {
-                    PRS_ENTRY(t, u);
-                    off[t][u] = s_off[ok ? c : 0];
-                }
-            double x[NG][RPT][VEC], cf[NG][RPT];
-#pragma unroll
-            for (int t = 0; t < NG; ++t)
-#pragma unroll
-                for (int u = 0; u < RPT; ++u) {
-                    PRS_ENTRY(t, u);
-                    const double *src = col + (ok ? off[t][u] : 0);
-                    if constexpr (VEC == 2) {
-                        const double2_t w = __builtin_nontemporal_load(reinterpret_cast<const double2_t *>(src));
-                        x[t][u][0] = w.x;
-                        x[t][u][1] = w.y;
-                    } else {
-                        x[t][u][0] = __builtin_nontemporal_load(src);
-                    }
-                }
-            __builtin_amdgcn_sched_barrier(0);
-#pragma unroll
-            for (int t = 0; t < NG; ++t)
-#pragma unroll
-                for (int u = 0; u < RPT; ++u) {
-                    PRS_ENTRY(t, u);
-                    cf[t][u] = s_coef[ok ? c : 0];
-                }
-#pragma unroll
-            for (int t = 0; t < NG; ++t)
-#pragma unroll
-                for (int u = 0; u < RPT; ++u) {
-                    PRS_ENTRY(t, u);
-#pragma unroll
-                    for (int e = 0; e < VEC; ++e)
-                        acc[t][e] = ok ? fma(cf[t][u], x[t][u][e], acc[t][e]) : acc[t][e];
-                }
-#undef PRS_ENTRY
-        }
-#pragma unroll
-        for (int t = 0; t < NG; ++t)
-            if (g0 + NS * t < G) {
-#pragma unroll
-                for (int e = 0; e < VEC; ++e) s_part[g0 + NS * t][h * VEC + e] = acc[t][e];
-            }
-    }
+    const int G = price_small_rows<VEC, NG, RPT>(At, ldt, (int)blockIdx.x, k, lcode, s_off, s_coef, s_part);
     __syncthreads();
     ts.mark(PRS_STAMP_SLOT);
-    DzgCand2 best = dzg_cand2_none();
-    if (pos >= 0) {
-        double sum = 0.0;
-        for (int g = 0; g < G; ++g) sum = sum + s_part[g][lane];
-        dz[pos] = -sum;
-        price_candidate_v(best, -sum, pos, mu, tau, zc, zbc);
-    }
-    if (scode < 0) {
-        const double p = 1.0 * -sv;
-        const double d = 0.0 + p;
-        dz[spos] = d;
-        price_candidate_v(best, d, spos, mu, tau, sz, szb);
-    }
-    for (int ps = spos + (int)gridDim.x * 512; ps < q; ps += (int)gridDim.x * 512) {
-        const int code = nbcode[ps];
-        if (code < 0) {
-            const double p = 1.0 * -v[-1 - code];
-            const double d = 0.0 + p;
-            dz[ps] = d;
-            price_candidate(best, d, ps, mu, tau, z, zbar);
-        }
-    }
-    ts.pin(best);
-    const unsigned long long t_publish = ts.now();
-    price_publish_small(best, rz_r, rz_k, rz_h);
-    ts.site(DZG_SITE_PUBLISH, t_publish);
+    price_small_finish<true>(ts, G, s_part, pos, zc, zbc, scode, spos, sv, sz, szb, (int)gridDim.x, q, nbcode, v, dz, z,
+                             zbar, mu, tau, rz_r, rz_k, rz_h);
     ts.mark(PRS_STAMP_SLOT);
     ts.done(PRS_STAMP_SLOT);
 }
diff --git a/dantzig_amd/csrc/price_small.h b/dantzig_amd/csrc/price_small.h
--- /dev/null
+++ b/dantzig_amd/csrc/price_small.h
@@ -0,0 +1,166 @@
+#pragma once
+#include "common.h"
+
+typedef double double2_t __attribute__((ext_vector_type(2)));
+
+#define PR_GMAX DZG_PR_GMAX
+#define PR_BATCH DZG_PR_BATCH
+
+__device__ __forceinline__ void price_candidate(DzgCand2 &best, double dzk, int pos, double mu,
+                                                double tau, const double *__restrict__ z,
+                                                const double *__restrict__ zbar)
+{
+    const double zk = z[pos], scaled = mu * zbar[pos];
+    const double den = zk + scaled;
+    DzgCand2 c;
+    c.r = dzg_div(dzk, den);
+    c.k = pos;
+    c.h = -__builtin_inf();
+    if (c.r > 0.0) best = dzg_better2(best, c);
+    if (dzg_noise_zero(den, zk, scaled, tau)) best.h = __builtin_inf();
+}
+
+__device__ __forceinline__ void price_candidate_v(DzgCand2 &best, double dzk, int pos, double mu,
+                                                  double tau, double zk, double zbk)
+{
+    const double scaled = mu * zbk;
+    const double den = zk + scaled;
+    DzgCand2 c;
+    c.r = dzg_div(dzk, den);
+    c.k = pos;
+    c.h = -__builtin_inf();
+    if (c.r > 0.0) best = dzg_better2(best, c);
+    if (dzg_noise_zero(den, zk, scaled, tau)) best.h = __builtin_inf();
+}
+
+__device__ __forceinline__ void price_publish_small(DzgCand2 best, double *__restrict__ rz_r,
+                                                    int *__restrict__ rz_k, double *__restrict__ rz_h)
+{
+    best = dzg_block_best2_flat<8>(best, false);
+    if (rz_r && threadIdx.x == 0) {
+        rz_r[blockIdx.x] = best.r;
+        rz_k[blockIdx.x] = best.k;
+        rz_h[blockIdx.x] = best.h;
+    }
+}
+
+#define PRS_TILE 64
+#define PRS_ROWS 512
+#define PRS_STAMP_SLOT 4
+template <int VEC, int NG, int RPT>
+__device__ __forceinline__ int price_small_rows(const double *__restrict__ At, long long ldt, int tile, int k,
+                                                int lcode, const long long *s_off, const double *s_coef,
+                                                double (*s_part)[PRS_TILE])
+{
+    constexpr int LPG = 64 / VEC;
+    constexpr int NS = 512 / LPG;
+    static_assert(VEC == 1 || VEC == 2, "8- or 16-byte loads");
+    static_assert(PR_BATCH % RPT == 0 && PR_GMAX * PR_BATCH >= PRS_ROWS, "a group has at most PR_BATCH rows");
+    const int tid = threadIdx.x;
+    const int nrows = k + (lcode < 0 ? 1 : 0);
+    int G = (k + 1 + PR_BATCH - 1) / PR_BATCH;
+    G = G > PR_GMAX ? PR_GMAX : G;
+    const int slot = tid / LPG, h = tid % LPG;
+    const long long jc = (long long)tile * PRS_TILE + h * VEC;
+    const double *col = At + (jc < ldt ? jc : 0);
+    for (int g0 = slot; g0 < G; g0 += NS * NG) {
+        double acc[NG][VEC];
+#pragma unroll
+        for (int t = 0; t < NG; ++t)
+#pragma unroll
+            for (int e = 0; e < VEC; ++e) acc[t][e] = 0.0;
+        for (int r0 = 0; r0 < PR_BATCH; r0 += RPT) {
+            if (RPT < PR_BATCH && g0 + r0 * G >= nrows) break;
+#define PRS_ENTRY(T, U)                                                                              \
+    const int c = g0 + NS * (T) + (r0 + (U)) * G;                                                    \
+    const bool ok = g0 + NS * (T) < G && c < nrows
+            long long off[NG][RPT];
+#pragma unroll
+            for (int t = 0; t < NG; ++t)
+#pragma unroll
+                for (int u = 0; u < RPT; ++u) {
+                    PRS_ENTRY(t, u);
+                    off[t][u] = s_off[ok ? c : 0];
+                }
+            double x[NG][RPT][VEC], cf[NG][RPT];
+#pragma unroll
+            for (int t = 0; t < NG; ++t)
+#pragma unroll
+                for (int u = 0; u < RPT; ++u) {
+                    PRS_ENTRY(t, u);
+                    const double *src = col + (ok ? off[t][u] : 0);
+                    if constexpr (VEC == 2) {
+                        const double2_t w = __builtin_nontemporal_load(reinterpret_cast<const double2_t *>(src));
+                        x[t][u][0] = w.x;
+                        x[t][u][1] = w.y;
+                    } else {
+                        x[t][u][0] = __builtin_nontemporal_load(src);
+                    }
+                }
+            __builtin_amdgcn_sched_barrier(0);
+#pragma unroll
+            for (int t = 0; t < NG; ++t)
+#pragma unroll
+                for (int u = 0; u < RPT; ++u) {
+                    PRS_ENTRY(t, u);
+                    cf[t][u] = s_coef[ok ? c : 0];
+                }
+#pragma unroll
+            for (int t = 0; t < NG; ++t)
+#pragma unroll
+                for (int u = 0; u < RPT; ++u) {
+                    PRS_ENTRY(t, u);
+#pragma unroll
+                    for (int e = 0; e < VEC; ++e)
+                        acc[t][e] = ok ? fma(cf[t][u], x[t][u][e], acc[t][e]) : acc[t][e];
+                }
+#undef PRS_ENTRY
+        }
+#pragma unroll
+        for (int t = 0; t < NG; ++t)
+            if (g0 + NS * t < G) {
+#pragma unroll
+                for (int e = 0; e < VEC; ++e) s_part[g0 + NS * t][h * VEC + e] = acc[t][e];
+            }
+    }
+    return G;
+}
+
+template <bool STRIDED>
+__device__ __forceinline__ void price_small_finish(ChainStamps &ts, int G, const double (*s_part)[PRS_TILE],
+                                                   int pos, double zc, double zbc, int scode, int spos,
+                                                   double sv, double sz, double szb, int nwg, int q,
+                                                   const int *__restrict__ nbcode, const double *__restrict__ v,
+                                                   double *__restrict__ dz, const double *__restrict__ z,
+                                                   const double *__restrict__ zbar, double mu, double tau,
+                                                   double *__restrict__ rz_r, int *__restrict__ rz_k,
+                                                   double *__restrict__ rz_h)
+{
+    const int lane = threadIdx.x & 63;
+    DzgCand2 best = dzg_cand2_none();
+    if (pos >= 0) {
+        double sum = 0.0;
+        for (int g = 0; g < G; ++g) sum = sum + s_part[g][lane];
+        dz[pos] = -sum;
+        price_candidate_v(best, -sum, pos, mu, tau, zc, zbc);
+    }
+    if (scode < 0) {
+        const double p = 1.0 * -sv;
+        const double d = 0.0 + p;
+        dz[spos] = d;
+        price_candidate_v(best, d, spos, mu, tau, sz, szb);
+    }
+    for (int ps = spos + nwg * 512; STRIDED && ps < q; ps += nwg * 512) {
+        const int code = nbcode[ps];
+        if (code < 0) {
+            const double p = 1.0 * -v[-1 - code];
+            const double d = 0.0 + p;
+            dz[ps] = d;
+            price_candidate(best, d, ps, mu, tau, z, zbar);
+        }
+    }
+    ts.pin(best);
+    const unsigned long long t_publish = ts.now();
+    price_publish_small(best, rz_r, rz_k, rz_h);
+    ts.site(DZG_SITE_PUBLISH, t_publish);
+}
diff --git a/include/dantzig_amd.h b/include/dantzig_amd.h
--- a/include/dantzig_amd.h
+++ b/include/dantzig_amd.h
@@ -455,6 +455,11 @@
 int dzg_debug_chain_instance(int32_t m, int32_t grid, int32_t k_bound, int32_t fold, int32_t nrz,
                              int32_t shard, int32_t post);
 
+int dzg_debug_chain_price_counts(dzg_solver *s, int64_t counts[2]);
+int dzg_debug_wk_mismatch(dzg_solver *s, int32_t clear_valid, int64_t info[2]);
+int dzg_debug_chain_price_rule(int32_t m, int32_t grid, int32_t k_hint, int32_t tiles, int64_t q,
+                               int32_t small, int32_t timed);
+
 int64_t dzg_merge_candidates(const dzg_candidate *cands, int64_t count);
 
 #ifdef __cplusplus
```

Result: faster. 35570, median of 6 (+3.6%).
